# cvjena/mvlm

Measured on NVIDIA B200. Metric: scans/sec, higher is better.
Workload: dtype bf16

## Files before the change

### include/mvlm_b200.h

```cpp
#ifndef MVLM_B200_H
#define MVLM_B200_H

#include <stddef.h>
#include <stdint.h>

#ifdef __cplusplus
extern "C" {
#endif

#define MVLM_OK 0
#define MVLM_E_INVALID (-1)
#define MVLM_E_CUDA (-2)
#define MVLM_E_UNSUPPORTED (-3)

const char* mvlm_last_error(void);
int mvlm_version(void);
long long mvlm_launch_count(int reset);

typedef struct mvlm_conv_args {
  const void* in;
  int n, h, w, cin, in_cs;
  const void* wpacked;
  int cout_pad, n_tile, kh, kw, y_off0, x_off0;
  const float* bias;
  const float* pre_scale;
  const float* pre_shift;
  void* out_pre;
  int pre_cs, pre_co;
  const void* res1;
  int res1_cs, res1_co;
  const void* res2;
  int res2_cs, res2_co;
  void* out_raw;
  int raw_cs, raw_co;
  const float* post_scale;
  const float* post_shift;
  void* out_post;
  int post_cs, post_co;
  float* out_f32;
  unsigned long long* argmax_keys;
  int cout_real;
  int up_sy, up_sx, up_py, up_px;
  const float* mid_scale;
  const float* mid_shift;
  int pool2;
  const void* res_up;
  int up_cs, up_co;
} mvlm_conv_args;

int mvlm_conv2d_bf16(const mvlm_conv_args* args, void* stream);

void mvlm_debug_conv_profile(long long* dev_buf);
int mvlm_debug_conv_profile_ints(void);
void mvlm_debug_conv_mode(int mode);

int mvlm_pack_conv_weight(const float* w_oihw, int cout, int cin, int kh, int kw, int cout_pad,
                          int cin_pad, void* out_bf16, void* stream);

typedef struct mvlm_obj mvlm_obj;
int mvlm_obj_load(const char* path, int n_threads, mvlm_obj** out);
int mvlm_obj_counts(const mvlm_obj* obj, int* n_verts, int* n_tris, int* has_uv);
int mvlm_obj_copy(const mvlm_obj* obj, float* verts, float* uvs, int32_t* tris);
void mvlm_obj_free(mvlm_obj* obj);
#define MVLM_OBJ_MATERIALS 1
int mvlm_obj_load_ex(const char* path, int n_threads, int flags, mvlm_obj** out);
int mvlm_obj_materials(const mvlm_obj* obj, int32_t* tri_material, int* n_materials, int* n_libraries);
const char* mvlm_obj_material_name(const mvlm_obj* obj, int i);
const char* mvlm_obj_library_name(const mvlm_obj* obj, int i);
int mvlm_debug_obj_chunk_starts(const char* text, size_t len, int n_threads, long long* starts);

typedef struct mvlm_obj_parse_info {
  int32_t n_verts, n_tris, has_uv, fallback;
  int32_t n_positions;
  size_t n_bytes;
} mvlm_obj_parse_info;
size_t mvlm_obj_parse_workspace_bytes(size_t n_bytes);
int mvlm_obj_parse_device(const char* text_dev, size_t n_bytes, const char* path, void* workspace,
                          size_t workspace_bytes, void* stream, mvlm_obj_parse_info* info);
int mvlm_obj_parse_write(const mvlm_obj_parse_info* info, const void* workspace, float* verts, float* uvs,
                         int32_t* tris, void* stream);
#define MVLM_OBJ_MAX_NAME_LINES 65536
typedef struct mvlm_obj_name_line {
  int64_t offset;
  int32_t kind;
  int32_t tris_before;
} mvlm_obj_name_line;
size_t mvlm_obj_parse_workspace_bytes_ex(size_t n_bytes, int flags);
int mvlm_obj_parse_device_ex(const char* text_dev, size_t n_bytes, const char* path, void* workspace,
                             size_t workspace_bytes, int flags, void* stream, mvlm_obj_parse_info* info,
                             mvlm_obj_name_line* name_lines, int max_name_lines, int* n_name_lines);
int mvlm_obj_parse_tri_page(const mvlm_obj_parse_info* info, void* workspace, const int32_t* line_page, int n_usemtl,
                            int32_t* tri_page, void* stream);
int mvlm_debug_obj_parse_lines(const char* text, size_t len, int max_lines, int* n_lines, int32_t* kind,
                               int32_t* status, float* values, int32_t* n_tris, long long* corners,
                               long long max_corners);

typedef struct mvlm_mesh mvlm_mesh;
int mvlm_mesh_load(const char* path, int n_threads, mvlm_mesh** out);
int mvlm_mesh_counts(const mvlm_mesh* mesh, int* n_verts, int* n_tris, int* has_colors);
int mvlm_mesh_copy(const mvlm_mesh* mesh, float* verts, uint8_t* colors, int32_t* tris);
void mvlm_mesh_free(mvlm_mesh* mesh);

typedef struct mvlm_mesh_parse_info {
  int32_t n_verts, n_tris, has_colors, fallback;
  int32_t is_stl;
  size_t n_bytes;
} mvlm_mesh_parse_info;
size_t mvlm_mesh_parse_workspace_bytes(size_t n_bytes, int is_stl);
int mvlm_mesh_parse_device(const uint8_t* host, size_t n_bytes, int is_stl, const char* path, void* workspace,
                           size_t workspace_bytes, void* stream, mvlm_mesh_parse_info* info);
int mvlm_mesh_parse_write(const mvlm_mesh_parse_info* info, const void* workspace, float* verts, uint8_t* colors,
                          int32_t* tris, void* stream);

int mvlm_jpeg_info(const uint8_t* data, size_t len, int* width, int* height);
int mvlm_jpeg_decode_rgb(const uint8_t* data, size_t len, uint8_t* out_rgb_dev, int width, int height, void* stream);

size_t mvlm_raster_workspace_bytes(int n_views, int h, int w, int n_verts);
int mvlm_raster_multiview(const float* verts, int n_verts, const float* uvs, const int32_t* tris, int n_tris,
                          const uint8_t* tex, int tex_h, int tex_w, int tex_channels, const double* rot,
                          int n_views, int h, int w, int channel_mode, void* workspace, size_t workspace_bytes,
                          uint8_t* out_u8 , float* out_f32 ,
                          int32_t* out_tri_id , float* out_depth ,
                          void* stream);

#define MVLM_MAX_SCANS 64
typedef struct mvlm_raster_scan {
  const float* verts;
  int n_verts;
  const float* uvs;
  const int32_t* tris;
  int n_tris;
  const uint8_t* tex;
  int tex_h, tex_w, tex_channels;
} mvlm_raster_scan;
size_t mvlm_raster_multiscan_workspace_bytes(int n_scans, int n_views, int h, int w, int max_verts);
int mvlm_raster_multiscan(const mvlm_raster_scan* scans , int n_scans,
                          const double* rot , int n_views, int h, int w, int channel_mode, void* workspace,
                          size_t workspace_bytes, uint8_t* out_u8 , float* out_f32 ,
                          int32_t* out_tri_id , float* out_depth , void* stream);
int mvlm_raster_multiscan_colored(const mvlm_raster_scan* scans ,
                                  const uint8_t* const* vertex_rgba ,
                                  int n_scans, const double* rot , int n_views, int h, int w,
                                  int channel_mode, void* workspace, size_t workspace_bytes, uint8_t* out_u8,
                                  float* out_f32, int32_t* out_tri_id, float* out_depth, void* stream);
int mvlm_raster_multiscan_paged(const mvlm_raster_scan* scans ,
                                const uint8_t* const* vertex_rgba ,
                                const int32_t* const* pages ,
                                int n_scans, const double* rot , int n_views, int h, int w, int channel_mode,
                                void* workspace, size_t workspace_bytes, uint8_t* out_u8, float* out_f32,
                                int32_t* out_tri_id, float* out_depth, void* stream);

typedef struct mvlm_hourglass mvlm_hourglass;
size_t mvlm_hourglass_workspace_bytes(int n_landmarks, int cin, int n_views, int h, int w);
double mvlm_hourglass_flops_per_view(int n_landmarks, int cin, int h, int w);
int mvlm_hourglass_create(const char* const* names, const void* const* ptrs, const long long* numels,
                          int n_entries, int n_landmarks, int cin, int n_views, int h, int w, void* workspace,
                          size_t workspace_bytes, mvlm_hourglass** out);
int mvlm_hourglass_forward(mvlm_hourglass* net, const uint8_t* img_u8, const float* img_f32,
                           float* out_heatmaps, float* out_peaks, void* stream);
int mvlm_hourglass_forward_graph(mvlm_hourglass* net, const uint8_t* img_u8, const float* img_f32,
                                 float* out_heatmaps, float* out_peaks, void* stream);
int mvlm_hourglass_set_selection_method(mvlm_hourglass* net, int method);
int mvlm_hourglass_forward_keys(mvlm_hourglass* net, const uint8_t* img_u8, const float* img_f32, uint64_t* out_keys,
                                void* stream);
int mvlm_peaks_from_gathered_keys(const uint64_t* keys, int n_views, int n_landmarks, int w, int world, int slot_views,
                                  float* out_peaks , void* stream);
int mvlm_hourglass_num_launches(const mvlm_hourglass* net);
int mvlm_debug_hourglass_profile(mvlm_hourglass* net, const uint8_t* img_u8, const float* img_f32,
                                 float* out_peaks, int reps, float* ms_out, double* roles_out, int trace_op,
                                 long long* trace_out ,
                                 void* stream);
int mvlm_debug_hourglass_describe(const mvlm_hourglass* net, int op, char* buf, int buf_len);
int mvlm_hourglass_probe(const mvlm_hourglass* net, const char* name, const void** ptr, int* h, int* w, int* c);
void mvlm_hourglass_destroy(mvlm_hourglass* net);

int mvlm_heatmap_peaks(const float* heatmaps, int n_views, int n_landmarks, int h, int w, int method,
                       float* out_peaks, void* stream);

int mvlm_rays_from_peaks(const float* peaks , const double* rot , int n_landmarks,
                         int n_views, int image_size, double* out_starts, double* out_ends, void* stream);

size_t mvlm_consensus_workspace_bytes(int n_landmarks, int n_views, int n_hyp);
int mvlm_consensus(const float* peaks, const double* starts, const double* ends, int n_landmarks,
                   int n_views, int mode, double threshold_quantile, float threshold_absolute,
                   const uint32_t* draws, int n_hyp, double dist_thres, void* workspace,
                   size_t workspace_bytes, double* out_landmarks , double* out_errors ,
                   int32_t* out_nlines , void* stream);

size_t mvlm_consensus_multiscan_workspace_bytes(int n_scans, int n_landmarks, int n_views, int n_hyp);
int mvlm_consensus_multiscan(const float* peaks, const double* starts, const double* ends, int n_scans,
                             int n_landmarks, int n_views, int mode, double threshold_quantile,
                             float threshold_absolute, const uint32_t* draws, int draws_per_scan, int n_hyp,
                             double dist_thres, void* workspace, size_t workspace_bytes,
                             double* out_landmarks , double* out_errors ,
                             int32_t* out_nlines , void* stream);

size_t mvlm_snap_workspace_bytes(int n_landmarks, int n_tris);
int mvlm_snap_to_mesh(const float* verts, const int32_t* tris, int n_tris, const double* landmarks,
                      int n_landmarks, void* workspace, size_t workspace_bytes, double* out ,
                      int32_t* out_tri , void* stream);

size_t mvlm_snap_grid_bytes(int n_tris);
size_t mvlm_snap_grid_query_workspace_bytes(int n_landmarks, int n_tris);
int mvlm_snap_grid_build(const float* verts, const int32_t* tris, int n_tris, void* grid, size_t grid_bytes,
                         void* stream);
int mvlm_snap_grid_query(const float* verts, const int32_t* tris, int n_tris, const void* grid,
                         size_t grid_bytes, const double* landmarks, int n_landmarks, void* workspace,
                         size_t workspace_bytes, double* out , int32_t* out_tri ,
                         int32_t* out_stats , void* stream);
typedef struct mvlm_snap_mesh {
  const float* verts;
  const int32_t* tris;
  int n_tris;
  const void* grid;
  size_t grid_bytes;
} mvlm_snap_mesh;
size_t mvlm_snap_to_meshes_workspace_bytes(const mvlm_snap_mesh* meshes, int n_scans, int n_landmarks);
int mvlm_snap_to_meshes(const mvlm_snap_mesh* meshes, int n_scans, const double* landmarks ,
                        int n_landmarks, void* workspace, size_t workspace_bytes, double* out ,
                        int32_t* out_tri , void* stream);
int mvlm_debug_snap_grid_describe(const void* grid, int32_t* dims_nover , double* edge_tau ,
                                  void* stream);

#ifdef __cplusplus
}
#endif
#endif
```

### mvlm_b200/_lib.py

```python
from __future__ import annotations

import ctypes as C
import os
from pathlib import Path

_HERE = Path(__file__).resolve().parent
LIB_PATH = Path(os.environ.get("MVLM_B200_LIB") or _HERE / "libmvlm_b200.so")


class MvlmError(RuntimeError):
    pass


class ConvArgs(C.Structure):
    _fields_ = [
        ("in_", C.c_void_p),
        ("n", C.c_int), ("h", C.c_int), ("w", C.c_int), ("cin", C.c_int), ("in_cs", C.c_int),
        ("wpacked", C.c_void_p),
        ("cout_pad", C.c_int), ("n_tile", C.c_int), ("kh", C.c_int), ("kw", C.c_int),
        ("y_off0", C.c_int), ("x_off0", C.c_int),
        ("bias", C.c_void_p),
        ("pre_scale", C.c_void_p), ("pre_shift", C.c_void_p), ("out_pre", C.c_void_p),
        ("pre_cs", C.c_int), ("pre_co", C.c_int),
        ("res1", C.c_void_p), ("res1_cs", C.c_int), ("res1_co", C.c_int),
        ("res2", C.c_void_p), ("res2_cs", C.c_int), ("res2_co", C.c_int),
        ("out_raw", C.c_void_p), ("raw_cs", C.c_int), ("raw_co", C.c_int),
        ("post_scale", C.c_void_p), ("post_shift", C.c_void_p), ("out_post", C.c_void_p),
        ("post_cs", C.c_int), ("post_co", C.c_int),
        ("out_f32", C.c_void_p), ("argmax_keys", C.c_void_p),
        ("cout_real", C.c_int),
        ("up_sy", C.c_int), ("up_sx", C.c_int), ("up_py", C.c_int), ("up_px", C.c_int),
        ("mid_scale", C.c_void_p), ("mid_shift", C.c_void_p),
        ("pool2", C.c_int),
        ("res_up", C.c_void_p), ("up_cs", C.c_int), ("up_co", C.c_int),
    ]


class ObjParseInfo(C.Structure):
    _fields_ = [("n_verts", C.c_int32), ("n_tris", C.c_int32), ("has_uv", C.c_int32), ("fallback", C.c_int32),
                ("n_positions", C.c_int32), ("n_bytes", C.c_size_t)]


class ObjNameLine(C.Structure):
    _fields_ = [("offset", C.c_int64), ("kind", C.c_int32), ("tris_before", C.c_int32)]


class MeshParseInfo(C.Structure):
    _fields_ = [("n_verts", C.c_int32), ("n_tris", C.c_int32), ("has_colors", C.c_int32), ("fallback", C.c_int32),
                ("is_stl", C.c_int32), ("n_bytes", C.c_size_t)]


class RasterScan(C.Structure):
    _fields_ = [("verts", C.c_void_p), ("n_verts", C.c_int), ("uvs", C.c_void_p), ("tris", C.c_void_p),
                ("n_tris", C.c_int), ("tex", C.c_void_p), ("tex_h", C.c_int), ("tex_w", C.c_int),
                ("tex_channels", C.c_int)]


class SnapMesh(C.Structure):
    _fields_ = [("verts", C.c_void_p), ("tris", C.c_void_p), ("n_tris", C.c_int), ("grid", C.c_void_p),
                ("grid_bytes", C.c_size_t)]


MAX_SCANS = 64
OBJ_MATERIALS = 1
OBJ_MAX_NAME_LINES = 65536

_lib = None


def load() -> C.CDLL:
    global _lib
    if _lib is not None:
        return _lib
    if not LIB_PATH.exists():
        raise MvlmError(
            f"{LIB_PATH} is missing: run `python -m mvlm_b200.build` (there is no CPU fallback)")
    lib = C.CDLL(str(LIB_PATH))
    lib.mvlm_last_error.restype = C.c_char_p
    lib.mvlm_launch_count.restype = C.c_longlong
    lib.mvlm_launch_count.argtypes = [C.c_int]
    _lib = lib
    _declare(lib)
    return lib


def _declare(lib: C.CDLL) -> None:
    vp, i32, f32, f64, u64 = C.c_void_p, C.c_int, C.c_float, C.c_double, C.c_uint64
    sigs = {
        "mvlm_version": ([], i32),
        "mvlm_conv2d_bf16": ([C.POINTER(ConvArgs), vp], i32),
        "mvlm_pack_conv_weight": ([vp, i32, i32, i32, i32, i32, i32, vp, vp], i32),
        "mvlm_raster_workspace_bytes": ([i32, i32, i32, i32], C.c_size_t),
        "mvlm_raster_multiview": ([vp, i32, vp, vp, i32, vp, i32, i32, i32, vp, i32, i32, i32, i32, vp, C.c_size_t, vp, vp,
                                   vp, vp, vp], i32),
        "mvlm_raster_multiscan_workspace_bytes": ([i32, i32, i32, i32, i32], C.c_size_t),
        "mvlm_raster_multiscan": ([C.POINTER(RasterScan), i32, vp, i32, i32, i32, i32, vp, C.c_size_t, vp, vp, vp, vp, vp],
                                  i32),
        "mvlm_raster_multiscan_colored": ([C.POINTER(RasterScan), C.POINTER(vp), i32, vp, i32, i32, i32, i32, vp,
                                           C.c_size_t, vp, vp, vp, vp, vp], i32),
        "mvlm_raster_multiscan_paged": ([C.POINTER(RasterScan), C.POINTER(vp), C.POINTER(vp), i32, vp, i32, i32, i32,
                                         i32, vp, C.c_size_t, vp, vp, vp, vp, vp], i32),
        "mvlm_hourglass_workspace_bytes": ([i32, i32, i32, i32, i32], C.c_size_t),
        "mvlm_hourglass_flops_per_view": ([i32, i32, i32, i32], f64),
        "mvlm_hourglass_create": ([C.POINTER(C.c_char_p), C.POINTER(vp), C.POINTER(C.c_longlong), i32, i32, i32, i32,
                                   i32, i32, vp, C.c_size_t, C.POINTER(vp)], i32),
        "mvlm_hourglass_forward": ([vp, vp, vp, vp, vp, vp], i32),
        "mvlm_hourglass_forward_graph": ([vp, vp, vp, vp, vp, vp], i32),
        "mvlm_hourglass_set_selection_method": ([vp, i32], i32),
        "mvlm_hourglass_forward_keys": ([vp, vp, vp, vp, vp], i32),
        "mvlm_peaks_from_gathered_keys": ([vp, i32, i32, i32, i32, i32, vp, vp], i32),
        "mvlm_hourglass_num_launches": ([vp], i32),
        "mvlm_debug_hourglass_profile": ([vp, vp, vp, vp, i32, C.POINTER(C.c_float), C.POINTER(C.c_double), i32,
                                         C.POINTER(C.c_longlong), vp], i32),
        "mvlm_debug_conv_profile_ints": ([], i32),
        "mvlm_debug_hourglass_describe": ([vp, i32, C.c_char_p, i32], i32),
        "mvlm_hourglass_probe": ([vp, C.c_char_p, C.POINTER(vp), C.POINTER(i32), C.POINTER(i32), C.POINTER(i32)], i32),
        "mvlm_hourglass_destroy": ([vp], None),
        "mvlm_obj_load": ([C.c_char_p, i32, C.POINTER(vp)], i32),
        "mvlm_obj_counts": ([vp, C.POINTER(i32), C.POINTER(i32), C.POINTER(i32)], i32),
        "mvlm_obj_copy": ([vp, vp, vp, vp], i32),
        "mvlm_obj_free": ([vp], None),
        "mvlm_obj_load_ex": ([C.c_char_p, i32, i32, C.POINTER(vp)], i32),
        "mvlm_obj_materials": ([vp, vp, C.POINTER(i32), C.POINTER(i32)], i32),
        "mvlm_obj_material_name": ([vp, i32], C.c_char_p),
        "mvlm_obj_library_name": ([vp, i32], C.c_char_p),
        "mvlm_debug_obj_chunk_starts": ([C.c_char_p, C.c_size_t, i32, vp], i32),
        "mvlm_obj_parse_workspace_bytes": ([C.c_size_t], C.c_size_t),
        "mvlm_obj_parse_device": ([vp, C.c_size_t, C.c_char_p, vp, C.c_size_t, vp, C.POINTER(ObjParseInfo)], i32),
        "mvlm_obj_parse_write": ([C.POINTER(ObjParseInfo), vp, vp, vp, vp, vp], i32),
        "mvlm_obj_parse_workspace_bytes_ex": ([C.c_size_t, i32], C.c_size_t),
        "mvlm_obj_parse_device_ex": ([vp, C.c_size_t, C.c_char_p, vp, C.c_size_t, i32, vp, C.POINTER(ObjParseInfo),
                                      C.POINTER(ObjNameLine), i32, C.POINTER(i32)], i32),
        "mvlm_obj_parse_tri_page": ([C.POINTER(ObjParseInfo), vp, vp, i32, vp, vp], i32),
        "mvlm_debug_obj_parse_lines": ([C.c_char_p, C.c_size_t, i32, C.POINTER(i32), vp, vp, vp, vp, vp, C.c_longlong],
                                       i32),
        "mvlm_mesh_load": ([C.c_char_p, i32, C.POINTER(vp)], i32),
        "mvlm_mesh_counts": ([vp, C.POINTER(i32), C.POINTER(i32), C.POINTER(i32)], i32),
        "mvlm_mesh_copy": ([vp, vp, vp, vp], i32),
        "mvlm_mesh_free": ([vp], None),
        "mvlm_mesh_parse_workspace_bytes": ([C.c_size_t, i32], C.c_size_t),
        "mvlm_mesh_parse_device": ([vp, C.c_size_t, i32, C.c_char_p, vp, C.c_size_t, vp, C.POINTER(MeshParseInfo)], i32),
        "mvlm_mesh_parse_write": ([C.POINTER(MeshParseInfo), vp, vp, vp, vp, vp], i32),
        "mvlm_jpeg_info": ([C.c_char_p, C.c_size_t, C.POINTER(i32), C.POINTER(i32)], i32),
        "mvlm_jpeg_decode_rgb": ([C.c_char_p, C.c_size_t, vp, i32, i32, vp], i32),
        "mvlm_heatmap_peaks": ([vp, i32, i32, i32, i32, i32, vp, vp], i32),
        "mvlm_rays_from_peaks": ([vp, vp, i32, i32, i32, vp, vp, vp], i32),
        "mvlm_consensus_workspace_bytes": ([i32, i32, i32], C.c_size_t),
        "mvlm_consensus": ([vp, vp, vp, i32, i32, i32, f64, f32, vp, i32, f64, vp, C.c_size_t, vp, vp, vp, vp], i32),
        "mvlm_consensus_multiscan_workspace_bytes": ([i32, i32, i32, i32], C.c_size_t),
        "mvlm_consensus_multiscan": ([vp, vp, vp, i32, i32, i32, i32, f64, f32, vp, i32, i32, f64, vp, C.c_size_t, vp, vp,
                                      vp, vp], i32),
        "mvlm_snap_workspace_bytes": ([i32, i32], C.c_size_t),
        "mvlm_snap_to_meshes_workspace_bytes": ([C.POINTER(SnapMesh), i32, i32], C.c_size_t),
        "mvlm_snap_to_meshes": ([C.POINTER(SnapMesh), i32, vp, i32, vp, C.c_size_t, vp, vp, vp], i32),
        "mvlm_snap_to_mesh": ([vp, vp, i32, vp, i32, vp, C.c_size_t, vp, vp, vp], i32),
        "mvlm_snap_grid_bytes": ([i32], C.c_size_t),
        "mvlm_snap_grid_build": ([vp, vp, i32, vp, C.c_size_t, vp], i32),
        "mvlm_snap_grid_query_workspace_bytes": ([i32, i32], C.c_size_t),
        "mvlm_snap_grid_query": ([vp, vp, i32, vp, C.c_size_t, vp, i32, vp, C.c_size_t, vp, vp, vp, vp], i32),
        "mvlm_debug_snap_grid_describe": ([vp, vp, vp, vp], i32),
    }
    sigs.update(_EXTRA_SIGS)
    for name, (argtypes, restype) in sigs.items():
        fn = getattr(lib, name)
        fn.argtypes = argtypes
        fn.restype = restype


_EXTRA_SIGS: dict = {}


def check(rc: int, what: str = "") -> None:
    if rc != 0:
        msg = load().mvlm_last_error().decode("utf-8", "replace")
        raise MvlmError(f"{what or 'mvlm call'} failed ({rc}): {msg}")


def ptr(t) -> int | None:
    if t is None:
        return None
    return t.data_ptr()


def cur_stream() -> int:
    import torch

    return torch.cuda.current_stream().cuda_stream
```

### mvlm_b200/csrc/api.cu

```cuda
#include <stdarg.h>

#include <atomic>

#include "../../include/mvlm_b200.h"
#include "common.cuh"
#include "conv_umma.cuh"
#include "hourglass.cuh"
#include "stages.cuh"

namespace mvlm {

static thread_local char g_err[1024] = "";
static std::atomic<long long> g_launches{0};

void set_error(const char* fmt, ...) {
  va_list ap;
  va_start(ap, fmt);
  vsnprintf(g_err, sizeof(g_err), fmt, ap);
  va_end(ap);
}

void count_launch(int n) { g_launches.fetch_add(n, std::memory_order_relaxed); }

int sm_count() {
  static std::atomic<int> cached[kMaxDevices];
  int dev = 0;
  if (cudaGetDevice(&dev) != cudaSuccess || dev < 0 || dev >= kMaxDevices) return kNumSMs;
  int n = cached[dev].load(std::memory_order_relaxed);
  if (n == 0) {
    if (cudaDeviceGetAttribute(&n, cudaDevAttrMultiProcessorCount, dev) != cudaSuccess || n <= 0) n = kNumSMs;
    cached[dev].store(n, std::memory_order_relaxed);
  }
  return n;
}

}

using namespace mvlm;
static_assert(kMaxScans == MVLM_MAX_SCANS, "scan table size");

extern "C" {

const char* mvlm_last_error(void) { return g_err; }

int mvlm_version(void) { return 1; }

long long mvlm_launch_count(int reset) {
  return reset ? g_launches.exchange(0) : g_launches.load();
}

void mvlm_debug_conv_profile(long long* dev_buf) { conv_set_profile_buffer(dev_buf); }
int mvlm_debug_conv_profile_ints(void) { return kConvProfInts; }
void mvlm_debug_conv_mode(int mode) { conv_set_debug_mode(mode); }

int mvlm_conv2d_bf16(const mvlm_conv_args* a, void* stream) {
  MVLM_REQUIRE(a != nullptr, "mvlm_conv2d_bf16: null args");
  ConvShape s;
  s.in = static_cast<const __nv_bfloat16*>(a->in);
  s.n = a->n; s.h = a->h; s.w = a->w; s.cin = a->cin; s.in_cs = a->in_cs;
  s.wpacked = static_cast<const __nv_bfloat16*>(a->wpacked);
  s.cout_pad = a->cout_pad; s.n_tile = a->n_tile; s.kh = a->kh; s.kw = a->kw;
  s.y_off0 = a->y_off0; s.x_off0 = a->x_off0;
  ConvEpilogue e;
  e.bias = a->bias;
  e.mid_scale = a->mid_scale; e.mid_shift = a->mid_shift;
  e.pool2 = a->pool2 != 0;
  e.pre_scale = a->pre_scale; e.pre_shift = a->pre_shift;
  e.out_pre = static_cast<__nv_bfloat16*>(a->out_pre); e.pre_cs = a->pre_cs; e.pre_co = a->pre_co;
  e.res1 = static_cast<const __nv_bfloat16*>(a->res1); e.res1_cs = a->res1_cs; e.res1_co = a->res1_co;
  e.res2 = static_cast<const __nv_bfloat16*>(a->res2); e.res2_cs = a->res2_cs; e.res2_co = a->res2_co;
  e.res_up = static_cast<const __nv_bfloat16*>(a->res_up); e.up_cs = a->up_cs; e.up_co = a->up_co;
  e.out_raw = static_cast<__nv_bfloat16*>(a->out_raw); e.raw_cs = a->raw_cs; e.raw_co = a->raw_co;
  e.post_scale = a->post_scale; e.post_shift = a->post_shift;
  e.out_post = static_cast<__nv_bfloat16*>(a->out_post); e.post_cs = a->post_cs; e.post_co = a->post_co;
  e.out_f32 = a->out_f32; e.argmax_keys = a->argmax_keys; e.cout_real = a->cout_real;
  e.up_sy = a->up_sy > 0 ? a->up_sy : 1; e.up_sx = a->up_sx > 0 ? a->up_sx : 1;
  e.up_py = a->up_py; e.up_px = a->up_px;
  ConvParams p;
  int rc = conv_plan(s, e, &p);
  if (rc != MVLM_OK) return rc;
  return conv_launch(p, static_cast<cudaStream_t>(stream));
}

int mvlm_pack_conv_weight(const float* w_oihw, int cout, int cin, int kh, int kw, int cout_pad, int cin_pad,
                          void* out_bf16, void* stream) {
  MVLM_REQUIRE(w_oihw && out_bf16, "mvlm_pack_conv_weight: null pointer");
  MVLM_REQUIRE(cout_pad >= cout && cin_pad >= cin, "mvlm_pack_conv_weight: pads smaller than dims");
  const int rc = pack_conv_weight(w_oihw, cout, cin, kh, kw, cout_pad, cin_pad, static_cast<__nv_bfloat16*>(out_bf16),
                                  static_cast<cudaStream_t>(stream));
  count_launch();
  return rc;
}

size_t mvlm_raster_workspace_bytes(int n_views, int h, int w, int n_verts) {
  return raster_workspace_bytes(n_views, h, w, n_verts);
}

int mvlm_raster_multiview(const float* verts, int n_verts, const float* uvs, const int32_t* tris, int n_tris,
                          const uint8_t* tex, int tex_h, int tex_w, int tex_channels, const double* rot, int n_views, int h,
                          int w, int channel_mode, void* workspace, size_t workspace_bytes, uint8_t* out_u8, float* out_f32,
                          int32_t* out_tri_id, float* out_depth, void* stream) {
  const mvlm_raster_scan scan = {verts, n_verts, uvs, tris, n_tris, tex, tex_h, tex_w, tex_channels};
  return mvlm_raster_multiscan(&scan, 1, rot, n_views, h, w, channel_mode, workspace, workspace_bytes, out_u8, out_f32,
                               out_tri_id, out_depth, stream);
}

size_t mvlm_raster_multiscan_workspace_bytes(int n_scans, int n_views, int h, int w, int max_verts) {
  return raster_workspace_bytes(n_scans * n_views, h, w, max_verts);
}

int mvlm_raster_multiscan(const mvlm_raster_scan* scans, int n_scans, const double* rot, int n_views, int h, int w,
                          int channel_mode, void* workspace, size_t workspace_bytes, uint8_t* out_u8, float* out_f32,
                          int32_t* out_tri_id, float* out_depth, void* stream) {
  return mvlm_raster_multiscan_colored(scans, nullptr, n_scans, rot, n_views, h, w, channel_mode, workspace,
                                       workspace_bytes, out_u8, out_f32, out_tri_id, out_depth, stream);
}

int mvlm_raster_multiscan_colored(const mvlm_raster_scan* scans, const uint8_t* const* vertex_rgba, int n_scans,
                                  const double* rot, int n_views, int h, int w, int channel_mode, void* workspace,
                                  size_t workspace_bytes, uint8_t* out_u8, float* out_f32, int32_t* out_tri_id,
                                  float* out_depth, void* stream) {
  return mvlm_raster_multiscan_paged(scans, vertex_rgba, nullptr, n_scans, rot, n_views, h, w, channel_mode, workspace,
                                     workspace_bytes, out_u8, out_f32, out_tri_id, out_depth, stream);
}

int mvlm_raster_multiscan_paged(const mvlm_raster_scan* scans, const uint8_t* const* vertex_rgba,
                                const int32_t* const* pages, int n_scans, const double* rot, int n_views, int h, int w,
                                int channel_mode, void* workspace, size_t workspace_bytes, uint8_t* out_u8,
                                float* out_f32, int32_t* out_tri_id, float* out_depth, void* stream) {
  MVLM_REQUIRE(scans, "mvlm_raster_multiscan: null scan table");
  MVLM_REQUIRE(n_scans > 0 && n_scans <= kMaxScans, "mvlm_raster_multiscan: 1 to %d scans per pass (got %d)", kMaxScans,
               n_scans);
  RasterScan table[kMaxScans];
  for (int s = 0; s < n_scans; ++s) {
    const mvlm_raster_scan& q = scans[s];
    const uchar4* colors = vertex_rgba ? reinterpret_cast<const uchar4*>(vertex_rgba[s]) : nullptr;
    MVLM_REQUIRE((reinterpret_cast<uintptr_t>(colors) & 3) == 0, "mvlm_raster_multiscan: vertex colours of scan %d not 4-byte aligned", s);
    const int* paged = pages ? pages[s] : nullptr;
    MVLM_REQUIRE(!paged || (q.tex && q.uvs && q.tex_channels == 4 && (reinterpret_cast<uintptr_t>(q.tex) & 3) == 0),
                 "mvlm_raster_multiscan: scan %d has pages but no 4-byte aligned RGBA texel buffer and uvs", s);
    table[s] = RasterScan{q.verts, q.uvs, q.tris, q.tex, colors, paged, q.n_verts, q.n_tris, q.tex_h, q.tex_w,
                          q.tex_channels};
  }
  RasterArgs a;
  a.scans = table; a.n_scans = n_scans;
  a.rot = rot; a.n_views = n_views; a.h = h; a.w = w; a.channel_mode = channel_mode;
  a.zbuf = static_cast<unsigned long long*>(workspace); a.workspace_bytes = workspace_bytes;
  a.out_u8 = out_u8; a.out_f32 = out_f32; a.out_tri = out_tri_id; a.out_z = out_depth;
  return raster_launch(a, static_cast<cudaStream_t>(stream));
}

struct mvlm_hourglass {
  HourglassNet net;
};

size_t mvlm_hourglass_workspace_bytes(int n_landmarks, int cin, int n_views, int h, int w) {
  HourglassNet dry;
  if (dry.build(nullptr, n_landmarks, cin, n_views, h, w, nullptr, 0, true) != MVLM_OK) return 0;
  return dry.workspace_needed();
}

double mvlm_hourglass_flops_per_view(int n_landmarks, int cin, int h, int w) {
  HourglassNet dry;
  if (dry.build(nullptr, n_landmarks, cin, 1, h, w, nullptr, 0, true) != MVLM_OK) return 0.0;
  return dry.flops_per_view();
}

int mvlm_hourglass_create(const char* const* names, const void* const* ptrs, const long long* numels, int n_entries,
                          int n_landmarks, int cin, int n_views, int h, int w, void* workspace, size_t workspace_bytes,
                          mvlm_hourglass** out) {
  MVLM_REQUIRE(names && ptrs && out, "mvlm_hourglass_create: null pointer");
  StateDict sd;
  for (int i = 0; i < n_entries; ++i) {
    SdEntry e;
    e.p = static_cast<const float*>(ptrs[i]);
    e.numel = numels ? numels[i] : -1;
    sd[names[i]] = e;
  }
  mvlm_hourglass* h_ = new mvlm_hourglass();
  const int rc = h_->net.build(&sd, n_landmarks, cin, n_views, h, w, workspace, workspace_bytes, false);
  if (rc != MVLM_OK) {
    delete h_;
    return rc;
  }
  *out = h_;
  return MVLM_OK;
}

int mvlm_hourglass_forward(mvlm_hourglass* net, const uint8_t* img_u8, const float* img_f32, float* out_heatmaps,
                           float* out_peaks, void* stream) {
  MVLM_REQUIRE(net, "mvlm_hourglass_forward: null handle");
  return net->net.forward(img_u8, img_f32, out_heatmaps, out_peaks, static_cast<cudaStream_t>(stream));
}

int mvlm_hourglass_forward_graph(mvlm_hourglass* net, const uint8_t* img_u8, const float* img_f32,
                                 float* out_heatmaps, float* out_peaks, void* stream) {
  MVLM_REQUIRE(net, "mvlm_hourglass_forward_graph: null handle");
  return net->net.forward_graph(img_u8, img_f32, out_heatmaps, out_peaks, static_cast<cudaStream_t>(stream));
}

int mvlm_hourglass_set_selection_method(mvlm_hourglass* net, int method) {
  MVLM_REQUIRE(net, "mvlm_hourglass_set_selection_method: null handle");
  return net->net.set_selection_method(method);
}

int mvlm_hourglass_forward_keys(mvlm_hourglass* net, const uint8_t* img_u8, const float* img_f32, uint64_t* out_keys,
                                void* stream) {
  MVLM_REQUIRE(net, "mvlm_hourglass_forward_keys: null handle");
  return net->net.forward_keys(img_u8, img_f32, reinterpret_cast<unsigned long long*>(out_keys),
                               static_cast<cudaStream_t>(stream));
}

int mvlm_peaks_from_gathered_keys(const uint64_t* keys, int n_views, int n_landmarks, int w, int world, int slot_views,
                                  float* out_peaks, void* stream) {
  return peaks_from_gathered_keys(reinterpret_cast<const unsigned long long*>(keys), n_views, n_landmarks, w, world,
                                  slot_views, out_peaks, static_cast<cudaStream_t>(stream));
}

int mvlm_debug_hourglass_profile(mvlm_hourglass* net, const uint8_t* img_u8, const float* img_f32, float* out_peaks,
                                 int reps, float* ms_out, double* roles_out, int trace_op, long long* trace_out,
                                 void* stream) {
  MVLM_REQUIRE(net, "mvlm_debug_hourglass_profile: null handle");
  return net->net.profile_ops(img_u8, img_f32, out_peaks, reps, ms_out, roles_out, trace_op, trace_out,
                              static_cast<cudaStream_t>(stream));
}

int mvlm_debug_hourglass_describe(const mvlm_hourglass* net, int op, char* buf, int buf_len) {
  MVLM_REQUIRE(net && buf && buf_len > 0, "mvlm_debug_hourglass_describe: null pointer");
  snprintf(buf, buf_len, "%s", net->net.describe_op(op).c_str());
  return MVLM_OK;
}

int mvlm_hourglass_num_launches(const mvlm_hourglass* net) { return net ? net->net.n_ops() : 0; }

int mvlm_hourglass_probe(const mvlm_hourglass* net, const char* name, const void** ptr, int* h, int* w, int* c) {
  MVLM_REQUIRE(net && name && ptr && h && w && c, "mvlm_hourglass_probe: null pointer");
  auto it = net->net.probes.find(name);
  MVLM_REQUIRE(it != net->net.probes.end(), "mvlm_hourglass_probe: unknown probe %s", name);
  *ptr = it->second.p; *h = it->second.h; *w = it->second.w; *c = it->second.c;
  return MVLM_OK;
}

void mvlm_hourglass_destroy(mvlm_hourglass* net) { delete net; }

int mvlm_heatmap_peaks(const float* heatmaps, int n_views, int n_landmarks, int h, int w, int method,
                       float* out_peaks, void* stream) {
  return peaks_from_heatmaps(heatmaps, n_views, n_landmarks, h, w, method, out_peaks,
                             static_cast<cudaStream_t>(stream));
}

int mvlm_rays_from_peaks(const float* peaks, const double* rot, int n_landmarks, int n_views, int image_size,
                         double* out_starts, double* out_ends, void* stream) {
  return rays_from_peaks(peaks, rot, n_landmarks, n_views, image_size, out_starts, out_ends,
                         static_cast<cudaStream_t>(stream));
}

size_t mvlm_consensus_workspace_bytes(int n_landmarks, int n_views, int n_hyp) {
  return consensus_workspace_bytes(n_landmarks, n_views, n_hyp);
}

int mvlm_consensus(const float* peaks, const double* starts, const double* ends, int n_landmarks, int n_views,
                   int mode, double threshold_quantile, float threshold_absolute, const uint32_t* draws, int n_hyp,
                   double dist_thres, void* workspace, size_t workspace_bytes, double* out_landmarks,
                   double* out_errors, int32_t* out_nlines, void* stream) {
  return mvlm_consensus_multiscan(peaks, starts, ends, 1, n_landmarks, n_views, mode, threshold_quantile,
                                  threshold_absolute, draws, 0, n_hyp, dist_thres, workspace, workspace_bytes,
                                  out_landmarks, out_errors, out_nlines, stream);
}

size_t mvlm_consensus_multiscan_workspace_bytes(int n_scans, int n_landmarks, int n_views, int n_hyp) {
  return consensus_workspace_bytes(n_landmarks, n_views, n_hyp, n_scans);
}

int mvlm_consensus_multiscan(const float* peaks, const double* starts, const double* ends, int n_scans,
                             int n_landmarks, int n_views, int mode, double threshold_quantile,
                             float threshold_absolute, const uint32_t* draws, int draws_per_scan, int n_hyp,
                             double dist_thres, void* workspace, size_t workspace_bytes, double* out_landmarks,
                             double* out_errors, int32_t* out_nlines, void* stream) {
  ConsensusArgs a;
  a.peaks = peaks; a.starts = starts; a.ends = ends; a.l = n_landmarks; a.v = n_views; a.n_scans = n_scans;
  a.mode = mode;
  a.threshold_quantile = threshold_quantile; a.threshold_absolute = threshold_absolute;
  a.draws = draws; a.n_hyp = n_hyp; a.dist_thres = dist_thres;
  a.draws_scan_stride = draws_per_scan ? static_cast<size_t>(n_landmarks) * n_hyp * 8 : 0;
  a.workspace = workspace; a.workspace_bytes = workspace_bytes;
  a.out_landmarks = out_landmarks; a.out_errors = out_errors; a.out_nlines = out_nlines;
  return consensus_launch(a, static_cast<cudaStream_t>(stream));
}

size_t mvlm_snap_workspace_bytes(int n_landmarks, int n_tris) { return snap_workspace_bytes(n_landmarks, n_tris); }

int mvlm_snap_to_mesh(const float* verts, const int32_t* tris, int n_tris, const double* landmarks, int n_landmarks,
                      void* workspace, size_t workspace_bytes, double* out, int32_t* out_tri, void* stream) {
  return snap_launch(verts, tris, n_tris, landmarks, n_landmarks, workspace, workspace_bytes, out, out_tri,
                     static_cast<cudaStream_t>(stream));
}

size_t mvlm_snap_grid_bytes(int n_tris) { return snap_grid_bytes(n_tris); }

int mvlm_snap_grid_build(const float* verts, const int32_t* tris, int n_tris, void* grid, size_t grid_bytes, void* stream) {
  return snap_grid_build(verts, tris, n_tris, grid, grid_bytes, static_cast<cudaStream_t>(stream));
}

size_t mvlm_snap_grid_query_workspace_bytes(int n_landmarks, int n_tris) {
  return snap_grid_query_workspace_bytes(n_landmarks, n_tris);
}

int mvlm_snap_grid_query(const float* verts, const int32_t* tris, int n_tris, const void* grid, size_t grid_bytes,
                         const double* landmarks, int n_landmarks, void* workspace, size_t workspace_bytes, double* out,
                         int32_t* out_tri, int32_t* out_stats, void* stream) {
  return snap_grid_query(verts, tris, n_tris, grid, grid_bytes, landmarks, n_landmarks, workspace, workspace_bytes, out,
                         out_tri, out_stats, static_cast<cudaStream_t>(stream));
}

static int snap_table(const mvlm_snap_mesh* meshes, int n_scans, SnapMesh* table, const void** grids) {
  MVLM_REQUIRE(meshes, "mvlm_snap_to_meshes: null mesh table");
  MVLM_REQUIRE(n_scans > 0 && n_scans <= kMaxScans, "mvlm_snap_to_meshes: 1 to %d scans per pass (got %d)", kMaxScans,
               n_scans);
  for (int i = 0; i < n_scans; ++i) {
    table[i] = SnapMesh{meshes[i].verts, meshes[i].tris, meshes[i].n_tris};
// ... 33 lines not shown
```

### mvlm_b200/csrc/conv_epilogue.cuh

```cuda
#pragma once
#include "conv_umma.cuh"

#include <type_traits>

namespace mvlm {
namespace epi {

constexpr int kThreads = 352;
constexpr int kEpiWarps = 8;
constexpr int kTileW = 8;
constexpr int kMaxTileH = 32;
constexpr int kMTile = 128;
constexpr int kStageFloats = 16 * 36;
constexpr int kMaxCout = 256;
constexpr int kTraceTiles = 64;

enum : int { F_PRE = 1, F_RES1 = 2, F_RES2 = 4, F_RAW = 8, F_POST = 16, F_F32 = 32 , F_ARGMAX = 64,
              F_MID = 128 , F_POOL = 256 ,
              F_UP = 512 ,
              F_M64 = 1024 ,
              F_POST2 = 2048 ,
              F_POOLX = 4096 ,
              F_STAT = 8192  };
constexpr int F_HEAD = F_F32 | F_ARGMAX;

inline int feature_mask(const ConvEpilogue& e) {
  return (e.out_pre ? F_PRE : 0) | (e.res1 ? F_RES1 : 0) | (e.res2 ? F_RES2 : 0) | (e.out_raw ? F_RAW : 0) |
         (e.out_post ? F_POST : 0) | (e.out_f32 ? F_F32 : 0) | (e.argmax_keys ? F_ARGMAX : 0) |
         (e.mid_scale ? F_MID : 0) | (e.pool2 ? F_POOL : 0) | (e.res_up ? F_UP : 0) |
         (e.aux_mode == 1 ? F_POST2 : 0) | (e.aux_mode == 2 ? F_POOLX : 0);
}

#ifdef __CUDACC__

__device__ __forceinline__ uint32_t order_f32(float f) {
  const uint32_t b = __float_as_uint(f);
  return b ^ (static_cast<uint32_t>(static_cast<int32_t>(b) >> 31) | 0x80000000u);
}

__device__ __forceinline__ uint4 pack8(const float (&f)[8]) {
  __nv_bfloat162 a = __floats2bfloat162_rn(f[0], f[1]);
  __nv_bfloat162 b = __floats2bfloat162_rn(f[2], f[3]);
  __nv_bfloat162 c = __floats2bfloat162_rn(f[4], f[5]);
  __nv_bfloat162 d = __floats2bfloat162_rn(f[6], f[7]);
  uint4 r;
  r.x = *reinterpret_cast<uint32_t*>(&a);
  r.y = *reinterpret_cast<uint32_t*>(&b);
  r.z = *reinterpret_cast<uint32_t*>(&c);
  r.w = *reinterpret_cast<uint32_t*>(&d);
  return r;
}
__device__ __forceinline__ float fmax_nan(float a, float b) {
  float r;
  asm("max.NaN.f32 %0, %1, %2;" : "=f"(r) : "f"(a), "f"(b));
  return r;
}
__device__ __forceinline__ float fmax3_nan(float a, float b, float c) {
  float r;
  asm("max.NaN.f32 %0, %1, %2, %3;" : "=f"(r) : "f"(a), "f"(b), "f"(c));
  return r;
}
__device__ __forceinline__ uint32_t relu_bf16x2(float lo, float hi) {
  uint32_t r;
  asm("cvt.rn.relu.bf16x2.f32 %0, %1, %2;" : "=r"(r) : "f"(hi), "f"(lo));
  return r;
}
__device__ __forceinline__ uint4 affine_relu_pack8(const float (&f)[8], const float (&sc)[8], const float (&sh)[8]) {
  uint4 r;
  r.x = relu_bf16x2(fmaf(f[0], sc[0], sh[0]), fmaf(f[1], sc[1], sh[1]));
  r.y = relu_bf16x2(fmaf(f[2], sc[2], sh[2]), fmaf(f[3], sc[3], sh[3]));
  r.z = relu_bf16x2(fmaf(f[4], sc[4], sh[4]), fmaf(f[5], sc[5], sh[5]));
  r.w = relu_bf16x2(fmaf(f[6], sc[6], sh[6]), fmaf(f[7], sc[7], sh[7]));
  return r;
}
__device__ __forceinline__ void add8(const uint4& q, float (&f)[8]) {
  const __nv_bfloat162* h = reinterpret_cast<const __nv_bfloat162*>(&q);
#pragma unroll
  for (int j = 0; j < 4; ++j) {
    const float2 t = __bfloat1622float2(h[j]);
    f[2 * j] += t.x;
    f[2 * j + 1] += t.y;
  }
}
__device__ __forceinline__ uint4 max_bf16x8(const uint4& a, const uint4& b) {
  uint4 r;
  const __nv_bfloat162* pa = reinterpret_cast<const __nv_bfloat162*>(&a);
  const __nv_bfloat162* pb = reinterpret_cast<const __nv_bfloat162*>(&b);
  __nv_bfloat162* pr = reinterpret_cast<__nv_bfloat162*>(&r);
#pragma unroll
  for (int j = 0; j < 4; ++j) pr[j] = __hmax2(pa[j], pb[j]);
  return r;
}
__device__ __forceinline__ void lds8(const float* src, float (&v)[8]) {
  const float4 a = reinterpret_cast<const float4*>(src)[0];
  const float4 b = reinterpret_cast<const float4*>(src)[1];
  v[0] = a.x; v[1] = a.y; v[2] = a.z; v[3] = a.w; v[4] = b.x; v[5] = b.y; v[6] = b.z; v[7] = b.w;
}

__device__ __forceinline__ void timed_wait(uint64_t* b, uint32_t parity, bool prof, long long& acc) {
  if (!prof) { ptx::mbar_wait_trap(b, parity); return; }
  const long long t0 = clock64();
  ptx::mbar_wait_trap(b, parity);
  acc += clock64() - t0;
}

struct TileCoord {
  int mt, tx, ty, img;
};

struct ChannelParams {
  const float* bias;
  const float* mid_s;
  const float* mid_t;
  const float* pre_s;
  const float* pre_t;
  const float* post_s;
  const float* post_t;
};

struct ArgmaxState {
  uint32_t best_hi = 0u, best_lo = 0u;
  int cur_img = -1;
};

struct EpiTrace {
  long long* trace = nullptr;
  int trace_i = 0;
  long long t0 = 0;
  bool on = false;
};
#define MVLM_EPI_TRACE(slot)                                                                              \
  do {                                                                                                    \
    if (tr.on && tr.trace && tr.trace_i < kTraceTiles) tr.trace[tr.trace_i * 16 + (slot)] = clock64() - tr.t0; \
  } while (0)

template <int F>
__device__ __forceinline__ void epilogue_tile(const ConvShape& s, const ConvEpilogue& e, const int tile_h,
                                              const ChannelParams& ep, const TileCoord& tc,
                                              uint64_t* t_full, const uint32_t parity, const uint32_t tmem_acc,
                                              float* stage, const int ew, const int lane_grp, const int lane,
                                              ArgmaxState& am, const bool prof, long long& w0, EpiTrace& tr) {
  constexpr bool WS = (F & F_M64) != 0;
  constexpr int kM = kMTile;
  constexpr int kChGrp = 32;
  constexpr int kPitch = 36;
  constexpr int kCols = 16;
  constexpr int kUnitRows = kCols / 8;
  static_assert(kCols * kPitch <= kStageFloats, "transpose buffer");
  const int rep_log2 = !WS ? 0 : (s.cout_pad <= 32 ? 2 : 1);
  const int n_cgrp = 4 >> rep_log2;
  const int cgrp = lane_grp & (n_cgrp - 1);
  const int replica = lane_grp >> (2 - rep_log2);
  const int n_units = max(1, tile_h / kUnitRows);
  const int upr = max(1, n_units >> rep_log2);
  const int upw = max(1, upr >> 1);
  const int u_local = (ew >> 2) * upw;
  const int u_begin = replica * upr + u_local;
  const int oh = s.h * e.up_sy, ow = s.w * e.up_sx;
  const int pj = lane >> 2;
  const int cq = (lane & 3) * 8;
  constexpr bool kBf16Out = (F & (F_PRE | F_RAW | F_POST)) != 0;
  const uint32_t rs_pre = static_cast<uint32_t>(s.w * e.pre_cs) * 2u, rs_res1 = static_cast<uint32_t>(s.w * e.res1_cs) * 2u;
  const uint32_t rs_res2 = static_cast<uint32_t>(s.w * e.res2_cs) * 2u;
  const uint32_t rs_up = static_cast<uint32_t>((s.w >> 1) * e.up_cs) * 2u;
  const uint32_t rs_raw = static_cast<uint32_t>(((F & F_POOL) ? (s.w >> 1) : s.w) * e.raw_cs) * 2u;
  const uint32_t rs_post = static_cast<uint32_t>(((F & F_POOL) ? (s.w >> 1) : s.w) * e.post_cs) * 2u;
  const uint32_t rs_aux1 = static_cast<uint32_t>(((F & F_POOLX) ? (s.w >> 1) : s.w) * e.aux1_cs) * 2u;
  const uint32_t rs_aux2 = static_cast<uint32_t>((s.w >> 1) * e.aux2_cs) * 2u;
  constexpr bool kHasRes = (F & (F_RES1 | F_RES2 | F_UP)) != 0;
  constexpr int kMaxUpw = WS ? 4 : 8;
  constexpr int kResRegs = 4 * (2 * (((F & F_RES1) ? 1 : 0) + ((F & F_RES2) ? 1 : 0)) + ((F & F_UP) ? 1 : 0));
  constexpr int kResBudget = 64;
  constexpr int kPref = !kHasRes ? 1 : (kResRegs * kMaxUpw <= kResBudget ? kMaxUpw : (kResRegs * kMaxUpw <= 2 * kResBudget ? kMaxUpw / 2 : (kMaxUpw >= 4 ? kMaxUpw / 4 : 1)));
  uint4 r1[kPref][2], r2[(F & F_RES2) ? kPref : 1][2], ru[(F & F_UP) ? kPref : 1][1];

  const int m0 = tc.mt * kM;
  const int c_lane = m0 + cgrp * kChGrp + lane;
  const int c0 = m0 + cgrp * kChGrp + cq;
  const bool grp_active = m0 + cgrp * kChGrp < s.cout_pad;
  const int y_first = tc.ty * tile_h + kUnitRows * u_begin;
  const bool rows_active = u_local < upr && y_first < s.h;
  const bool ch_ok = c0 < s.cout_pad;
  const int xa = tc.tx * kTileW + pj;
  const bool vx = ch_ok && xa < s.w;
  auto pix = [&]() __attribute__((always_inline)) { return (static_cast<uint32_t>(tc.img) * s.h + y_first) * s.w + xa; };
  auto ppix = [&]() __attribute__((always_inline)) {
    return (static_cast<uint32_t>(tc.img) * (s.h >> 1) + (y_first >> 1)) * (s.w >> 1) + (xa >> 1);
  };
  if ((F & F_ARGMAX) && tc.img != am.cur_img) {
    if (am.cur_img >= 0 && am.best_hi != 0u && c_lane < e.cout_real)
      atomicMax(e.argmax_keys + static_cast<size_t>(am.cur_img) * e.cout_real + c_lane,
                (static_cast<unsigned long long>(am.best_hi) << 32) | am.best_lo);
    am.best_hi = 0u; am.best_lo = 0u;
    am.cur_img = tc.img;
  }
  uint8_t* const b_pre = (F & F_PRE) ? reinterpret_cast<uint8_t*>(e.out_pre + e.pre_co + c0 + static_cast<size_t>(pix()) * e.pre_cs) : nullptr;
  uint8_t* const b_raw = (F & F_RAW) ? reinterpret_cast<uint8_t*>(e.out_raw + e.raw_co + c0 + static_cast<size_t>((F & F_POOL) ? ppix() : pix()) * e.raw_cs) : nullptr;
  uint8_t* const b_post = (F & F_POST) ? reinterpret_cast<uint8_t*>(e.out_post + e.post_co + c0 + static_cast<size_t>((F & F_POOL) ? ppix() : pix()) * e.post_cs) : nullptr;
  uint8_t* const b_aux1 = (F & (F_POST2 | F_POOLX)) ? reinterpret_cast<uint8_t*>(e.out_aux1 + e.aux1_co + c0 + static_cast<size_t>((F & F_POOLX) ? ppix() : pix()) * e.aux1_cs) : nullptr;
  uint8_t* const b_aux2 = (F & F_POOLX) ? reinterpret_cast<uint8_t*>(e.out_aux2 + e.aux2_co + c0 + static_cast<size_t>(ppix()) * e.aux2_cs) : nullptr;
  const int n_rows_ok = vx ? s.h - y_first : 0;
  const uint8_t* const b_res1 = (F & F_RES1) ? reinterpret_cast<const uint8_t*>(e.res1 + e.res1_co + c0 + static_cast<size_t>(pix()) * e.res1_cs) : nullptr;
  const uint8_t* const b_res2 = (F & F_RES2) ? reinterpret_cast<const uint8_t*>(e.res2 + e.res2_co + c0 + static_cast<size_t>(pix()) * e.res2_cs) : nullptr;
  const uint8_t* const b_up = (F & F_UP) ? reinterpret_cast<const uint8_t*>(e.res_up + e.up_co + c0 + static_cast<size_t>(ppix()) * e.up_cs) : nullptr;
  auto prefetch_batch = [&](int u0) __attribute__((always_inline)) {
#pragma unroll
    for (int q = 0; q < kPref; ++q) {
      const int u = u0 + q;
      if (u < upw) {
#pragma unroll
        for (int ip = 0; ip < 2; ++ip) {
          const int row = kUnitRows * u + ip;
          if (row < n_rows_ok) {
            if (F & F_RES1) r1[q][ip] = *reinterpret_cast<const uint4*>(b_res1 + static_cast<size_t>(row * rs_res1));
            if (F & F_RES2) r2[q][ip] = *reinterpret_cast<const uint4*>(b_res2 + static_cast<size_t>(row * rs_res2));
            if ((F & F_UP) && ip == 0)
              ru[q][0] = *reinterpret_cast<const uint4*>(b_up + static_cast<size_t>((row >> 1) * rs_up));
          }
        }
      }
    }
  };
  if (kHasRes && grp_active && rows_active) prefetch_batch(0);
  float pre_s[8], pre_t[8], post_s[8], post_t[8];
  const int c0_ok = ch_ok ? c0 : 0;
  if (F & F_PRE) { lds8(ep.pre_s + c0_ok, pre_s); lds8(ep.pre_t + c0_ok, pre_t); }
  if (F & F_POST) { lds8(ep.post_s + c0_ok, post_s); lds8(ep.post_t + c0_ok, post_t); }
  const int c_lane_ok = c_lane < s.cout_pad ? c_lane : 0;
  const float bias_c = ep.bias[c_lane_ok];
  const float mid_s_c = ep.mid_s[c_lane_ok], mid_t_c = ep.mid_t[c_lane_ok];
  MVLM_EPI_TRACE(7);
  timed_wait(t_full, parity, prof, w0);
  ptx::tc_fence_after();
  MVLM_EPI_TRACE(5);
  if (grp_active && rows_active) {
    const uint32_t taddr = tmem_acc + (static_cast<uint32_t>(lane_grp * 32) << 16) + static_cast<uint32_t>((WS ? u_local : u_begin) * kCols);
    uint32_t vr[kCols];
    auto tmem_load = [&](int u) __attribute__((always_inline)) { ptx::tmem_ld16(taddr + u * kCols, vr); };
    tmem_load(0);
#pragma unroll
    for (int r = 0; r < kMaxUpw; ++r) {
      if (r < upw) {
        if (kHasRes && kPref < kMaxUpw && r > 0 && r % kPref == 0) prefetch_batch(r);
        const int y = y_first + kUnitRows * r;
        ptx::tmem_ld_wait();
        if (r < 2) MVLM_EPI_TRACE(8 + 4 * r);
        if (y < s.h) {
          if (F & F_HEAD) {
            const int x0 = tc.tx * kTileW;
            const int nvx = s.w - x0;
            bool exact_search = c_lane < e.cout_real;
            if constexpr ((F & F_HEAD) == F_ARGMAX) {
              if (c_lane < e.cout_real) {
                auto unit = [&](auto interior_c) __attribute__((always_inline)) {
                  constexpr bool kInterior = decltype(interior_c)::value;
                  auto ok = [&](int j) __attribute__((always_inline)) { return kInterior || ((j & 7) < nvx && y + (j >> 3) < s.h); };
                  float w[kCols];
#pragma unroll
                  for (int j = 0; j < kCols; ++j) w[j] = ok(j) ? __uint_as_float(vr[j]) : -INFINITY;
                  float m = fmax3_nan(w[0], w[1], w[2]);
#pragma unroll
                  for (int j = 3; j + 1 < kCols; j += 2) m = fmax3_nan(m, w[j], w[j + 1]);
                  m = fmax_nan(m, w[kCols - 1]);
                  const float mb = m + bias_c;
                  const uint32_t key = order_f32(mb);
                  exact_search = mb != mb;
                  if (key >= am.best_hi && !exact_search) {
                    const uint32_t mbits = __float_as_uint(mb);
                    int jf = kCols - 1;
#pragma unroll
                    for (int j = kCols - 2; j >= 0; --j)
                      if (__float_as_uint(w[j] + bias_c) == mbits && ok(j)) jf = j;
                    const int oy = (y + (jf >> 3)) * e.up_sy + e.up_py;
                    const uint32_t lo = 0xFFFFFFFFu - static_cast<uint32_t>(oy * ow + (x0 + (jf & 7)) * e.up_sx + e.up_px);
                    if (key > am.best_hi || lo > am.best_lo) {
                      am.best_hi = key;
                      am.best_lo = lo;
                    }
                  }
                };
                if (nvx >= kTileW && y + kUnitRows <= s.h) unit(std::true_type());
                else unit(std::false_type());
              }
            }
            if (exact_search) {
#pragma unroll
              for (int i = 0; i < kUnitRows; ++i) {
                if (y + i < s.h) {
                  const int oy = (y + i) * e.up_sy + e.up_py;
                  const uint32_t idx0 = static_cast<uint32_t>(oy * ow + x0 * e.up_sx + e.up_px);
                  if (F & F_ARGMAX) {
                    uint32_t k8[8];
                    uint32_t j8[8];
#pragma unroll
                    for (int j = 0; j < 8; ++j) {
                      k8[j] = j < nvx ? order_f32(__uint_as_float(vr[8 * i + j]) + bias_c) : 0u;
                      j8[j] = static_cast<uint32_t>(j);
                    }
#pragma unroll
                    for (int st = 1; st < 8; st *= 2) {
#pragma unroll
                      for (int j = 0; j < 8; j += 2 * st) {
                        const bool take = k8[j + st] > k8[j];
                        k8[j] = take ? k8[j + st] : k8[j];
                        j8[j] = take ? j8[j + st] : j8[j];
                      }
                    }
                    const uint32_t lo = 0xFFFFFFFFu - (idx0 + j8[0] * static_cast<uint32_t>(e.up_sx));
                    if (k8[0] > am.best_hi || (k8[0] == am.best_hi && lo > am.best_lo)) {
                      am.best_hi = k8[0];
                      am.best_lo = lo;
                    }
                  }
                  if (F & F_F32) {
                    float* dst = e.out_f32 + (static_cast<size_t>(tc.img) * e.cout_real + c_lane) * oh * ow + idx0;
#pragma unroll
                    for (int j = 0; j < 8; ++j)
                      if (j < nvx) dst[j * e.up_sx] = __uint_as_float(vr[8 * i + j]) + bias_c;
                  }
                }
              }
            }
          }
// ... 101 lines not shown
```

### mvlm_b200/csrc/conv_umma.cu

```cuda
#include "conv_epilogue.cuh"

#include <algorithm>
#include <type_traits>
#include <atomic>

namespace mvlm {

namespace {

using namespace epi;
constexpr int kMaxHSlots = 4;
constexpr int kMaxWSlots = 12;
constexpr int kPoolBytes = 198 * 1024;

struct __align__(8) Barriers {
  uint64_t h_full[kMaxHSlots];
  uint64_t h_empty[kMaxHSlots];
  uint64_t w_full[kMaxWSlots];
  uint64_t w_empty[kMaxWSlots];
  uint64_t t_full[2];
  uint64_t t_empty[2];
  uint32_t tmem_base;
};
static_assert(sizeof(Barriers) <= 512, "barrier block");

struct EpiParams {
  float bias[kMaxCout];
  float mid_s[kMaxCout];
  float mid_t[kMaxCout];
  float pre_s[kMaxCout];
  float pre_t[kMaxCout];
  float post_s[kMaxCout];
  float post_t[kMaxCout];
};

constexpr int kSmemBytes = kPoolBytes + kEpiWarps * kStageFloats * 4 + 512 + static_cast<int>(sizeof(EpiParams)) +
                           1024 ;
static_assert(kSmemBytes <= 227 * 1024, "shared memory budget");

__device__ __forceinline__ TileCoord decode_tile(const ConvParams& p, int t) {
  TileCoord c;
  c.mt = t % p.n_nt;
  int r = t / p.n_nt;
  c.tx = r % p.tiles_x;
  r /= p.tiles_x;
  c.ty = r % p.tiles_y;
  c.img = r / p.tiles_y;
  return c;
}

struct TileIter {
  TileCoord c, d;
  int n_nt, tiles_x, tiles_y;
  __device__ __forceinline__ TileIter(const ConvParams& p, int t_begin, int t_step)
      : c(decode_tile(p, t_begin)), d(decode_tile(p, t_step)), n_nt(p.n_nt), tiles_x(p.tiles_x), tiles_y(p.tiles_y) {}
  __device__ __forceinline__ void next() {
    c.mt += d.mt;
    int carry = c.mt >= n_nt ? 1 : 0;
    c.mt -= carry ? n_nt : 0;
    c.tx += d.tx + carry;
    carry = c.tx >= tiles_x ? 1 : 0;
    c.tx -= carry ? tiles_x : 0;
    c.ty += d.ty + carry;
    carry = c.ty >= tiles_y ? 1 : 0;
    c.ty -= carry ? tiles_y : 0;
    c.img += d.img + carry;
  }
};

template <int F>
__global__ void __launch_bounds__(kThreads, 1) conv_umma_kernel(const __grid_constant__ ConvParams p) {
  constexpr bool ARGMAX = (F & F_ARGMAX) != 0;
  extern __shared__ uint8_t smem_raw[];
  const uint32_t raw_addr = ptx::smem_u32(smem_raw);
  uint8_t* smem = smem_raw + ((1024u - (raw_addr & 1023u)) & 1023u);
  uint8_t* h_slots = smem;
  uint8_t* w_slots = smem + p.n_hslots * p.h_slot_bytes;
  float* stage_all = reinterpret_cast<float*>(smem + kPoolBytes);
  Barriers* bar = reinterpret_cast<Barriers*>(reinterpret_cast<uint8_t*>(stage_all) + kEpiWarps * kStageFloats * 4);
  EpiParams* ep = reinterpret_cast<EpiParams*>(reinterpret_cast<uint8_t*>(bar) + 512);

  const int warp = threadIdx.x >> 5;
  const int lane = threadIdx.x & 31;

  const ConvShape& s = p.s;
  const ConvEpilogue& e = p.e;
  const int n_chunks = (s.cin + 63) >> 6;
  const int n_hslots = p.n_hslots, n_wslots = p.n_wslots;
  const int halo_px = kTileW + s.kw - 1;
  const int halo_rows = p.tile_h + s.kh - 1;
  constexpr bool M64 = (F & F_M64) != 0;
  constexpr bool STAT = (F & F_STAT) != 0;
  constexpr int kM = M64 ? 64 : kMTile;
  const int w_rows = s.cout_pad < kM ? s.cout_pad : kM;
  const int mma_m = M64 ? (s.cout_pad <= 32 ? 32 : 64) : kMTile;
  const uint32_t w_tap_bytes = M64 ? 64u * 128u : ((static_cast<uint32_t>(w_rows) * 128u + 1023u) & ~1023u);
  const uint32_t w_slot_bytes = w_tap_bytes * static_cast<uint32_t>(M64 ? s.kh : 1);
  const bool w_stat = p.w_stationary != 0;

  int t_begin, t_end, t_step;
  if (ARGMAX) {
    const int per = (p.total_tiles + gridDim.x - 1) / gridDim.x;
    t_begin = blockIdx.x * per;
    t_end = min(p.total_tiles, t_begin + per);
    t_step = 1;
  } else {
    t_begin = blockIdx.x; t_end = p.total_tiles; t_step = gridDim.x;
  }

  for (int i = threadIdx.x; i < s.cout_pad; i += kThreads) {
    ep->bias[i] = e.bias ? e.bias[i] : 0.f;
    ep->mid_s[i] = e.mid_scale ? e.mid_scale[i] : (e.aux_scale ? e.aux_scale[i] : 1.f);
    ep->mid_t[i] = e.mid_scale ? e.mid_shift[i] : (e.aux_shift ? e.aux_shift[i] : 0.f);
    ep->pre_s[i] = e.out_pre ? e.pre_scale[i] : 0.f;
    ep->pre_t[i] = e.out_pre ? e.pre_shift[i] : 0.f;
    ep->post_s[i] = e.out_post ? e.post_scale[i] : 0.f;
    ep->post_t[i] = e.out_post ? e.post_shift[i] : 0.f;
  }
  if (warp == 0 && lane == 0) {
    ptx::tma_prefetch_desc(&p.tm_a);
    ptx::tma_prefetch_desc(&p.tm_b);
    if (p.tail) { ptx::tma_prefetch_desc(&p.tm_a2); ptx::tma_prefetch_desc(&p.tm_b2); }
    if (F & F_RES1) ptx::tma_prefetch_desc(&p.tm_r1);
    if (F & F_RES2) ptx::tma_prefetch_desc(&p.tm_r2);
    if (F & F_UP) ptx::tma_prefetch_desc(&p.tm_up);
    for (int i = 0; i < n_hslots; ++i) {
      ptx::mbar_init(&bar->h_full[i], 1);
      ptx::mbar_init(&bar->h_empty[i], 1);
    }
    for (int i = 0; i < n_wslots; ++i) {
      ptx::mbar_init(&bar->w_full[i], 1);
      ptx::mbar_init(&bar->w_empty[i], 1);
    }
    for (int i = 0; i < 2; ++i) {
      ptx::mbar_init(&bar->t_full[i], 1);
      ptx::mbar_init(&bar->t_empty[i], kEpiWarps);
    }
    ptx::fence_mbar_init();
  }
  if (warp == 1) {
    ptx::tmem_alloc(&bar->tmem_base, 512);
    ptx::tmem_relinquish();
  }
  ptx::tc_fence_before();
  __syncthreads();
  ptx::tc_fence_after();
  asm volatile("griddepcontrol.wait;" ::: "memory");
  asm volatile("griddepcontrol.launch_dependents;" ::: "memory");
  const uint32_t tmem_base = bar->tmem_base;
  const bool prof = p.prof != nullptr;
  const long long t_kernel0 = clock64();
  long long w0 = 0, w1 = 0;
  long long* const trace = (prof && blockIdx.x == 0) ? p.prof + kNumSMs * 8 : nullptr;
  int trace_i = 0;
#define MVLM_TRACE(slot)                                                                  \
  do {                                                                                    \
    if (trace && trace_i < kTraceTiles) trace[trace_i * 16 + (slot)] = clock64() - t_kernel0; \
  } while (0)

  if (warp == 0) {
    if (ptx::elect_one() && (p.debug_mode & 1) == 0) {
      int sh = 0;
      uint32_t ph = 0;
      TileIter it(p, t_begin, t_step);
      for (int t = t_begin; t < t_end; t += t_step, it.next()) {
        const TileCoord tc = it.c;
        const int x0 = tc.tx * kTileW + s.x_off0;
        const int y0 = tc.ty * p.tile_h + s.y_off0;
        for (int c = 0; c < n_chunks; ++c) {
          const bool is_tail = p.tail != 0 && c == n_chunks - 1;
          const uint32_t row_b = is_tail ? static_cast<uint32_t>(p.tail) * 2u : 128u;
          timed_wait(&bar->h_empty[sh], ph ^ 1, prof, w0);
          ptx::mbar_expect_tx(&bar->h_full[sh], static_cast<uint32_t>(halo_rows * halo_px) * row_b);
          ptx::tma_load_4d(is_tail ? &p.tm_a2 : &p.tm_a, &bar->h_full[sh], h_slots + sh * p.h_slot_bytes, c * 64, x0, y0, tc.img);
          if (c == 0) MVLM_TRACE(0);
          if (++sh == n_hslots) { sh = 0; ph ^= 1; }
        }
        if constexpr ((F & (F_RES1 | F_RES2 | F_UP)) != 0) {
          const int xa = tc.tx * kTileW, ya = tc.ty * p.tile_h, c_lo = tc.mt * kM;
          if (F & F_RES1) ptx::tma_prefetch_l2_4d(&p.tm_r1, c_lo, xa, ya, tc.img);
          if (F & F_RES2) ptx::tma_prefetch_l2_4d(&p.tm_r2, c_lo, xa, ya, tc.img);
          if (F & F_UP) ptx::tma_prefetch_l2_4d(&p.tm_up, c_lo, xa >> 1, ya >> 1, tc.img);
        }
        ++trace_i;
      }
      if (prof) { p.prof[blockIdx.x * 8 + 0] = w0; p.prof[blockIdx.x * 8 + 7] = clock64() - t_kernel0; }
    }
  } else if (warp == 10) {
    if (ptx::elect_one() && (p.debug_mode & 1) == 0) {
      int sw = 0;
      uint32_t pw = 0;
      for (int t = t_begin; t < t_end; t += t_step) {
        const int mt = t % p.n_nt;
        for (int c = 0; c < n_chunks; ++c) {
          const bool is_tail = p.tail != 0 && c == n_chunks - 1;
          const void* tmb = is_tail ? &p.tm_b2 : &p.tm_b;
          const uint32_t row_b = is_tail ? static_cast<uint32_t>(p.tail) * 2u : 128u;
          const uint32_t wb = static_cast<uint32_t>(w_rows) * row_b;
          if constexpr (M64) {
            for (int kx = 0; kx < s.kw; ++kx) {
              if (!w_stat) timed_wait(&bar->w_empty[sw], pw ^ 1, prof, w1);
              ptx::mbar_expect_tx(&bar->w_full[sw], wb * static_cast<uint32_t>(s.kh));
              for (int ky = 0; ky < s.kh; ++ky)
                ptx::tma_load_2d(tmb, &bar->w_full[sw], w_slots + sw * w_slot_bytes + ky * w_tap_bytes,
                                 (kx * s.kh + ky) * s.cin + c * 64, mt * kM);
              if (++sw == n_wslots) { sw = 0; pw ^= 1; }
            }
          } else
          for (int tap = 0; tap < s.kw * s.kh; ++tap) {
            if (!w_stat) timed_wait(&bar->w_empty[sw], pw ^ 1, prof, w1);
            ptx::mbar_expect_tx(&bar->w_full[sw], wb);
            ptx::tma_load_2d(tmb, &bar->w_full[sw], w_slots + sw * w_slot_bytes, tap * s.cin + c * 64, mt * kM);
            if (++sw == n_wslots) { sw = 0; pw ^= 1; }
          }
        }
        MVLM_TRACE(1);
        ++trace_i;
        if (w_stat) break;
      }
      if (prof) p.prof[blockIdx.x * 8 + 1] = w1;
    }
  } else if (warp == 1) {
    if (ptx::elect_one()) {
      const uint32_t idesc = ptx::umma_idesc_bf16(mma_m, p.tile_h * kTileW);
      const bool live = (p.debug_mode & 1) == 0;
      const int n_kx = s.kw, n_ky = s.kh;
      const uint32_t tail_row_b = p.tail ? static_cast<uint32_t>(p.tail) * 2u : 128u;
      const uint32_t tail_swz = !p.tail ? 2u : (p.tail == 16 ? 6u : 4u);
      const uint64_t a_hi_full = static_cast<uint64_t>(((8u * 128u) >> 4) | (1u << 14) | (2u << 29)) << 32;
      const uint64_t b_hi_full = static_cast<uint64_t>(((static_cast<uint32_t>(halo_px) * 128u) >> 4) | (1u << 14) | (2u << 29)) << 32;
      const uint64_t a_hi_tail = static_cast<uint64_t>(((8u * tail_row_b) >> 4) | (1u << 14) | (tail_swz << 29)) << 32;
      const uint64_t b_hi_tail = static_cast<uint64_t>(((static_cast<uint32_t>(halo_px) * tail_row_b) >> 4) | (1u << 14) | (tail_swz << 29)) << 32;
      const uint32_t h_lo0 = (ptx::smem_u32(h_slots) >> 4) | (1u << 16), h_step = static_cast<uint32_t>(p.h_slot_bytes) >> 4;
      const uint32_t w_lo0 = (ptx::smem_u32(w_slots) >> 4) | (1u << 16), w_step = w_slot_bytes >> 4;
      const int last_chunk = n_chunks - 1;
      const int nk_last = (s.cin - last_chunk * 64) >= 64 ? 4 : ((s.cin - last_chunk * 64) >> 4);
      int sh = 0, sw = 0;
      uint32_t ph = 0, pw = 0;
      int acc = 0;
      uint32_t pacc = 0;
      bool w_wait = live;
      for (int t = t_begin; t < t_end; t += t_step) {
        timed_wait(&bar->t_empty[acc], pacc ^ 1, prof, w1);
        ptx::tc_fence_after();
        MVLM_TRACE(2);
        const uint32_t d = tmem_base + static_cast<uint32_t>(acc * 256);
        uint32_t accumulate = 0;
        for (int c = 0; c < n_chunks; ++c) {
          const bool is_tail = p.tail != 0 && c == last_chunk;
          const int nk = c == last_chunk ? nk_last : 4;
          const uint32_t rb16 = (is_tail ? tail_row_b : 128u) >> 4;
          const uint64_t a_hi = is_tail ? a_hi_tail : a_hi_full;
          const uint64_t b_hi = is_tail ? b_hi_tail : b_hi_full;
          const uint32_t ky_step = static_cast<uint32_t>(halo_px) * rb16;
          if (live) timed_wait(&bar->h_full[sh], ph, prof, w0);
          if (c == 0) MVLM_TRACE(3);
          uint32_t x_col = h_lo0 + static_cast<uint32_t>(sh) * h_step;
          if (STAT && !w_wait && (nk == 4 || nk == 2 || nk == 1)) {
            auto taps = [&](auto nk_c, auto kk_c) __attribute__((always_inline)) {
              constexpr int NK = decltype(nk_c)::value;
              constexpr int KK = decltype(kk_c)::value;
              constexpr uint32_t kRb16 = NK * 2;
              const uint32_t tap16 = M64 ? (64u * 128u >> 4) : w_step;
              const uint32_t w_base = w_lo0 + static_cast<uint32_t>(c * KK * KK) * tap16;
#pragma unroll
              for (int tap = 0; tap < KK * KK; ++tap) {
                const uint32_t x_lo = x_col + static_cast<uint32_t>(((tap % KK) * (kTileW + KK - 1) + tap / KK)) * kRb16;
                const uint32_t w_lo = w_base + static_cast<uint32_t>(tap) * tap16;
#pragma unroll
                for (int k = 0; k < NK; ++k) {
                  const uint32_t en = (tap == 0 && k == 0) ? accumulate : 1u;
                  if constexpr (M64) ptx::umma_ws_bf16(d, a_hi | (w_lo + 2 * k), b_hi | (x_lo + 2 * k), idesc, en);
                  else ptx::umma_bf16(d, a_hi | (w_lo + 2 * k), b_hi | (x_lo + 2 * k), idesc, en);
                }
              }
              accumulate = 1;
            };
            using std::integral_constant;
            if constexpr (M64) {
              if (nk == 4) taps(integral_constant<int, 4>(), integral_constant<int, 3>());
              else if (nk == 2) taps(integral_constant<int, 2>(), integral_constant<int, 3>());
              else taps(integral_constant<int, 1>(), integral_constant<int, 3>());
            } else {
              if (nk == 4) taps(integral_constant<int, 4>(), integral_constant<int, 2>());
              else if (nk == 2) taps(integral_constant<int, 2>(), integral_constant<int, 2>());
              else taps(integral_constant<int, 1>(), integral_constant<int, 2>());
            }
          } else if constexpr (M64) {
            for (int kx = 0; kx < n_kx; ++kx, x_col += rb16) {
              if (w_wait) timed_wait(&bar->w_full[sw], w_stat ? 0u : pw, prof, w0);
              uint32_t x_lo = x_col;
              uint32_t w_lo = w_lo0 + static_cast<uint32_t>(sw) * w_step;
              for (int ky = 0; ky < n_ky; ++ky, x_lo += ky_step, w_lo += (w_tap_bytes >> 4)) {
                ptx::umma_ws_bf16(d, a_hi | w_lo, b_hi | x_lo, idesc, accumulate);
                if (nk == 4) {
                  ptx::umma_ws_bf16(d, a_hi | (w_lo + 2), b_hi | (x_lo + 2), idesc, 1u);
                  ptx::umma_ws_bf16(d, a_hi | (w_lo + 4), b_hi | (x_lo + 4), idesc, 1u);
                  ptx::umma_ws_bf16(d, a_hi | (w_lo + 6), b_hi | (x_lo + 6), idesc, 1u);
                } else {
                  for (int k = 1; k < nk; ++k) ptx::umma_ws_bf16(d, a_hi | (w_lo + 2 * k), b_hi | (x_lo + 2 * k), idesc, 1u);
                }
                accumulate = 1;
              }
              if (live && !w_stat) ptx::umma_commit(&bar->w_empty[sw]);
              if (++sw == n_wslots) { sw = 0; pw ^= 1; }
            }
          } else
          for (int kx = 0; kx < n_kx; ++kx, x_col += rb16) {
            uint32_t x_lo = x_col;
            for (int ky = 0; ky < n_ky; ++ky, x_lo += ky_step) {
              if (w_wait) timed_wait(&bar->w_full[sw], w_stat ? 0u : pw, prof, w0);
              const uint32_t w_lo = w_lo0 + static_cast<uint32_t>(sw) * w_step;
              auto mma = [&](int k, uint32_t en) __attribute__((always_inline)) {
                if constexpr (M64) ptx::umma_ws_bf16(d, a_hi | (w_lo + 2 * k), b_hi | (x_lo + 2 * k), idesc, en);
                else ptx::umma_bf16(d, a_hi | (w_lo + 2 * k), b_hi | (x_lo + 2 * k), idesc, en);
              };
              mma(0, accumulate);
              if (nk == 4) {
                mma(1, 1u); mma(2, 1u); mma(3, 1u);
              } else {
                for (int k = 1; k < nk; ++k) mma(k, 1u);
              }
              accumulate = 1;
              if (live && !w_stat) ptx::umma_commit(&bar->w_empty[sw]);
              if (++sw == n_wslots) { sw = 0; pw ^= 1; }
            }
          }
          if (live) ptx::umma_commit(&bar->h_empty[sh]);
          if (++sh == n_hslots) { sh = 0; ph ^= 1; }
        }
        ptx::umma_commit(&bar->t_full[acc]);
        MVLM_TRACE(4);
        ++trace_i;
        if (w_stat) w_wait = false;
        if (++acc == 2) { acc = 0; pacc ^= 1; }
      }
      if (prof) { p.prof[blockIdx.x * 8 + 2] = w0; p.prof[blockIdx.x * 8 + 3] = w1; p.prof[blockIdx.x * 8 + 4] = clock64() - t_kernel0; }
    }
  } else {
    float* stage = stage_all + (warp - 2) * kStageFloats;
    const ChannelParams cp = {ep->bias, ep->mid_s, ep->mid_t, ep->pre_s, ep->pre_t, ep->post_s, ep->post_t};
    int acc = 0;
    uint32_t pacc = 0;
    ArgmaxState am;
    EpiTrace tr;
    tr.trace = trace; tr.t0 = t_kernel0; tr.on = warp == 2 && lane == 0;
    TileIter it(p, t_begin, t_step);
    for (int t = t_begin; t < t_end; t += t_step, it.next()) {
      const TileCoord tc = it.c;
      tr.trace_i = trace_i;
      if (p.debug_mode & 2) {
        timed_wait(&bar->t_full[acc], pacc, prof, w0);
        ptx::tc_fence_after();
      } else {
        epilogue_tile<F>(s, e, p.tile_h, cp, tc, &bar->t_full[acc], pacc, tmem_base + static_cast<uint32_t>(acc * 256),
                         stage, warp - 2, warp & 3, lane, am, prof, w0, tr);
      }
      ptx::tc_fence_before();
      __syncwarp();
      if (lane == 0) ptx::mbar_arrive(&bar->t_empty[acc]);
      if (warp == 2 && lane == 0) MVLM_TRACE(6);
      ++trace_i;
      if (++acc == 2) { acc = 0; pacc ^= 1; }
    }
    epilogue_argmax_flush<F>(s, e, warp & 3, lane, am);
    if (prof && warp == 2 && lane == 0) { p.prof[blockIdx.x * 8 + 5] = w0; p.prof[blockIdx.x * 8 + 6] = clock64() - t_kernel0; }
  }

#undef MVLM_TRACE
  ptx::tc_fence_before();
  __syncthreads();
  if (warp == 1) {
    ptx::tc_fence_after();
    ptx::tmem_dealloc(tmem_base, 512);
  }
}

typedef CUresult (*EncodeTiledFn)(CUtensorMap*, CUtensorMapDataType, cuuint32_t, void*,
                                  const cuuint64_t*, const cuuint64_t*, const cuuint32_t*,
                                  const cuuint32_t*, CUtensorMapInterleave, CUtensorMapSwizzle,
                                  CUtensorMapL2promotion, CUtensorMapFloatOOBfill);

EncodeTiledFn get_encode_fn() {
  static EncodeTiledFn fn = nullptr;
  if (fn) return fn;
  void* sym = nullptr;
  cudaDriverEntryPointQueryResult q;
  if (cudaGetDriverEntryPoint("cuTensorMapEncodeTiled", &sym, cudaEnableDefault, &q) != cudaSuccess ||
      q != cudaDriverEntryPointSuccess || !sym)
    return nullptr;
  fn = reinterpret_cast<EncodeTiledFn>(sym);
  return fn;
}

template <int F>
int launch_t(const ConvParams& p, cudaStream_t stream) {
  static std::atomic<bool> configured[kMaxDevices];
  int dev = 0;
  MVLM_CHECK_CUDA(cudaGetDevice(&dev));
  if (dev < 0 || dev >= kMaxDevices || !configured[dev].load(std::memory_order_acquire)) {
    MVLM_CHECK_CUDA(cudaFuncSetAttribute(conv_umma_kernel<F>, cudaFuncAttributeMaxDynamicSharedMemorySize, kSmemBytes));
    if (dev >= 0 && dev < kMaxDevices) configured[dev].store(true, std::memory_order_release);
  }
  const int n_sms = sm_count();
  const int grid = p.total_tiles < n_sms ? p.total_tiles : n_sms;
  cudaLaunchConfig_t cfg = {};
  cfg.gridDim = dim3(static_cast<unsigned>(grid));
  cfg.blockDim = dim3(kThreads);
  cfg.dynamicSmemBytes = kSmemBytes;
  cfg.stream = stream;
  cudaLaunchAttribute attr[1];
  attr[0].id = cudaLaunchAttributeProgrammaticStreamSerialization;
  attr[0].val.programmaticStreamSerializationAllowed = 1;
  cfg.attrs = attr;
  cfg.numAttrs = 1;
  MVLM_CHECK_CUDA(cudaLaunchKernelEx(&cfg, conv_umma_kernel<F>, p));
  count_launch();
  MVLM_CHECK_CUDA(cudaGetLastError());
  return MVLM_OK;
}

thread_local long long* g_prof_buf = nullptr;
thread_local int g_debug_mode = 0;

}

int conv_plan(const ConvShape& s, const ConvEpilogue& e, ConvParams* out) {
  MVLM_REQUIRE(s.in && s.wpacked, "conv_plan: null input/weights");
  MVLM_REQUIRE(s.n > 0 && s.h > 0 && s.w > 0, "conv_plan: bad image dims %d %d %d", s.n, s.h, s.w);
  MVLM_REQUIRE(s.cin >= 16 && s.cin % 16 == 0, "conv_plan: cin=%d must be a multiple of 16", s.cin);
  MVLM_REQUIRE(s.in_cs >= s.cin && s.in_cs % 8 == 0, "conv_plan: in_cs=%d invalid", s.in_cs);
  MVLM_REQUIRE(s.cout_pad >= 16 && s.cout_pad % 16 == 0, "conv_plan: cout_pad=%d must be a multiple of 16", s.cout_pad);
  MVLM_REQUIRE(s.cout_pad <= kMTile || s.cout_pad % kMTile == 0,
               "conv_plan: cout_pad=%d must be <= 128 or a multiple of 128", s.cout_pad);
  MVLM_REQUIRE(s.cout_pad <= kMaxCout, "conv_plan: cout_pad=%d exceeds %d", s.cout_pad, kMaxCout);
  MVLM_REQUIRE(!e.argmax_keys || s.cout_pad <= kMTile, "conv_plan: fused arg-max needs cout_pad <= 128");
  MVLM_REQUIRE(!e.pool2 || (s.h % 2 == 0 && s.w % 2 == 0 && (e.out_raw || e.out_post) && !e.out_f32 && !e.argmax_keys),
               "conv_plan: pool2 needs even H, W and a bf16 raw/post output");
  MVLM_REQUIRE(!e.res_up || (s.h % 2 == 0 && s.w % 2 == 0 && !e.pool2 && !e.out_f32 && !e.argmax_keys),
               "conv_plan: res_up needs even H, W and bf16 outputs");
  MVLM_REQUIRE(!e.mid_scale || (e.mid_shift && !e.out_f32 && !e.argmax_keys), "conv_plan: mid affine needs mid_shift and bf16 outputs");
  MVLM_REQUIRE(e.aux_mode >= 0 && e.aux_mode <= 2, "conv_plan: unknown aux_mode %d", e.aux_mode);
  MVLM_REQUIRE(e.aux_mode == 0 || (e.aux_scale && e.aux_shift && e.out_aux1 && !e.mid_scale && !e.pool2 && !e.out_f32 &&
                                   !e.argmax_keys && e.aux1_cs % 8 == 0),
               "conv_plan: aux copies need aux_scale / aux_shift / out_aux1 and cannot be combined with mid / pool2 / fp32 outputs");
  MVLM_REQUIRE(e.aux_mode != 2 || (e.out_aux2 && e.aux2_cs % 8 == 0 && s.h % 2 == 0 && s.w % 2 == 0),
               "conv_plan: pooled aux copies need out_aux2 and even H, W");
  MVLM_REQUIRE(!((e.argmax_keys || e.out_f32) && (e.res1 || e.res2 || e.out_pre || e.out_raw || e.out_post)),
               "conv_plan: fp32 / arg-max outputs cannot be combined with bf16 outputs or residual inputs");
  MVLM_REQUIRE(1ll * s.n * s.h * s.w < (1ll << 32), "conv_plan: %d x %d x %d pixels exceed 32-bit pixel indices", s.n, s.h, s.w);
  MVLM_REQUIRE(s.kh >= 1 && s.kh <= 3 && s.kw >= 1 && s.kw <= 3, "conv_plan: kernel %dx%d unsupported", s.kh, s.kw);
  MVLM_REQUIRE((reinterpret_cast<uintptr_t>(s.in) & 15) == 0 && (reinterpret_cast<uintptr_t>(s.wpacked) & 15) == 0,
               "conv_plan: pointers must be 16-byte aligned");
  EncodeTiledFn enc = get_encode_fn();
  if (!enc) {
    set_error("conv_plan: cuTensorMapEncodeTiled entry point unavailable");
    return MVLM_E_CUDA;
  }
  ConvParams p;
  memset(&p, 0, sizeof(p));
  p.s = s;
  p.e = e;
  const int tile_h = s.h >= 32 ? kMaxTileH : (s.h >= 16 ? 16 : ((s.h >= 8 || s.cout_pad <= 64) ? 8 : 4));
  p.tile_h = tile_h;
  {
    const int hbytes = (kTileW + s.kw - 1) * (tile_h + s.kh - 1) * 128;
    p.h_slot_bytes = (hbytes + 1023) & ~1023;
    const int m_tile = s.cout_pad <= 64 ? 64 : kMTile;
    const int w_tap = m_tile == 64 ? 64 * 128 : ((std::min(s.cout_pad, kMTile) * 128 + 1023) & ~1023);
    const int wslot = w_tap * (m_tile == 64 ? s.kh : 1);
    const int n_wtiles = ((s.cin + 63) / 64) * (m_tile == 64 ? s.kw : s.kh * s.kw);
    int nh = s.kh * s.kw == 1 ? 3 : 2, nw = s.kh * s.kw == 1 ? 6 : (m_tile == 64 ? kMaxWSlots : 7);
    const bool fits_128 = m_tile == kMTile && s.cout_pad <= kMTile && n_wtiles <= kMaxWSlots &&
                          nh * p.h_slot_bytes + n_wtiles * wslot <= kPoolBytes;
    p.w_stationary = (m_tile == 64 ? n_wtiles * wslot <= kMaxWSlots * 8192 : fits_128) ? 1 : 0;
    if (p.w_stationary) nw = n_wtiles;
    while (nh * p.h_slot_bytes + nw * wslot > kPoolBytes && nw > 2 && !p.w_stationary) --nw;
    while (nh * p.h_slot_bytes + nw * wslot > kPoolBytes && nh > 2) --nh;
    MVLM_REQUIRE(nh * p.h_slot_bytes + nw * wslot <= kPoolBytes, "conv_plan: operand rings do not fit");
    p.n_hslots = nh;
    p.n_wslots = nw;
  }
  {
    cuuint64_t gdim[4] = {(cuuint64_t)s.cin, (cuuint64_t)s.w, (cuuint64_t)s.h, (cuuint64_t)s.n};
    cuuint64_t gstr[3] = {(cuuint64_t)s.in_cs * 2, (cuuint64_t)s.in_cs * 2 * s.w,
                          (cuuint64_t)s.in_cs * 2 * s.w * s.h};
    cuuint32_t box[4] = {64, (cuuint32_t)(kTileW + s.kw - 1), (cuuint32_t)(tile_h + s.kh - 1), 1};
    cuuint32_t estr[4] = {1, 1, 1, 1};
    CUresult r = enc(&p.tm_a, CU_TENSOR_MAP_DATA_TYPE_BFLOAT16, 4, const_cast<__nv_bfloat16*>(s.in), gdim, gstr,
                     box, estr, CU_TENSOR_MAP_INTERLEAVE_NONE, CU_TENSOR_MAP_SWIZZLE_128B,
                     CU_TENSOR_MAP_L2_PROMOTION_L2_128B, CU_TENSOR_MAP_FLOAT_OOB_FILL_NONE);
    if (r != CUDA_SUCCESS) {
      set_error("conv_plan: cuTensorMapEncodeTiled(X) failed with %d (cin=%d w=%d h=%d n=%d cs=%d)", (int)r, s.cin,
                s.w, s.h, s.n, s.in_cs);
      return MVLM_E_CUDA;
    }
  }
  {
    const cuuint64_t ktot = (cuuint64_t)s.kw * s.kh * s.cin;
    cuuint64_t gdim[2] = {ktot, (cuuint64_t)s.cout_pad};
    cuuint64_t gstr[1] = {ktot * 2};
    cuuint32_t box[2] = {64, (cuuint32_t)(s.cout_pad < kMTile ? s.cout_pad : kMTile)};
    cuuint32_t estr[2] = {1, 1};
    CUresult r = enc(&p.tm_b, CU_TENSOR_MAP_DATA_TYPE_BFLOAT16, 2, const_cast<__nv_bfloat16*>(s.wpacked), gdim,
                     gstr, box, estr, CU_TENSOR_MAP_INTERLEAVE_NONE, CU_TENSOR_MAP_SWIZZLE_128B,
                     CU_TENSOR_MAP_L2_PROMOTION_L2_256B, CU_TENSOR_MAP_FLOAT_OOB_FILL_NONE);
    if (r != CUDA_SUCCESS) {
      set_error("conv_plan: cuTensorMapEncodeTiled(W) failed with %d (ktot=%llu cout_pad=%d)", (int)r,
                (unsigned long long)ktot, s.cout_pad);
      return MVLM_E_CUDA;
    }
  }
  p.tail = (s.cin % 64 == 16 || s.cin % 64 == 32) ? s.cin % 64 : 0;
  if (p.tail) {
    const CUtensorMapSwizzle sw = p.tail == 16 ? CU_TENSOR_MAP_SWIZZLE_32B : CU_TENSOR_MAP_SWIZZLE_64B;
    cuuint64_t gdim[4] = {(cuuint64_t)s.cin, (cuuint64_t)s.w, (cuuint64_t)s.h, (cuuint64_t)s.n};
    cuuint64_t gstr[3] = {(cuuint64_t)s.in_cs * 2, (cuuint64_t)s.in_cs * 2 * s.w, (cuuint64_t)s.in_cs * 2 * s.w * s.h};
    cuuint32_t box[4] = {(cuuint32_t)p.tail, (cuuint32_t)(kTileW + s.kw - 1), (cuuint32_t)(tile_h + s.kh - 1), 1};
    cuuint32_t estr[4] = {1, 1, 1, 1};
    CUresult r = enc(&p.tm_a2, CU_TENSOR_MAP_DATA_TYPE_BFLOAT16, 4, const_cast<__nv_bfloat16*>(s.in), gdim, gstr, box,
                     estr, CU_TENSOR_MAP_INTERLEAVE_NONE, sw, CU_TENSOR_MAP_L2_PROMOTION_L2_128B,
                     CU_TENSOR_MAP_FLOAT_OOB_FILL_NONE);
    const cuuint64_t ktot = (cuuint64_t)s.kw * s.kh * s.cin;
    cuuint64_t gdim2[2] = {ktot, (cuuint64_t)s.cout_pad};
    cuuint64_t gstr2[1] = {ktot * 2};
    cuuint32_t box2[2] = {(cuuint32_t)p.tail, (cuuint32_t)(s.cout_pad < kMTile ? s.cout_pad : kMTile)};
    CUresult r2 = enc(&p.tm_b2, CU_TENSOR_MAP_DATA_TYPE_BFLOAT16, 2, const_cast<__nv_bfloat16*>(s.wpacked), gdim2,
                      gstr2, box2, estr, CU_TENSOR_MAP_INTERLEAVE_NONE, sw, CU_TENSOR_MAP_L2_PROMOTION_L2_256B,
                      CU_TENSOR_MAP_FLOAT_OOB_FILL_NONE);
    if (r != CUDA_SUCCESS || r2 != CUDA_SUCCESS) {
      set_error("conv_plan: cuTensorMapEncodeTiled(tail %d) failed with %d / %d", p.tail, (int)r, (int)r2);
      return MVLM_E_CUDA;
    }
  }
  {
    auto res_map = [&](CUtensorMap* tm, const __nv_bfloat16* base, int co, int cs, int hh, int ww, int box_w, int box_h) -> bool {
      if (!base) return true;
      const int c_ext = std::min(s.cout_pad, cs);
      cuuint64_t gdim[4] = {(cuuint64_t)c_ext, (cuuint64_t)ww, (cuuint64_t)hh, (cuuint64_t)s.n};
      cuuint64_t gstr[3] = {(cuuint64_t)cs * 2, (cuuint64_t)cs * 2 * ww, (cuuint64_t)cs * 2 * ww * hh};
      cuuint32_t box[4] = {(cuuint32_t)std::min(c_ext, s.cout_pad <= 64 ? 64 : kMTile), (cuuint32_t)box_w, (cuuint32_t)box_h, 1};
      cuuint32_t estr[4] = {1, 1, 1, 1};
      return enc(tm, CU_TENSOR_MAP_DATA_TYPE_BFLOAT16, 4, const_cast<__nv_bfloat16*>(base + co), gdim, gstr, box, estr,
                 CU_TENSOR_MAP_INTERLEAVE_NONE, CU_TENSOR_MAP_SWIZZLE_NONE, CU_TENSOR_MAP_L2_PROMOTION_L2_128B,
                 CU_TENSOR_MAP_FLOAT_OOB_FILL_NONE) == CUDA_SUCCESS;
    };
    const bool ok = res_map(&p.tm_r1, e.res1, e.res1_co, e.res1_cs, s.h, s.w, kTileW, tile_h) &&
                    res_map(&p.tm_r2, e.res2, e.res2_co, e.res2_cs, s.h, s.w, kTileW, tile_h) &&
                    res_map(&p.tm_up, e.res_up, e.up_co, e.up_cs, s.h >> 1, s.w >> 1, kTileW / 2, std::max(1, tile_h / 2));
    if (!ok) {
      set_error("conv_plan: cuTensorMapEncodeTiled(residual) failed (cout_pad=%d w=%d h=%d)", s.cout_pad, s.w, s.h);
      return MVLM_E_CUDA;
    }
  }
  p.tiles_x = ceil_div(s.w, kTileW);
  p.tiles_y = ceil_div(s.h, tile_h);
  p.n_nt = s.cout_pad <= 64 ? 1 : ceil_div(s.cout_pad, kMTile);
  p.total_tiles = s.n * p.tiles_x * p.tiles_y * p.n_nt;
  p.prof = nullptr;
  p.debug_mode = 0;
  *out = p;
  return MVLM_OK;
}

void conv_set_profile_buffer(long long* dev_buf) { g_prof_buf = dev_buf; }
void conv_set_debug_mode(int mode) { g_debug_mode = mode; }

int conv_launch(const ConvParams& p_in, cudaStream_t stream) {
  ConvParams p = p_in;
  p.prof = g_prof_buf;
  p.debug_mode = g_debug_mode;
  const ConvEpilogue& e = p.e;
  const int f = feature_mask(e);
  const bool m64 = p.s.cout_pad <= 64;
  const bool stat = m64 && p.w_stationary && p.s.kw == 3 && p.s.kh == 3;
#define MVLM_CASE_BOTH(FLAGS) \
  case (FLAGS):               \
    return m64 ? (stat ? launch_t<(FLAGS) | F_M64 | F_STAT>(p, stream) : launch_t<(FLAGS) | F_M64>(p, stream)) : launch_t<(FLAGS)>(p, stream)
#define MVLM_CASE_128(FLAGS) \
  case (FLAGS):              \
    if (!m64) return launch_t<(FLAGS)>(p, stream); \
    break
  if (f == F_ARGMAX && !m64 && p.w_stationary && p.s.kw == 2 && p.s.kh == 2) return launch_t<F_ARGMAX | F_STAT>(p, stream);
  switch (f) {
    MVLM_CASE_BOTH(F_PRE | F_RES1 | F_RAW | F_POST);
    MVLM_CASE_BOTH(F_PRE | F_RES1 | F_RAW);
    MVLM_CASE_BOTH(F_RES1 | F_RAW | F_POST);
    MVLM_CASE_BOTH(F_RES1 | F_RAW);
    MVLM_CASE_BOTH(F_RAW);
    MVLM_CASE_128(F_PRE);
    MVLM_CASE_128(F_RES1 | F_RES2 | F_RAW | F_POST);
    MVLM_CASE_128(F_ARGMAX);
    MVLM_CASE_BOTH(F_F32);
    MVLM_CASE_BOTH(F_F32 | F_ARGMAX);
    MVLM_CASE_BOTH(F_MID | F_PRE | F_POST);
    MVLM_CASE_BOTH(F_POOL | F_PRE | F_RES1 | F_RAW | F_POST);
    MVLM_CASE_BOTH(F_POOL | F_RES1 | F_RAW | F_POST);
    MVLM_CASE_BOTH(F_POOL | F_RAW);
    MVLM_CASE_128(F_PRE | F_RES1 | F_RES2 | F_RAW | F_POST);
    MVLM_CASE_BOTH(F_UP | F_PRE | F_RES1 | F_RAW | F_POST);
    MVLM_CASE_BOTH(F_UP | F_PRE | F_RES1 | F_RAW);
    MVLM_CASE_BOTH(F_UP | F_RES1 | F_RAW | F_POST);
    MVLM_CASE_BOTH(F_UP | F_RES1 | F_RAW);
    MVLM_CASE_BOTH(F_POST2 | F_PRE | F_RES1 | F_RAW | F_POST);
    MVLM_CASE_BOTH(F_POST2 | F_RES1 | F_RAW | F_POST);
    MVLM_CASE_BOTH(F_POOLX | F_PRE | F_RES1 | F_RAW | F_POST);
    MVLM_CASE_BOTH(F_POOLX | F_RES1 | F_RAW | F_POST);
    MVLM_CASE_128(F_POOLX | F_RES1 | F_RES2 | F_RAW | F_POST);
  }
#undef MVLM_CASE_BOTH
#undef MVLM_CASE_128
  set_error("conv_launch: unsupported epilogue combination 0x%x (cout_pad %d)", f, p.s.cout_pad);
  return MVLM_E_UNSUPPORTED;
}

}
```

### mvlm_b200/csrc/conv_umma.cuh

```cuda
#pragma once
#include "common.cuh"

namespace mvlm {

struct ConvEpilogue {
  const float* bias = nullptr;
  const float* mid_scale = nullptr;
  const float* mid_shift = nullptr;
  const float* pre_scale = nullptr;
  const float* pre_shift = nullptr;
  __nv_bfloat16* out_pre = nullptr;
  int pre_cs = 0, pre_co = 0;
  const __nv_bfloat16* res1 = nullptr;
  int res1_cs = 0, res1_co = 0;
  const __nv_bfloat16* res2 = nullptr;
  int res2_cs = 0, res2_co = 0;
  const __nv_bfloat16* res_up = nullptr;
  int up_cs = 0, up_co = 0;
  __nv_bfloat16* out_raw = nullptr;
  int raw_cs = 0, raw_co = 0;
  const float* post_scale = nullptr;
  const float* post_shift = nullptr;
  __nv_bfloat16* out_post = nullptr;
  int post_cs = 0, post_co = 0;
  int aux_mode = 0;
  const float* aux_scale = nullptr;
  const float* aux_shift = nullptr;
  __nv_bfloat16* out_aux1 = nullptr;
  int aux1_cs = 0, aux1_co = 0;
  __nv_bfloat16* out_aux2 = nullptr;
  int aux2_cs = 0, aux2_co = 0;
  bool pool2 = false;
  float* out_f32 = nullptr;
  unsigned long long* argmax_keys = nullptr;
  int cout_real = 0;
  int up_sy = 1, up_sx = 1, up_py = 0, up_px = 0;
};

struct ConvShape {
  const __nv_bfloat16* in = nullptr;
  int n = 0, h = 0, w = 0;
  int cin = 0;
  int in_cs = 0;
  const __nv_bfloat16* wpacked = nullptr;
  int cout_pad = 0;
  int n_tile = 0;
  int kh = 3, kw = 3;
  int y_off0 = -1, x_off0 = -1;
};

struct alignas(64) ConvParams {
  CUtensorMap tm_a;
  CUtensorMap tm_b;
  CUtensorMap tm_a2;
  CUtensorMap tm_b2;
  CUtensorMap tm_r1, tm_r2, tm_up;
  int tail;
  ConvShape s;
  ConvEpilogue e;
  int tiles_x, tiles_y, n_nt, total_tiles;
  int tile_h;
  int h_slot_bytes, n_hslots, n_wslots;
  int w_stationary;
  long long* prof;
  int debug_mode;
};

int conv_plan(const ConvShape& s, const ConvEpilogue& e, ConvParams* out);
int conv_launch(const ConvParams& p, cudaStream_t stream);
int pack_conv_weight(const float* w_oihw, int cout, int cin, int kh, int kw, int cout_pad, int cin_pad,
                     __nv_bfloat16* out, cudaStream_t stream);
constexpr int kConvTraceTiles = 64;
constexpr int kConvProfInts = 148 * 8 + kConvTraceTiles * 16;
void conv_set_profile_buffer(long long* dev_buf);
void conv_set_debug_mode(int mode);

}
```

### mvlm_b200/csrc/hourglass.cu

```cuda
#include "hourglass.cuh"

#include <math.h>
#include <stdlib.h>

#include <algorithm>

namespace mvlm {

namespace {

__global__ void fold_bn_kernel(const float* w, const float* b, const float* m, const float* v, float eps, int n,
                               float* scale, float* shift) {
  const int i = blockIdx.x * blockDim.x + threadIdx.x;
  if (i >= n) return;
  const float s = w[i] / sqrtf(v[i] + eps);
  scale[i] = s;
  shift[i] = b[i] - m[i] * s;
}

__global__ void pack_conv_weight_kernel(const float* __restrict__ w, int cout, int cin, int kh, int kw,
                                        int cout_pad, int cin_pad, __nv_bfloat16* __restrict__ out) {
  const long long total = 1ll * cout_pad * kw * kh * cin_pad;
  for (long long i = blockIdx.x * 1ll * blockDim.x + threadIdx.x; i < total;
       i += 1ll * gridDim.x * blockDim.x) {
// ... 124 lines not shown
  std::vector<Block> free_list;
  std::vector<size_t> live;
  size_t top = 0;
  auto release = [&](size_t id) {
    Block nb = {bufs_[id].offset, bufs_[id].bytes};
    size_t k = 0;
    while (k < free_list.size() && free_list[k].off < nb.off) ++k;
    free_list.insert(free_list.begin() + k, nb);
    for (size_t j = 0; j + 1 < free_list.size();) {
      if (free_list[j].off + free_list[j].bytes == free_list[j + 1].off) {
        free_list[j].bytes += free_list[j + 1].bytes;
        free_list.erase(free_list.begin() + j + 1);
      } else {
        ++j;
      }
    }
    if (!free_list.empty() && free_list.back().off + free_list.back().bytes == top) {
      top = free_list.back().off;
      free_list.pop_back();
    }
  };
  for (size_t id : order) {
    Buf& b = bufs_[id];
    for (size_t j = 0; j < live.size();) {
      if (bufs_[live[j]].last < b.first) {
        release(live[j]);
        live.erase(live.begin() + j);
      } else {
        ++j;
      }
    }
    size_t best = free_list.size();
    for (size_t j = 0; j < free_list.size(); ++j)
      if (free_list[j].bytes >= b.bytes && (best == free_list.size() || free_list[j].bytes < free_list[best].bytes)) best = j;
    if (best < free_list.size()) {
      b.offset = free_list[best].off;
      free_list[best].off += b.bytes;
      free_list[best].bytes -= b.bytes;
      if (free_list[best].bytes == 0) free_list.erase(free_list.begin() + best);
    } else {
      b.offset = top;
      top += b.bytes;
    }
    ws_needed_ = std::max(ws_needed_, b.offset + b.bytes);
    ws_needed_ = std::max(ws_needed_, top);
    live.push_back(id);
  }
}

HourglassNet::T HourglassNet::alloc(int h, int w, int c) {
  T t;
  t.h = h; t.w = w; t.c = c;
  t.p = static_cast<__nv_bfloat16*>(ws_alloc(static_cast<size_t>(V_) * h * w * c * sizeof(__nv_bfloat16)));
  return t;
}

int HourglassNet::param(const std::string& name, long long numel, size_t bytes, void** dst, const float** src) {
  const size_t aligned = (bytes + 255) & ~static_cast<size_t>(255);
  *dst = (layout_pass_ || params_ == nullptr || param_off_ + aligned > param_cap_) ? nullptr : params_ + param_off_;
  *src = nullptr;
  param_off_ += aligned;
  if (layout_pass_) return MVLM_OK;
  const int rc = sd_get(name, numel, src);
  if (rc) return rc;
  MVLM_REQUIRE(*dst, "hourglass: parameter arena exhausted (%s)", name.c_str());
  return MVLM_OK;
}

int HourglassNet::sd_get(const std::string& name, long long numel, const float** out) const {
  auto f = sd_->find(name);
  MVLM_REQUIRE(f != sd_->end(), "hourglass: missing state_dict key %s", name.c_str());
  MVLM_REQUIRE(f->second.p != nullptr, "hourglass: null tensor for state_dict key %s", name.c_str());
  MVLM_REQUIRE(f->second.numel < 0 || f->second.numel == numel,
               "hourglass: size mismatch for %s: the checkpoint has %lld elements, this model (%d landmarks, %d image "
               "channels) needs %lld", name.c_str(), f->second.numel, L_, cin_, numel);
  *out = f->second.p;
  return MVLM_OK;
}

int HourglassNet::bn(const std::string& name, int c, const float** scale, const float** shift) {
  auto it = bn_cache_.find(name);
  if (it == bn_cache_.end()) {
    void* buf;
    const float* src[4];
    int rc = param(name + ".weight", c, sizeof(float) * 2 * c, &buf, &src[0]);
    if (rc) return rc;
    float* f = static_cast<float*>(buf);
    if (!layout_pass_) {
      const char* suffix[3] = {".bias", ".running_mean", ".running_var"};
      for (int k = 0; k < 3; ++k)
        if ((rc = sd_get(name + suffix[k], c, &src[k + 1]))) return rc;
      fold_bn_kernel<<<ceil_div(c, 128), 128, 0, build_stream_>>>(src[0], src[1], src[2], src[3], 1e-5f, c, f, f + c);
      MVLM_CHECK_CUDA(cudaGetLastError());
    }
    it = bn_cache_.emplace(name, std::make_pair(f, f ? f + c : nullptr)).first;
  }
  *scale = it->second.first;
  *shift = it->second.second;
  return MVLM_OK;
}

int HourglassNet::packed(const std::string& name, int cout, int cin, int k, int cout_pad, int cin_pad,
                         const __nv_bfloat16** out) {
  void* buf;
  const float* src;
  const int rc = param(name, 1ll * cout * cin * k * k, sizeof(__nv_bfloat16) * cout_pad * k * k * cin_pad, &buf, &src);
  *out = static_cast<__nv_bfloat16*>(buf);
  if (rc || layout_pass_) return rc;
  return pack_conv_weight(src, cout, cin, k, k, cout_pad, cin_pad, static_cast<__nv_bfloat16*>(buf), build_stream_);
}

int HourglassNet::bias(const std::string& name, int cout, int cout_pad, const float** out) {
  void* buf;
  const float* src;
  const int rc = param(name, cout, sizeof(float) * cout_pad, &buf, &src);
  *out = static_cast<float*>(buf);
  if (rc || layout_pass_) return rc;
  pad_bias_kernel<<<ceil_div(cout_pad, 128), 128, 0, build_stream_>>>(src, cout, cout_pad, static_cast<float*>(buf));
  MVLM_CHECK_CUDA(cudaGetLastError());
  return MVLM_OK;
}

int HourglassNet::stem_weight(const __nv_bfloat16** out) {
  void* buf;
  const float* src;
  const int rc = param("conv1.weight", 64ll * cin_ * 9, sizeof(__nv_bfloat16) * 64 * 9 * 16, &buf, &src);
  *out = static_cast<__nv_bfloat16*>(buf);
  if (rc || layout_pass_) return rc;
  pack_stem_weight_kernel<<<36, 256, 0, build_stream_>>>(src, 64, cin_, 64, static_cast<__nv_bfloat16*>(buf));
  MVLM_CHECK_CUDA(cudaGetLastError());
  return MVLM_OK;
}

int HourglassNet::phase_weight(int a, int b, const __nv_bfloat16** out) {
  void* buf;
  const float* src;
  const int rc = param("conv11.weight", 9ll * L_ * L_, sizeof(__nv_bfloat16) * Lp_ * 4 * Lp_, &buf, &src);
  *out = static_cast<__nv_bfloat16*>(buf);
  if (rc || layout_pass_) return rc;
  pack_phase_weight_kernel<<<64, 256, 0, build_stream_>>>(src, L_, L_, a, b, Lp_, Lp_, static_cast<__nv_bfloat16*>(buf));
  MVLM_CHECK_CUDA(cudaGetLastError());
  return MVLM_OK;
}

int HourglassNet::emit_conv(const char* tag, T in, int cin, const __nv_bfloat16* w, int cout_pad, int n_tile, int kh,
                            int kw, int y_off0, int x_off0, const ConvEpilogue& e, double flops, bool is_head) {
  flops_ += flops;
  note_conv(in.p, e);
  NetOp op;
  op.kind = NetOp::CONV;
  op.tag = tag;
  op.is_head = is_head;
  op.h = in.h; op.w = in.w;
  if (!layout_pass_) {
    ConvShape s;
    s.in = in.p; s.n = V_; s.h = in.h; s.w = in.w; s.cin = cin; s.in_cs = in.c;
    s.wpacked = w; s.cout_pad = cout_pad; s.n_tile = n_tile; s.kh = kh; s.kw = kw;
    s.y_off0 = y_off0; s.x_off0 = x_off0;
    const int rc = conv_plan(s, e, &op.conv);
    if (rc) return rc;
  }
  ops_.push_back(op);
  return MVLM_OK;
}

int HourglassNet::rb(const std::string& p, T x, T a_in, T ar, int cin, int cout, const char* post_bn, T* post_act,
                     T* y_out, T* pool_raw, const T* up_low, const RbAux* aux) {
  const int h = a_in.h, w = a_in.w;
  T y = alloc(h, w, cout);
  T skip = x;
  int rc;
  if (cin != cout) {
    ConvEpilogue e;
    e.out_raw = y.p; e.raw_cs = cout; e.raw_co = 0;
    const __nv_bfloat16* wr;
    if ((rc = packed(p + ".resample.2.weight", cout, cin, 1, cout, cin, &wr)) ||
        (rc = emit_conv("rb.resample", ar, cin, wr, cout, cout < 128 ? cout : 128, 1, 1, 0, 0, e,
                        2.0 * cout * cin * ar.h * ar.w)))
      return rc;
    skip = y;
  }
  const float *ps = nullptr, *pt = nullptr;
  if (post_bn) {
    rc = bn(post_bn, cout, &ps, &pt);
    if (rc) return rc;
    *post_act = pool_raw ? alloc(h / 2, w / 2, cout) : alloc(h, w, cout);
  }
  if (pool_raw) *pool_raw = alloc(h / 2, w / 2, cout);
  const float *as = nullptr, *at = nullptr;
  if (aux) {
    rc = bn(aux->bn, cout, &as, &at);
    if (rc) return rc;
    *aux->out1 = aux->mode == 2 ? alloc(h / 2, w / 2, cout) : alloc(h, w, cout);
    if (aux->mode == 2) *aux->out2 = alloc(h / 2, w / 2, cout);
  }
  const int c1 = cout / 2, c2 = cout / 4;
  T a1 = alloc(h, w, c1);
  T a2 = alloc(h, w, c2);
  const int widths[3] = {c1, c2, c2};
  const int offs[3] = {0, c1, c1 + c2};
  const int cins[3] = {cin, c1, c2};
  const T ins[3] = {a_in, a1, a2};
  const T pres[3] = {a1, a2, T()};
  const char* pre_bn[3] = {".bn2", ".bn3", nullptr};
  const char* names[3] = {".conv1", ".conv2", ".conv3"};
  for (int i = 0; i < 3; ++i) {
    ConvEpilogue e;
    if (pre_bn[i]) {
      rc = bn(p + pre_bn[i], widths[i], &e.pre_scale, &e.pre_shift);
      if (rc) return rc;
      e.out_pre = pres[i].p; e.pre_cs = pres[i].c; e.pre_co = 0;
    }
    e.res1 = skip.p; e.res1_cs = skip.c; e.res1_co = offs[i];
    if (up_low) { e.res_up = up_low->p; e.up_cs = up_low->c; e.up_co = offs[i]; }
    e.out_raw = pool_raw ? pool_raw->p : y.p; e.raw_cs = cout; e.raw_co = offs[i];
    e.pool2 = pool_raw != nullptr;
    if (post_bn) {
      e.post_scale = layout_pass_ ? nullptr : ps + offs[i];
      e.post_shift = layout_pass_ ? nullptr : pt + offs[i];
      e.out_post = post_act->p; e.post_cs = cout; e.post_co = offs[i];
    }
    if (aux) {
      e.aux_mode = aux->mode;
      e.aux_scale = layout_pass_ ? nullptr : as + offs[i];
      e.aux_shift = layout_pass_ ? nullptr : at + offs[i];
      e.out_aux1 = aux->out1->p; e.aux1_cs = cout; e.aux1_co = offs[i];
      if (aux->mode == 2) { e.out_aux2 = aux->out2->p; e.aux2_cs = cout; e.aux2_co = offs[i]; }
    }
    const int nt = widths[i] < 128 ? widths[i] : 128;
    const __nv_bfloat16* wc;
    if ((rc = packed(p + names[i] + ".weight", widths[i], cins[i], 3, widths[i], cins[i], &wc)) ||
        (rc = emit_conv("rb.conv", ins[i], cins[i], wc, widths[i], nt, 3, 3, -1, -1, e,
                        2.0 * widths[i] * cins[i] * 9 * h * w)))
      return rc;
  }
  *y_out = y;
  return MVLM_OK;
}

int HourglassNet::emit_pool(T in, T out_raw, const char* bn_name, T out_act) {
  note_use(in.p); note_use(out_raw.p); note_use(out_act.p);
  NetOp op;
  op.kind = NetOp::POOL;
  op.in0 = in.p; op.out_raw = out_raw.p; op.out_act = out_act.p;
  op.h = in.h; op.w = in.w; op.c = in.c;
  if (bn_name) {
    int rc = bn(bn_name, in.c, &op.scale, &op.shift);
    if (rc) return rc;
  }
  ops_.push_back(op);
  return MVLM_OK;
}

int HourglassNet::hourglass(const std::string& p, T x, T a_x, T* out, const T* in_pooled, const T* in_pooled_act) {
  const int F = 256;
  int rc;
  T none;
  T lows[5], a_lows[5];
  T cur = x;
  const int low_blocks[5] = {2, 4, 6, 8, 10};
  const int skip_blocks[4] = {3, 5, 7, 9};
  T pooled, a;
  if (in_pooled) {
    pooled = *in_pooled;
    a = *in_pooled_act;
  }
  for (int lvl = 0; lvl < 5; ++lvl) {
    const std::string lb = p + ".rb" + std::to_string(low_blocks[lvl]);
    if (!(fuse_elt_ && (lvl > 0 || in_pooled))) {
      pooled = alloc(cur.h / 2, cur.w / 2, F);
      a = alloc(cur.h / 2, cur.w / 2, F);
      rc = emit_pool(cur, pooled, (lb + ".bn1").c_str(), a);
      if (rc) return rc;
    }
    const int nxt = lvl < 4 ? skip_blocks[lvl] : 11;
    const std::string post = p + ".rb" + std::to_string(nxt) + ".bn1";
    T next_pooled, next_a;
    const std::string next_bn = lvl < 4 ? p + ".rb" + std::to_string(low_blocks[lvl + 1]) + ".bn1" : "";
    RbAux aux = {2, next_bn.c_str(), &next_pooled, &next_a};
    rc = rb(lb, pooled, a, none, F, F, post.c_str(), &a_lows[lvl], &lows[lvl], nullptr, nullptr,
            (fuse_elt_ && lvl < 4) ? &aux : nullptr);
    if (rc) return rc;
    cur = lows[lvl];
    pooled = next_pooled;
    a = next_a;
  }
  T low2, a2, low3;
  rc = rb(p + ".rb11", cur, a_lows[4], none, F, F, (p + ".rb12.bn1").c_str(), &a2, &low2);
  if (rc) return rc;
  rc = rb(p + ".rb12", low2, a2, none, F, F, nullptr, nullptr, &low3);
  if (rc) return rc;
  cur = low3;
  const int ups[4][2] = {{13, 14}, {15, 16}, {17, 18}, {19, 20}};
  for (int lvl = 0; lvl < 4; ++lvl) {
    const std::string sb = p + ".rb" + std::to_string(skip_blocks[3 - lvl]);
    const std::string b1 = p + ".rb" + std::to_string(ups[lvl][0]);
    const std::string b2 = p + ".rb" + std::to_string(ups[lvl][1]);
    T s, a;
    rc = rb(sb, lows[3 - lvl], a_lows[3 - lvl], none, F, F, (b1 + ".bn1").c_str(), &a, &s, nullptr, &cur);
    if (rc) return rc;
    T l1, a1, l2;
    rc = rb(b1, s, a, none, F, F, (b2 + ".bn1").c_str(), &a1, &l1);
    if (rc) return rc;
    rc = rb(b2, l1, a1, none, F, F, nullptr, nullptr, &l2);
    if (rc) return rc;
    cur = l2;
  }
  T add5;
  rc = rb(p + ".rb1", x, a_x, none, F, F, nullptr, nullptr, &add5, nullptr, &cur);
  if (rc) return rc;
  *out = add5;
  return MVLM_OK;
}

int HourglassNet::build(const StateDict* sd, int n_landmarks, int cin, int n_views, int h,
                        int w, void* workspace, size_t workspace_bytes, bool dry) {
  MVLM_REQUIRE(n_landmarks > 0 && n_landmarks <= 128, "hourglass: n_landmarks=%d unsupported", n_landmarks);
  MVLM_REQUIRE(cin >= 1 && cin <= 4, "hourglass: image channels=%d unsupported", cin);
  MVLM_REQUIRE(n_views > 0 && h >= 64 && w >= 64 && h % 64 == 0 && w % 64 == 0,
               "hourglass: image size %dx%d must be a positive multiple of 64", h, w);
  MVLM_REQUIRE(dry || (sd && workspace), "hourglass: null state_dict/workspace");
  sd_ = sd;
  V_ = n_views; H_ = h; W_ = w; L_ = n_landmarks; cin_ = cin;
  Lp_ = pad_to(L_, 16);
  if (Lp_ == 112) Lp_ = 128;
  if (Lp_ == 48) Lp_ = 64;
  if (Lp_ == 16) Lp_ = 32;
  ws_ = static_cast<uint8_t*>(workspace); ws_size_ = workspace_bytes;
  keep_probes_ = getenv("MVLM_HG_KEEP_PROBES") != nullptr && atoi(getenv("MVLM_HG_KEEP_PROBES")) != 0;
  reuse_ = !(getenv("MVLM_HG_NO_REUSE") != nullptr && atoi(getenv("MVLM_HG_NO_REUSE")) != 0);
  fuse_elt_ = !(getenv("MVLM_HG_ELT_FUSION") != nullptr && atoi(getenv("MVLM_HG_ELT_FUSION")) == 0);
  bufs_.clear(); fake_off_ = 0; ws_needed_ = 0; next_buf_ = 0;
  layout_pass_ = true;
  int rc = emit();
  layout_pass_ = false;
  if (rc) return rc;
  assign_offsets();
  if (dry) return MVLM_OK;
  MVLM_REQUIRE(ws_needed_ <= ws_size_, "hourglass: workspace too small (%zu needed, %zu given)", ws_needed_, ws_size_);
  const size_t param_bytes = param_off_ + 4096;
  MVLM_CHECK_CUDA(cudaMalloc(&params_, param_bytes));
  owned_.push_back(params_);
  param_cap_ = param_bytes;
  MVLM_CHECK_CUDA(cudaStreamCreateWithFlags(&build_stream_, cudaStreamNonBlocking));
  rc = emit();
  if (rc == MVLM_OK && param_off_ > param_bytes) {
    set_error("hourglass: parameter arena overrun (%zu of %zu bytes)", param_off_, param_bytes);
    rc = MVLM_E_INVALID;
  }
  const cudaError_t ce = cudaStreamSynchronize(build_stream_);
  cudaStreamDestroy(build_stream_);
  build_stream_ = nullptr;
  if (rc) return rc;
  MVLM_CHECK_CUDA(ce);
  return MVLM_OK;
}

void HourglassNet::probe(const char* name, const T& t) {
  probes[name] = {t.p, t.h, t.w, t.c};
  if (layout_pass_ && keep_probes_ && t.p) {
    const size_t off = static_cast<size_t>(reinterpret_cast<const uint8_t*>(t.p) - kFakeBase);
    for (Buf& b : bufs_)
      if (b.fake_off == off) b.pinned = true;
  }
}

int HourglassNet::emit() {
  const int h = H_, w = W_, cin = cin_;
  ops_.clear(); flops_ = 0.0; probes.clear();
  param_off_ = 0; bn_cache_.clear();
  int rc;
  const int F = 256, h2 = h / 2, w2 = w / 2;

  T a_c2 = alloc(h, w, 64), ar_c2 = alloc(h, w, 64);
  T img16 = alloc(h, w, 16);
  {
    note_use(img16.p);
    NetOp op;
    op.kind = NetOp::STEM;
    op.out_raw = img16.p; op.h = h; op.w = w; op.c = cin;
    ops_.push_back(op);
    const __nv_bfloat16* w1;
    ConvEpilogue e;
    if ((rc = stem_weight(&w1))) return rc;
    if ((rc = bias("conv1.bias", 64, 64, &e.bias))) return rc;
    if ((rc = bn("bn1", 64, &e.mid_scale, &e.mid_shift))) return rc;
    if ((rc = bn("conv2.bn1", 64, &e.pre_scale, &e.pre_shift))) return rc;
    if ((rc = bn("conv2.resample.0", 64, &e.post_scale, &e.post_shift))) return rc;
    e.out_pre = a_c2.p; e.pre_cs = 64; e.pre_co = 0;
    e.out_post = ar_c2.p; e.post_cs = 64; e.post_co = 0;
    if ((rc = emit_conv("conv1", img16, 16, w1, 64, 64, 3, 3, -1, -1, e, 2.0 * 64 * cin * 9 * h * w))) return rc;
  }
  T none, y2, y3, r3, a3, a4, a_h1, ar4;
  T x1;
  if ((rc = rb("conv2", none, a_c2, ar_c2, 64, 128, "conv3.bn1", &a3, &y2, &x1))) return rc;
  probe("x1", x1);
  if (fuse_elt_) {
    RbAux aux = {1, "conv4.resample.0", &ar4, nullptr};
    if ((rc = rb("conv3", x1, a3, none, 128, 128, "conv4.bn1", &a4, &y3, nullptr, nullptr, &aux))) return rc;
    probe("y3", y3);
  } else {
    if ((rc = rb("conv3", x1, a3, none, 128, 128, "conv4.bn1", &a4, &y3))) return rc;
    probe("y3", y3);
    ar4 = alloc(h2, w2, 128);
    note_use(y3.p); note_use(ar4.p);
    NetOp op;
    op.kind = NetOp::BNRELU;
    op.in0 = y3.p; op.out_act = ar4.p; op.h = h2; op.w = w2; op.c = 128;
    if ((rc = bn("conv4.resample.0", 128, &op.scale, &op.shift))) return rc;
    ops_.push_back(op);
  }
  T p1, pa1, p2, pa2;
  RbAux aux4 = {2, "hg1.rb2.bn1", &p1, &pa1};
  if ((rc = rb("conv4", y3, a4, ar4, 128, F, "hg1.rb1.bn1", &a_h1, &r3, nullptr, nullptr, fuse_elt_ ? &aux4 : nullptr))) return rc;
  probe("r3", r3);
  T hg1;
  if ((rc = hourglass("hg1", r3, a_h1, &hg1, fuse_elt_ ? &p1 : nullptr, fuse_elt_ ? &pa1 : nullptr))) return rc;
  probe("hg1", hg1);
  T ll1 = alloc(h2, w2, F);
  {
    ConvEpilogue e;
    const __nv_bfloat16* w5;
    if ((rc = bn("bn2", F, &e.pre_scale, &e.pre_shift))) return rc;
    e.out_pre = ll1.p; e.pre_cs = F; e.pre_co = 0;
    if ((rc = packed("conv5.weight", F, F, 3, F, F, &w5)) || (rc = bias("conv5.bias", F, F, &e.bias)) ||
        (rc = emit_conv("conv5", hg1, F, w5, F, 128, 3, 3, -1, -1, e, 2.0 * F * F * 9 * h2 * w2)))
      return rc;
  }
  T x6 = alloc(h2, w2, Lp_);
  {
    ConvEpilogue e;
    const __nv_bfloat16* w6;
    e.out_raw = x6.p; e.raw_cs = Lp_; e.raw_co = 0;
    if ((rc = packed("conv6.weight", L_, F, 3, Lp_, F, &w6)) || (rc = bias("conv6.bias", L_, Lp_, &e.bias)) ||
        (rc = emit_conv("conv6", ll1, F, w6, Lp_, Lp_, 3, 3, -1, -1, e, 2.0 * L_ * F * 9 * h2 * w2)))
      return rc;
  }
  T sum = alloc(h2, w2, F), a_h2;
  {
    ConvEpilogue e;
    e.res1 = r3.p; e.res1_cs = F; e.res1_co = 0;
    e.res2 = ll1.p; e.res2_cs = F; e.res2_co = 0;
    e.out_raw = sum.p; e.raw_cs = F; e.raw_co = 0;
    a_h2 = alloc(h2, w2, F);
    if ((rc = bn("hg2.rb1.bn1", F, &e.post_scale, &e.post_shift))) return rc;
    e.out_post = a_h2.p; e.post_cs = F; e.post_co = 0;
    if (fuse_elt_) {
      p2 = alloc(h2 / 2, w2 / 2, F);
      pa2 = alloc(h2 / 2, w2 / 2, F);
      if ((rc = bn("hg2.rb2.bn1", F, &e.aux_scale, &e.aux_shift))) return rc;
      e.aux_mode = 2;
      e.out_aux1 = p2.p; e.aux1_cs = F; e.aux1_co = 0;
      e.out_aux2 = pa2.p; e.aux2_cs = F; e.aux2_co = 0;
    }
    const __nv_bfloat16* w7;
    if ((rc = packed("conv7.weight", F, L_, 3, F, Lp_, &w7)) || (rc = bias("conv7.bias", F, F, &e.bias)) ||
        (rc = emit_conv("conv7", x6, Lp_, w7, F, 128, 3, 3, -1, -1, e, 2.0 * F * L_ * 9 * h2 * w2)))
      return rc;
  }
  probe("sum_temp", sum);
  T hg2;
  if ((rc = hourglass("hg2", sum, a_h2, &hg2, fuse_elt_ ? &p2 : nullptr, fuse_elt_ ? &pa2 : nullptr))) return rc;
  T ll2 = alloc(h2, w2, F);
  {
    ConvEpilogue e;
    const __nv_bfloat16* w9;
    if ((rc = bn("bn3", F, &e.pre_scale, &e.pre_shift))) return rc;
    e.out_pre = ll2.p; e.pre_cs = F; e.pre_co = 0;
    if ((rc = packed("conv9.weight", F, F, 3, F, F, &w9)) || (rc = bias("conv9.bias", F, F, &e.bias)) ||
        (rc = emit_conv("conv9", hg2, F, w9, F, 128, 3, 3, -1, -1, e, 2.0 * F * F * 9 * h2 * w2)))
      return rc;
  }
  T x10 = alloc(h2, w2, Lp_);
  {
    ConvEpilogue e;
    const __nv_bfloat16* w10;
    e.out_raw = x10.p; e.raw_cs = Lp_; e.raw_co = 0;
    if ((rc = packed("conv10.weight", L_, F, 3, Lp_, F, &w10)) || (rc = bias("conv10.bias", L_, Lp_, &e.bias)) ||
        (rc = emit_conv("conv10", ll2, F, w10, Lp_, Lp_, 3, 3, -1, -1, e, 2.0 * L_ * F * 9 * h2 * w2)))
      return rc;
  }
  probe("x10", x10);
  keys_ = static_cast<unsigned long long*>(ws_alloc(sizeof(unsigned long long) * V_ * L_));
  {
    note_use(keys_);
    NetOp op;
    op.kind = NetOp::MEMSET;
    op.bytes = sizeof(unsigned long long) * V_ * L_;
    ops_.push_back(op);
  }
  if ((rc = bias("conv11.bias", L_, Lp_, &b11_))) return rc;
  x10_ = x10.p;
  for (int a = 0; a < 2; ++a) {
    for (int b = 0; b < 2; ++b) {
      ConvEpilogue e;
      e.bias = b11_;
      e.argmax_keys = keys_;
      e.cout_real = L_;
      e.up_sy = 2; e.up_sx = 2; e.up_py = a; e.up_px = b;
      if ((rc = phase_weight(a, b, &phase_w_[2 * a + b])) ||
          (rc = emit_conv("conv11.phase", x10, Lp_, phase_w_[2 * a + b], Lp_, Lp_, 2, 2, a - 1, b - 1, e,
                          2.0 * L_ * L_ * 9 * h2 * w2, true)))
        return rc;
    }
  }
  {
    note_use(keys_);
    note_use(x10.p);
    NetOp op;
    op.kind = NetOp::PEAKS;
    ops_.push_back(op);
  }
  return MVLM_OK;
}

int HourglassNet::run_op(NetOp& op, const unsigned char* img_u8, const float* img_f32, float* out_heatmaps,
                         float* out_peaks, cudaStream_t stream) {
  unsigned long long* const keys = out_keys_ ? out_keys_ : keys_;
  switch (op.kind) {
    case NetOp::STEM:
      return image_to_hilo16(img_u8, img_f32, op.c, static_cast<size_t>(V_) * op.h * op.w, op.out_raw, stream);
    case NetOp::CONV:
      if (op.is_head) {
        ConvParams p = op.conv;
        p.e.out_f32 = out_heatmaps;
        p.e.argmax_keys = keys;
        return conv_launch(p, stream);
      }
      return conv_launch(op.conv, stream);
    case NetOp::POOL:
      return pool2_act(op.in0, V_, op.h, op.w, op.c, op.out_raw, op.scale, op.shift, op.out_act, stream);
    case NetOp::BNRELU:
      return bn_relu(op.in0, static_cast<size_t>(V_) * op.h * op.w, op.c, op.scale, op.shift, op.out_act, stream);
    case NetOp::MEMSET:
      MVLM_CHECK_CUDA(cudaMemsetAsync(keys, 0, op.bytes, stream));
      return MVLM_OK;
    case NetOp::PEAKS:
      if (out_peaks && !out_keys_) {
        if (peak_method_ == 1)
          return peaks_moment_from_keys(keys_, x10_, Lp_, Lp_, phase_w_, b11_, V_, L_, H_, W_, out_peaks, stream);
        return peaks_from_keys(keys_, V_, L_, H_, W_, out_peaks, stream);
      }
      return MVLM_OK;
  }
  return MVLM_OK;
}

int HourglassNet::set_selection_method(int method) {
  MVLM_REQUIRE(method == 0 || method == 1, "hourglass: unknown selection method %d", method);
  if (method != peak_method_) {
    for (auto& g : graphs_) cudaGraphExecDestroy(g.second);
    graphs_.clear();
    peak_method_ = method;
  }
  return MVLM_OK;
}

int HourglassNet::forward_keys(const unsigned char* img_u8, const float* img_f32, unsigned long long* out_keys,
                               cudaStream_t stream) {
  MVLM_REQUIRE(out_keys, "hourglass: null key buffer");
  out_keys_ = out_keys;
  const int rc = forward_graph(img_u8, img_f32, nullptr, reinterpret_cast<float*>(out_keys), stream);
  out_keys_ = nullptr;
  return rc;
}

int HourglassNet::forward(const unsigned char* img_u8, const float* img_f32, float* out_heatmaps, float* out_peaks,
                          cudaStream_t stream) {
  MVLM_REQUIRE(params_, "hourglass: forward on a dry plan");
  MVLM_REQUIRE(out_peaks || out_heatmaps, "hourglass: no output requested");
  for (NetOp& op : ops_) {
    const int rc = run_op(op, img_u8, img_f32, out_heatmaps, out_peaks, stream);
    if (rc != MVLM_OK) return rc;
  }
  return MVLM_OK;
}

int HourglassNet::profile_ops(const unsigned char* img_u8, const float* img_f32, float* out_peaks, int reps,
                              float* ms_out, double* roles_out, int trace_op, long long* trace_out,
                              cudaStream_t stream) {
  MVLM_REQUIRE(params_ && out_peaks && ms_out && reps > 0, "hourglass: bad profile_ops arguments");
  const size_t n = ops_.size();
  std::vector<cudaEvent_t> ev(n + 1);
  for (auto& e : ev) MVLM_CHECK_CUDA(cudaEventCreate(&e));
  for (size_t i = 0; i < n; ++i) ms_out[i] = 0.f;
  int rc = forward(img_u8, img_f32, nullptr, out_peaks, stream);
  for (int r = 0; r < reps && rc == MVLM_OK; ++r) {
    MVLM_CHECK_CUDA(cudaEventRecord(ev[0], stream));
    for (size_t i = 0; i < n && rc == MVLM_OK; ++i) {
      rc = run_op(ops_[i], img_u8, img_f32, nullptr, out_peaks, stream);
      MVLM_CHECK_CUDA(cudaEventRecord(ev[i + 1], stream));
    }
    MVLM_CHECK_CUDA(cudaStreamSynchronize(stream));
    for (size_t i = 0; i < n; ++i) {
      float ms = 0.f;
      MVLM_CHECK_CUDA(cudaEventElapsedTime(&ms, ev[i], ev[i + 1]));
      ms_out[i] += ms / reps;
    }
  }
  for (auto& e : ev) cudaEventDestroy(e);
  if (roles_out && rc == MVLM_OK) {
    long long* dev = nullptr;
    MVLM_CHECK_CUDA(cudaMalloc(&dev, sizeof(long long) * kConvProfInts));
    std::vector<long long> host(kConvProfInts);
    for (size_t i = 0; i < n && rc == MVLM_OK; ++i) {
      for (int k = 0; k < 8; ++k) roles_out[i * 8 + k] = 0.0;
      if (ops_[i].kind == NetOp::CONV) {
        MVLM_CHECK_CUDA(cudaMemsetAsync(dev, 0, sizeof(long long) * kConvProfInts, stream));
        conv_set_profile_buffer(dev);
      }
      rc = run_op(ops_[i], img_u8, img_f32, nullptr, out_peaks, stream);
      conv_set_profile_buffer(nullptr);
      if (ops_[i].kind == NetOp::CONV && rc == MVLM_OK) {
        MVLM_CHECK_CUDA(cudaStreamSynchronize(stream));
        MVLM_CHECK_CUDA(cudaMemcpy(host.data(), dev, sizeof(long long) * kConvProfInts, cudaMemcpyDeviceToHost));
        if (trace_out && static_cast<int>(i) == trace_op)
          for (int k = 0; k < kConvTraceTiles * 16; ++k) trace_out[k] = host[kNumSMs * 8 + k];
        int ctas = 0;
        for (int c = 0; c < kNumSMs; ++c) {
          if (host[c * 8 + 4] == 0) continue;
          ++ctas;
          for (int k = 0; k < 8; ++k) roles_out[i * 8 + k] += static_cast<double>(host[c * 8 + k]);
        }
        for (int k = 0; k < 8; ++k) roles_out[i * 8 + k] /= ctas > 0 ? ctas : 1;
      }
    }
    cudaFree(dev);
  }
  return rc;
}

std::string HourglassNet::describe_op(int i) const {
  if (i < 0 || i >= static_cast<int>(ops_.size())) return "";
  const NetOp& op = ops_[i];
  char buf[256];
  switch (op.kind) {
    case NetOp::CONV: {
      const ConvShape& s = op.conv.s;
      const ConvEpilogue& e = op.conv.e;
      snprintf(buf, sizeof(buf), "conv %s %dx%d %d->%d k%d%s%s%s%s%s%s%s%s", op.tag, s.h, s.w, s.cin, s.cout_pad, s.kh,
               e.out_pre ? " pre" : "", e.res1 ? " res1" : "", e.res2 ? " res2" : "", e.res_up ? " up" : "", e.out_raw ? " raw" : "",
               e.out_post ? " post" : "", e.pool2 ? " pool" : (e.aux_mode == 2 ? " +pooled" : (e.aux_mode == 1 ? " +act2" : "")),
               e.argmax_keys ? " argmax" : "");
      break;
    }
    case NetOp::POOL: snprintf(buf, sizeof(buf), "pool %dx%dx%d", op.h, op.w, op.c); break;
    case NetOp::BNRELU: snprintf(buf, sizeof(buf), "bnrelu %dx%dx%d", op.h, op.w, op.c); break;
    case NetOp::STEM: snprintf(buf, sizeof(buf), "stem-stage %dx%dx%d", op.h, op.w, op.c); break;
    case NetOp::MEMSET: snprintf(buf, sizeof(buf), "memset %zu", op.bytes); break;
    case NetOp::PEAKS: snprintf(buf, sizeof(buf), "peaks"); break;
  }
  return buf;
}

int HourglassNet::forward_graph(const unsigned char* img_u8, const float* img_f32, float* out_heatmaps,
                                float* out_peaks, cudaStream_t stream) {
  for (auto& g : graphs_) {
    if (g.first.a == img_u8 && g.first.b == img_f32 && g.first.c == out_heatmaps && g.first.d == out_peaks) {
      MVLM_CHECK_CUDA(cudaGraphLaunch(g.second, stream));
      count_launch(static_cast<int>(ops_.size()));
      return MVLM_OK;
    }
  }
  int rc = forward(img_u8, img_f32, out_heatmaps, out_peaks, stream);
  if (rc != MVLM_OK) return rc;
  if (graphs_.size() >= kMaxGraphs) {
    cudaGraphExecDestroy(graphs_.front().second);
    graphs_.erase(graphs_.begin());
  }
  cudaGraph_t graph = nullptr;
  if (cudaStreamBeginCapture(stream, cudaStreamCaptureModeThreadLocal) != cudaSuccess) {
    cudaGetLastError();
    return MVLM_OK;
  }
  rc = forward(img_u8, img_f32, out_heatmaps, out_peaks, stream);
  const cudaError_t ce = cudaStreamEndCapture(stream, &graph);
  if (rc != MVLM_OK || ce != cudaSuccess || !graph) {
    cudaGetLastError();
    if (graph) cudaGraphDestroy(graph);
    return rc;
  }
  cudaGraphExec_t exec = nullptr;
  if (cudaGraphInstantiate(&exec, graph, 0) == cudaSuccess && exec) {
    graphs_.push_back({GraphKey{img_u8, img_f32, out_heatmaps, out_peaks}, exec});
    MVLM_CHECK_CUDA(cudaGraphLaunch(exec, stream));
  } else {
    cudaGetLastError();
    rc = forward(img_u8, img_f32, out_heatmaps, out_peaks, stream);
  }
  cudaGraphDestroy(graph);
  return rc;
}

}
```

### mvlm_b200/csrc/hourglass.cuh

```cuda
#pragma once
#include <map>
#include <string>
#include <vector>

#include "conv_umma.cuh"
#include "stages.cuh"

namespace mvlm {

struct SdEntry {
  const float* p = nullptr;
  long long numel = -1;
};
typedef std::map<std::string, SdEntry> StateDict;

struct NetOp {
  enum Kind { CONV, POOL, BNRELU, STEM, MEMSET, PEAKS } kind;
  ConvParams conv;
  const __nv_bfloat16* in0 = nullptr;
  __nv_bfloat16* out_raw = nullptr;
  __nv_bfloat16* out_act = nullptr;
  const float* scale = nullptr;
  const float* shift = nullptr;
  int h = 0, w = 0, c = 0;
  size_t bytes = 0;
  bool is_head = false;
  const char* tag = "";
};

class HourglassNet {
 public:
  HourglassNet() = default;
  ~HourglassNet();
  int build(const StateDict* sd, int n_landmarks, int cin, int n_views, int h, int w,
            void* workspace, size_t workspace_bytes, bool dry);
  int forward(const unsigned char* img_u8, const float* img_f32, float* out_heatmaps, float* out_peaks,
              cudaStream_t stream);
  int run_op(NetOp& op, const unsigned char* img_u8, const float* img_f32, float* out_heatmaps, float* out_peaks,
             cudaStream_t stream);
  int forward_graph(const unsigned char* img_u8, const float* img_f32, float* out_heatmaps, float* out_peaks,
                    cudaStream_t stream);

  int set_selection_method(int method);
  int forward_keys(const unsigned char* img_u8, const float* img_f32, unsigned long long* out_keys, cudaStream_t stream);

  int profile_ops(const unsigned char* img_u8, const float* img_f32, float* out_peaks, int reps, float* ms_out,
                  double* roles_out, int trace_op, long long* trace_out, cudaStream_t stream);
  std::string describe_op(int i) const;

  size_t workspace_needed() const { return ws_needed_; }
  int n_views() const { return V_; }
  int n_landmarks() const { return L_; }
  int height() const { return H_; }
  int width() const { return W_; }
  double flops_per_view() const { return flops_; }
  int n_ops() const { return static_cast<int>(ops_.size()); }
  const std::vector<NetOp>& ops() const { return ops_; }
  struct Probe { const __nv_bfloat16* p; int h, w, c; };
  std::map<std::string, Probe> probes;

 private:
  struct T { __nv_bfloat16* p = nullptr; int h = 0, w = 0, c = 0; };
  T alloc(int h, int w, int c);
  void* ws_alloc(size_t bytes);
  struct Buf {
    size_t bytes = 0, fake_off = 0, offset = 0;
    int first = -1, last = -1;
    bool pinned = false;
  };
  int emit();
  void note_use(const void* p);
  void note_conv(const void* in, const ConvEpilogue& e);
  void assign_offsets();
  void probe(const char* name, const T& t);
  int param(const std::string& name, long long numel, size_t bytes, void** dst, const float** src);
  unsigned char* params_ = nullptr;
  size_t param_off_ = 0, param_cap_ = 0;
  cudaStream_t build_stream_ = nullptr;
  static constexpr size_t kMaxGraphs = 8;
  std::vector<Buf> bufs_;
  size_t fake_off_ = 0, ws_needed_ = 0, next_buf_ = 0;
  bool layout_pass_ = false, keep_probes_ = false, reuse_ = true, fuse_elt_ = false;
  int bn(const std::string& name, int c, const float** scale, const float** shift);
  int packed(const std::string& name, int cout, int cin, int k, int cout_pad, int cin_pad, const __nv_bfloat16** out);
  int bias(const std::string& name, int cout, int cout_pad, const float** out);
  int stem_weight(const __nv_bfloat16** out);
  int phase_weight(int a, int b, const __nv_bfloat16** out);
  int emit_conv(const char* tag, T in, int cin, const __nv_bfloat16* w, int cout_pad, int n_tile, int kh, int kw,
                int y_off0, int x_off0, const ConvEpilogue& e, double flops, bool is_head = false);
  struct RbAux { int mode; const char* bn; T* out1; T* out2; };
  int rb(const std::string& p, T x, T a_in, T ar, int cin, int cout, const char* post_bn, T* post_act, T* y_out,
         T* pool_raw = nullptr, const T* up_low = nullptr, const RbAux* aux = nullptr);
  int hourglass(const std::string& p, T x, T a_x, T* out, const T* in_pooled = nullptr, const T* in_pooled_act = nullptr);
  int emit_pool(T in, T out_raw, const char* bn_name, T out_act);

  const StateDict* sd_ = nullptr;
  int sd_get(const std::string& name, long long numel, const float** out) const;
  int V_ = 0, H_ = 0, W_ = 0, L_ = 0, Lp_ = 0, cin_ = 0;
  uint8_t* ws_ = nullptr;
  size_t ws_size_ = 0;
  std::vector<void*> owned_;
  std::map<std::string, std::pair<float*, float*>> bn_cache_;
  std::vector<NetOp> ops_;
  unsigned long long* keys_ = nullptr;
  unsigned long long* out_keys_ = nullptr;
  int peak_method_ = 0;
  const __nv_bfloat16* phase_w_[4] = {nullptr, nullptr, nullptr, nullptr};
  const float* b11_ = nullptr;
  const __nv_bfloat16* x10_ = nullptr;
  double flops_ = 0.0;
  struct GraphKey { const void* a; const void* b; const void* c; const void* d; };
  std::vector<std::pair<GraphKey, cudaGraphExec_t>> graphs_;
};

}
```

### mvlm_b200/ops.py

```python
from __future__ import annotations

import contextlib
import ctypes as C

import os
from typing import NamedTuple

import torch

from . import _lib
from ._lib import ConvArgs, check, cur_stream, ptr


def pack_conv_weight(w_oihw: torch.Tensor, cout_pad: int, cin_pad: int) -> torch.Tensor:
    lib = _lib.load()
    w = w_oihw.contiguous().float()
    cout, cin, kh, kw = w.shape
    out = torch.empty((cout_pad, kw, kh, cin_pad), dtype=torch.bfloat16, device=w.device)
    check(lib.mvlm_pack_conv_weight(ptr(w), cout, cin, kh, kw, cout_pad, cin_pad, ptr(out), cur_stream()),
          "mvlm_pack_conv_weight")
    return out


def conv2d_bf16(x: torch.Tensor, wpacked: torch.Tensor, *, cin: int | None = None, n_tile: int,
                kh: int = 3, kw: int = 3, y_off0: int | None = None, x_off0: int | None = None,
                bias=None, mid=None, pre=None, res1=None, res2=None, out_raw=None, post=None,
                out_f32=None, argmax_keys=None, cout_real: int | None = None,
                up=(1, 1, 0, 0), pool2: bool = False, res_up=None) -> None:
    lib = _lib.load()
    n, h, w, cs = x.shape
    a = ConvArgs()
    a.in_ = ptr(x)
    a.n, a.h, a.w, a.cin, a.in_cs = n, h, w, (cin if cin is not None else cs), cs
    a.wpacked = ptr(wpacked)
    a.cout_pad = wpacked.shape[0]
    a.n_tile, a.kh, a.kw = n_tile, kh, kw
    a.y_off0 = -(kh // 2) if y_off0 is None else y_off0
    a.x_off0 = -(kw // 2) if x_off0 is None else x_off0
    a.bias = ptr(bias)
    if mid is not None:
        a.mid_scale, a.mid_shift = ptr(mid[0]), ptr(mid[1])
    if pre is not None:
        a.pre_scale, a.pre_shift, a.out_pre = ptr(pre[0]), ptr(pre[1]), ptr(pre[2])
        a.pre_cs, a.pre_co = pre[2].shape[-1], pre[3]
    if res1 is not None:
        a.res1, a.res1_cs, a.res1_co = ptr(res1[0]), res1[0].shape[-1], res1[1]
    if res2 is not None:
        a.res2, a.res2_cs, a.res2_co = ptr(res2[0]), res2[0].shape[-1], res2[1]
    if out_raw is not None:
        a.out_raw, a.raw_cs, a.raw_co = ptr(out_raw[0]), out_raw[0].shape[-1], out_raw[1]
    if post is not None:
        a.post_scale, a.post_shift, a.out_post = ptr(post[0]), ptr(post[1]), ptr(post[2])
        a.post_cs, a.post_co = post[2].shape[-1], post[3]
    a.out_f32 = ptr(out_f32)
    a.argmax_keys = ptr(argmax_keys)
    a.cout_real = cout_real if cout_real is not None else wpacked.shape[0]
    a.up_sy, a.up_sx, a.up_py, a.up_px = up
    a.pool2 = 1 if pool2 else 0
    if res_up is not None:
        a.res_up, a.up_cs, a.up_co = ptr(res_up[0]), res_up[0].shape[-1], res_up[1]
    check(lib.mvlm_conv2d_bf16(C.byref(a), cur_stream()), "mvlm_conv2d_bf16")


CHANNEL_MODES = {"RGB+depth": 0, "geometry+depth": 1, "RGB": 2, "depth": 3, "geometry": 4}
MODE_CHANNELS = {0: 4, 1: 2, 2: 3, 3: 1, 4: 1}


def raster_workspace(n_views: int, h: int, w: int, n_verts: int, device) -> torch.Tensor:
    n = _lib.load().mvlm_raster_workspace_bytes(n_views, h, w, n_verts)
    return torch.empty(((n + 7) // 8,), dtype=torch.int64, device=device)


def raster_multiview(verts, uvs, tris, tex, rot, h: int, w: int, channel_mode: str = "RGB+depth",
                     want_f32: bool = False, want_tri: bool = False, want_z: bool = False, zbuf=None, out_u8=None):
    lib = _lib.load()
    dev = verts.device
    mode = CHANNEL_MODES[channel_mode]
    v = rot.shape[0]
    need = lib.mvlm_raster_workspace_bytes(v, h, w, verts.shape[0])
    if zbuf is None or zbuf.numel() * zbuf.element_size() < need:
        zbuf = raster_workspace(v, h, w, verts.shape[0], dev)
    if out_u8 is None:
        out_u8 = torch.empty((v, h, w, 4), dtype=torch.uint8, device=dev)
    f32 = torch.empty((v, h, w, MODE_CHANNELS[mode]), dtype=torch.float32, device=dev) if want_f32 else None
    tri = torch.empty((v, h, w), dtype=torch.int32, device=dev) if want_tri else None
    z = torch.empty((v, h, w), dtype=torch.float32, device=dev) if want_z else None
    th, tw, tc = (tex.shape[0], tex.shape[1], tex.shape[2]) if tex is not None else (0, 0, 3)
    check(lib.mvlm_raster_multiview(ptr(verts), verts.shape[0], ptr(uvs), ptr(tris), tris.shape[0], ptr(tex), th, tw, tc,
                                    ptr(rot), v, h, w, mode, ptr(zbuf), zbuf.numel() * zbuf.element_size(), ptr(out_u8),
                                    ptr(f32), ptr(tri), ptr(z), cur_stream()),
          "mvlm_raster_multiview")
    return {"u8": out_u8, "f32": f32, "tri": tri, "z": z}


class RasterInput(NamedTuple):
    verts: torch.Tensor
    uvs: torch.Tensor | None
    tris: torch.Tensor
    tex: torch.Tensor | None
    colors: torch.Tensor | None = None
    pages: torch.Tensor | None = None


def raster_multiscan(scans, rot, h: int, w: int, channel_mode: str = "RGB+depth", want_f32: bool = False,
                     want_tri: bool = False, want_z: bool = False, zbuf=None, out_u8=None):
    lib = _lib.load()
    n = len(scans)
    if not 1 <= n <= _lib.MAX_SCANS:
        raise ValueError(f"1 to {_lib.MAX_SCANS} scans per pass (got {n})")
    total = rot.shape[0]
    if total % n:
        raise ValueError(f"{total} views do not split evenly over {n} scans")
    v = total // n
    dev = scans[0][0].device
    mode = CHANNEL_MODES[channel_mode]
    table = (_lib.RasterScan * n)()
    rgba = (C.c_void_p * n)()
    paged = (C.c_void_p * n)()
    for i, (e, scan) in enumerate(zip(table, scans)):
        try:
            s = RasterInput(*scan)
        except TypeError:
            raise ValueError("a scan is (verts, uvs, tris, tex[, colors[, pages]])") from None
        if s.colors is not None and (s.colors.dtype != torch.uint8 or tuple(s.colors.shape) != (s.verts.shape[0], 4)):
            raise ValueError(f"vertex colours must be ({s.verts.shape[0]}, 4) uint8 RGBA")
        if s.pages is not None and (s.pages.dtype != torch.int32 or s.pages.dim() != 1
                                    or s.pages.numel() < s.tris.shape[0] or (s.pages.numel() - s.tris.shape[0]) % 3
                                    or s.tex is None or s.tex.shape[-1] != 4):
            raise ValueError("pages must be an int32 (Nt + 3P,) table with an RGBA texel buffer as tex")
        e.verts, e.n_verts, e.uvs = ptr(s.verts), s.verts.shape[0], ptr(s.uvs)
        e.tris, e.n_tris = ptr(s.tris), s.tris.shape[0]
        e.tex, (e.tex_h, e.tex_w, e.tex_channels) = ptr(s.tex), (s.tex.shape[:3] if s.tex is not None else (0, 0, 3))
        rgba[i], paged[i] = ptr(s.colors), ptr(s.pages)
    need = lib.mvlm_raster_multiscan_workspace_bytes(n, v, h, w, max(s[0].shape[0] for s in scans))
    if zbuf is None or zbuf.numel() * zbuf.element_size() < need:
        zbuf = torch.empty(((need + 7) // 8,), dtype=torch.int64, device=dev)
    if out_u8 is None:
        out_u8 = torch.empty((total, h, w, 4), dtype=torch.uint8, device=dev)
    f32 = torch.empty((total, h, w, MODE_CHANNELS[mode]), dtype=torch.float32, device=dev) if want_f32 else None
    tri = torch.empty((total, h, w), dtype=torch.int32, device=dev) if want_tri else None
    z = torch.empty((total, h, w), dtype=torch.float32, device=dev) if want_z else None
    check(lib.mvlm_raster_multiscan_paged(table, rgba, paged, n, ptr(rot), v, h, w, mode, ptr(zbuf),
                                          zbuf.numel() * zbuf.element_size(), ptr(out_u8), ptr(f32), ptr(tri), ptr(z),
                                          cur_stream()), "mvlm_raster_multiscan_paged")
    return {"u8": out_u8, "f32": f32, "tri": tri, "z": z}


def _on_device(device):
    device = torch.device(device)
    return torch.cuda.device(device) if device.type == "cuda" else contextlib.nullcontext()


@contextlib.contextmanager
def _plan_env(**kv):
    old = {k: os.environ.get(k) for k in kv}
    os.environ.update(kv)
    try:
        yield
    finally:
        for k, v in old.items():
            if v is None:
                os.environ.pop(k, None)
            else:
                os.environ[k] = v


class Hourglass:

    def __init__(self, state_dict: dict, n_landmarks: int, cin: int, n_views: int, h: int, w: int, device="cuda",
                 keep_probes: bool = False):
        lib = _lib.load()
        self.n_landmarks, self.cin, self.n_views, self.h, self.w = n_landmarks, cin, n_views, h, w
        self.device = torch.device(device)
        self.keep_probes = bool(keep_probes)
        with _on_device(self.device), _plan_env(MVLM_HG_KEEP_PROBES="1" if keep_probes else "0"):
            self._create(lib, state_dict, n_landmarks, cin, n_views, h, w)

    def _create(self, lib, state_dict, n_landmarks, cin, n_views, h, w):
        self._sd = {k: v.detach().to(self.device, torch.float32).contiguous() for k, v in state_dict.items()
                    if v.is_floating_point()}
        nbytes = lib.mvlm_hourglass_workspace_bytes(n_landmarks, cin, n_views, h, w)
        if nbytes == 0:
            raise _lib.MvlmError("mvlm_hourglass_workspace_bytes: " + lib.mvlm_last_error().decode())
        self.workspace = torch.empty((nbytes,), dtype=torch.uint8, device=self.device)
        names = list(self._sd.keys())
        arr_n = (C.c_char_p * len(names))(*[n.encode() for n in names])
        arr_p = (C.c_void_p * len(names))(*[self._sd[n].data_ptr() for n in names])
        arr_k = (C.c_longlong * len(names))(*[self._sd[n].numel() for n in names])
        handle = C.c_void_p()
        if self.device.type == "cuda":
            torch.cuda.current_stream(self.device).synchronize()
        check(lib.mvlm_hourglass_create(arr_n, arr_p, arr_k, len(names), n_landmarks, cin, n_views, h, w,
                                        self.workspace.data_ptr(), nbytes, C.byref(handle)), "mvlm_hourglass_create")
        self._h = handle
        self.flops_per_view = lib.mvlm_hourglass_flops_per_view(n_landmarks, cin, h, w)
        self.num_launches = lib.mvlm_hourglass_num_launches(handle)

    def forward(self, img, want_heatmaps: bool = False, want_peaks: bool = True, graph: bool = False,
                selection_method: str = "simple"):
        with _on_device(self.device):
            check(_lib.load().mvlm_hourglass_set_selection_method(self._h, {"simple": 0, "moment": 1}[selection_method]),
                  "mvlm_hourglass_set_selection_method")
            return self._forward(img, want_heatmaps, want_peaks, graph)

    def _forward(self, img, want_heatmaps: bool = False, want_peaks: bool = True, graph: bool = False):
        lib = _lib.load()
        assert img.shape[0] == self.n_views and img.shape[1] == self.h and img.shape[2] == self.w
        u8 = img if img.dtype == torch.uint8 else None
        f32 = img.contiguous() if img.dtype == torch.float32 else None
        if u8 is None and f32 is None:
            raise TypeError("img must be uint8 (V,H,W,4) or float32 (V,H,W,cin)")
# ... 189 lines not shown
```

Baseline: 62.44.

## Add 16-warp epilogue variant with setmaxnreg for large 1x1 raw-output convs

Adds a wide conv kernel form with 640 threads and 16 epilogue warps, used for 1x1 non-head convs at high resolution whose epilogue only writes raw output. Producer warps drop registers via setmaxnreg so the epilogue warps get more, and the operand smem pool shrinks to make room for the extra staging buffers. The goal is to cut epilogue drain time (TMEM to global) that bounds these memory-heavy 1x1 layers. In exchange the smaller pool can mean fewer operand ring slots, and register pressure per epilogue thread is tighter.

```diff
diff --git a/include/mvlm_b200.h b/include/mvlm_b200.h
--- a/include/mvlm_b200.h
+++ b/include/mvlm_b200.h
@@ -46,6 +46,7 @@
   int pool2;
   const void* res_up;
   int up_cs, up_co;
+  int epi_wide;
 } mvlm_conv_args;
 
 int mvlm_conv2d_bf16(const mvlm_conv_args* args, void* stream);
@@ -153,6 +154,7 @@
 typedef struct mvlm_hourglass mvlm_hourglass;
 size_t mvlm_hourglass_workspace_bytes(int n_landmarks, int cin, int n_views, int h, int w);
 double mvlm_hourglass_flops_per_view(int n_landmarks, int cin, int h, int w);
+int mvlm_hourglass_wide_ops(int n_landmarks, int cin, int n_views, int h, int w, int* ops, int cap);
 int mvlm_hourglass_create(const char* const* names, const void* const* ptrs, const long long* numels,
                           int n_entries, int n_landmarks, int cin, int n_views, int h, int w, void* workspace,
                           size_t workspace_bytes, mvlm_hourglass** out);
diff --git a/mvlm_b200/_lib.py b/mvlm_b200/_lib.py
--- a/mvlm_b200/_lib.py
+++ b/mvlm_b200/_lib.py
@@ -33,6 +33,7 @@
         ("mid_scale", C.c_void_p), ("mid_shift", C.c_void_p),
         ("pool2", C.c_int),
         ("res_up", C.c_void_p), ("up_cs", C.c_int), ("up_co", C.c_int),
+        ("epi_wide", C.c_int),
     ]
 
 
@@ -102,6 +103,7 @@
                                          i32, vp, C.c_size_t, vp, vp, vp, vp, vp], i32),
         "mvlm_hourglass_workspace_bytes": ([i32, i32, i32, i32, i32], C.c_size_t),
         "mvlm_hourglass_flops_per_view": ([i32, i32, i32, i32], f64),
+        "mvlm_hourglass_wide_ops": ([i32, i32, i32, i32, i32, C.POINTER(i32), i32], i32),
         "mvlm_hourglass_create": ([C.POINTER(C.c_char_p), C.POINTER(vp), C.POINTER(C.c_longlong), i32, i32, i32, i32,
                                    i32, i32, vp, C.c_size_t, C.POINTER(vp)], i32),
         "mvlm_hourglass_forward": ([vp, vp, vp, vp, vp, vp], i32),
diff --git a/mvlm_b200/csrc/api.cu b/mvlm_b200/csrc/api.cu
--- a/mvlm_b200/csrc/api.cu
+++ b/mvlm_b200/csrc/api.cu
@@ -77,7 +77,7 @@
   e.up_sy = a->up_sy > 0 ? a->up_sy : 1; e.up_sx = a->up_sx > 0 ? a->up_sx : 1;
   e.up_py = a->up_py; e.up_px = a->up_px;
   ConvParams p;
-  int rc = conv_plan(s, e, &p);
+  int rc = conv_plan(s, e, a->epi_wide != 0, &p);
   if (rc != MVLM_OK) return rc;
   return conv_launch(p, static_cast<cudaStream_t>(stream));
 }
@@ -166,6 +166,18 @@
   return dry.flops_per_view();
 }
 
+int mvlm_hourglass_wide_ops(int n_landmarks, int cin, int n_views, int h, int w, int* ops, int cap) {
+  HourglassNet dry;
+  if (dry.build(nullptr, n_landmarks, cin, n_views, h, w, nullptr, 0, true) != MVLM_OK) return -1;
+  int n = 0;
+  for (int i = 0; i < dry.n_ops(); ++i) {
+    if (!dry.ops()[i].epi_wide) continue;
+    if (ops && n < cap) ops[n] = i;
+    ++n;
+  }
+  return n;
+}
+
 int mvlm_hourglass_create(const char* const* names, const void* const* ptrs, const long long* numels, int n_entries,
                           int n_landmarks, int cin, int n_views, int h, int w, void* workspace, size_t workspace_bytes,
                           mvlm_hourglass** out) {
diff --git a/mvlm_b200/csrc/conv_epilogue.cuh b/mvlm_b200/csrc/conv_epilogue.cuh
--- a/mvlm_b200/csrc/conv_epilogue.cuh
+++ b/mvlm_b200/csrc/conv_epilogue.cuh
@@ -6,8 +6,6 @@
 namespace mvlm {
 namespace epi {
 
-constexpr int kThreads = 352;
-constexpr int kEpiWarps = 8;
 constexpr int kTileW = 8;
 constexpr int kMaxTileH = 32;
 constexpr int kMTile = 128;
@@ -21,8 +19,19 @@
               F_M64 = 1024 ,
               F_POST2 = 2048 ,
               F_POOLX = 4096 ,
-              F_STAT = 8192  };
+              F_STAT = 8192 ,
+              F_EPI16 = 16384  };
 constexpr int F_HEAD = F_F32 | F_ARGMAX;
+
+constexpr int epi_warps(int f) { return (f & F_EPI16) ? 16 : 8; }
+constexpr int first_epi_warp(int f) { return (f & F_EPI16) ? 4 : 2; }
+constexpr int weight_warp(int f) { return (f & F_EPI16) ? 2 : 10; }
+constexpr int cta_threads(int f) { return (f & F_EPI16) ? 640 : 352; }
+constexpr int kWideLaunchRegs = 96;
+constexpr int kWideProducerRegs = 64;
+constexpr int kWideEpiRegs = 104;
+static_assert(128 * kWideProducerRegs + 512 * kWideEpiRegs <= 640 * kWideLaunchRegs, "setmaxnreg split exceeds the pool");
+constexpr bool epi_wide_supported(int f) { return (f & ~(F_M64 | F_STAT | F_EPI16)) == F_RAW; }
 
 inline int feature_mask(const ConvEpilogue& e) {
   return (e.out_pre ? F_PRE : 0) | (e.res1 ? F_RES1 : 0) | (e.res2 ? F_RES2 : 0) | (e.out_raw ? F_RAW : 0) |
@@ -148,12 +157,13 @@
   constexpr int kUnitRows = kCols / 8;
   static_assert(kCols * kPitch <= kStageFloats, "transpose buffer");
   const int rep_log2 = !WS ? 0 : (s.cout_pad <= 32 ? 2 : 1);
+  constexpr int kShareLog2 = (F & F_EPI16) ? 2 : 1;
   const int n_cgrp = 4 >> rep_log2;
   const int cgrp = lane_grp & (n_cgrp - 1);
   const int replica = lane_grp >> (2 - rep_log2);
   const int n_units = max(1, tile_h / kUnitRows);
   const int upr = max(1, n_units >> rep_log2);
-  const int upw = max(1, upr >> 1);
+  const int upw = max(1, upr >> kShareLog2);
   const int u_local = (ew >> 2) * upw;
   const int u_begin = replica * upr + u_local;
   const int oh = s.h * e.up_sy, ow = s.w * e.up_sx;
@@ -168,7 +178,7 @@
   const uint32_t rs_aux1 = static_cast<uint32_t>(((F & F_POOLX) ? (s.w >> 1) : s.w) * e.aux1_cs) * 2u;
   const uint32_t rs_aux2 = static_cast<uint32_t>((s.w >> 1) * e.aux2_cs) * 2u;
   constexpr bool kHasRes = (F & (F_RES1 | F_RES2 | F_UP)) != 0;
-  constexpr int kMaxUpw = WS ? 4 : 8;
+  constexpr int kMaxUpw = (WS ? 8 : 16) >> kShareLog2;
   constexpr int kResRegs = 4 * (2 * (((F & F_RES1) ? 1 : 0) + ((F & F_RES2) ? 1 : 0)) + ((F & F_UP) ? 1 : 0));
   constexpr int kResBudget = 64;
   constexpr int kPref = !kHasRes ? 1 : (kResRegs * kMaxUpw <= kResBudget ? kMaxUpw : (kResRegs * kMaxUpw <= 2 * kResBudget ? kMaxUpw / 2 : (kMaxUpw >= 4 ? kMaxUpw / 4 : 1)));
diff --git a/mvlm_b200/csrc/conv_umma.cu b/mvlm_b200/csrc/conv_umma.cu
--- a/mvlm_b200/csrc/conv_umma.cu
+++ b/mvlm_b200/csrc/conv_umma.cu
@@ -12,6 +12,8 @@
 constexpr int kMaxHSlots = 4;
 constexpr int kMaxWSlots = 12;
 constexpr int kPoolBytes = 198 * 1024;
+constexpr int kPoolBytesWide = 182 * 1024;
+constexpr int pool_bytes(bool epi_wide) { return epi_wide ? kPoolBytesWide : kPoolBytes; }
 
 struct __align__(8) Barriers {
   uint64_t h_full[kMaxHSlots];
@@ -34,9 +36,11 @@
   float post_t[kMaxCout];
 };
 
-constexpr int kSmemBytes = kPoolBytes + kEpiWarps * kStageFloats * 4 + 512 + static_cast<int>(sizeof(EpiParams)) +
-                           1024 ;
-static_assert(kSmemBytes <= 227 * 1024, "shared memory budget");
+constexpr int smem_bytes(int f) {
+  return pool_bytes((f & F_EPI16) != 0) + epi_warps(f) * kStageFloats * 4 + 512 + static_cast<int>(sizeof(EpiParams)) +
+         1024 ;
+}
+static_assert(smem_bytes(0) <= 227 * 1024 && smem_bytes(F_EPI16) <= 227 * 1024, "shared memory budget");
 
 __device__ __forceinline__ TileCoord decode_tile(const ConvParams& p, int t) {
   TileCoord c;
@@ -69,14 +73,17 @@
 };
 
 template <int F>
-__global__ void __launch_bounds__(kThreads, 1) conv_umma_kernel(const __grid_constant__ ConvParams p) {
+__global__ void __launch_bounds__(cta_threads(F), 1) conv_umma_kernel(const __grid_constant__ ConvParams p) {
   constexpr bool ARGMAX = (F & F_ARGMAX) != 0;
+  constexpr bool WIDE = (F & F_EPI16) != 0;
+  constexpr int kThreads = cta_threads(F), kEpiWarps = epi_warps(F), kEpi0 = first_epi_warp(F);
+  static_assert(!WIDE || epi_wide_supported(F), "no 16-warp epilogue for this feature set");
   extern __shared__ uint8_t smem_raw[];
   const uint32_t raw_addr = ptx::smem_u32(smem_raw);
   uint8_t* smem = smem_raw + ((1024u - (raw_addr & 1023u)) & 1023u);
   uint8_t* h_slots = smem;
   uint8_t* w_slots = smem + p.n_hslots * p.h_slot_bytes;
-  float* stage_all = reinterpret_cast<float*>(smem + kPoolBytes);
+  float* stage_all = reinterpret_cast<float*>(smem + pool_bytes(WIDE));
   Barriers* bar = reinterpret_cast<Barriers*>(reinterpret_cast<uint8_t*>(stage_all) + kEpiWarps * kStageFloats * 4);
   EpiParams* ep = reinterpret_cast<EpiParams*>(reinterpret_cast<uint8_t*>(bar) + 512);
 
@@ -158,193 +165,197 @@
     if (trace && trace_i < kTraceTiles) trace[trace_i * 16 + (slot)] = clock64() - t_kernel0; \
   } while (0)
 
-  if (warp == 0) {
-    if (ptx::elect_one() && (p.debug_mode & 1) == 0) {
-      int sh = 0;
-      uint32_t ph = 0;
-      TileIter it(p, t_begin, t_step);
-      for (int t = t_begin; t < t_end; t += t_step, it.next()) {
-        const TileCoord tc = it.c;
-        const int x0 = tc.tx * kTileW + s.x_off0;
-        const int y0 = tc.ty * p.tile_h + s.y_off0;
-        for (int c = 0; c < n_chunks; ++c) {
-          const bool is_tail = p.tail != 0 && c == n_chunks - 1;
-          const uint32_t row_b = is_tail ? static_cast<uint32_t>(p.tail) * 2u : 128u;
-          timed_wait(&bar->h_empty[sh], ph ^ 1, prof, w0);
-          ptx::mbar_expect_tx(&bar->h_full[sh], static_cast<uint32_t>(halo_rows * halo_px) * row_b);
-          ptx::tma_load_4d(is_tail ? &p.tm_a2 : &p.tm_a, &bar->h_full[sh], h_slots + sh * p.h_slot_bytes, c * 64, x0, y0, tc.img);
-          if (c == 0) MVLM_TRACE(0);
-          if (++sh == n_hslots) { sh = 0; ph ^= 1; }
+  if (warp < kEpi0 || warp == weight_warp(F)) {
+    if constexpr (WIDE) asm volatile("setmaxnreg.dec.sync.aligned.u32 %0;" ::"n"(kWideProducerRegs));
+    if (warp == 0) {
+      if (ptx::elect_one() && (p.debug_mode & 1) == 0) {
+        int sh = 0;
+        uint32_t ph = 0;
+        TileIter it(p, t_begin, t_step);
+        for (int t = t_begin; t < t_end; t += t_step, it.next()) {
+          const TileCoord tc = it.c;
+          const int x0 = tc.tx * kTileW + s.x_off0;
+          const int y0 = tc.ty * p.tile_h + s.y_off0;
+          for (int c = 0; c < n_chunks; ++c) {
+            const bool is_tail = p.tail != 0 && c == n_chunks - 1;
+            const uint32_t row_b = is_tail ? static_cast<uint32_t>(p.tail) * 2u : 128u;
+            timed_wait(&bar->h_empty[sh], ph ^ 1, prof, w0);
+            ptx::mbar_expect_tx(&bar->h_full[sh], static_cast<uint32_t>(halo_rows * halo_px) * row_b);
+            ptx::tma_load_4d(is_tail ? &p.tm_a2 : &p.tm_a, &bar->h_full[sh], h_slots + sh * p.h_slot_bytes, c * 64, x0, y0, tc.img);
+            if (c == 0) MVLM_TRACE(0);
+            if (++sh == n_hslots) { sh = 0; ph ^= 1; }
+          }
+          if constexpr ((F & (F_RES1 | F_RES2 | F_UP)) != 0) {
+            const int xa = tc.tx * kTileW, ya = tc.ty * p.tile_h, c_lo = tc.mt * kM;
+            if (F & F_RES1) ptx::tma_prefetch_l2_4d(&p.tm_r1, c_lo, xa, ya, tc.img);
+            if (F & F_RES2) ptx::tma_prefetch_l2_4d(&p.tm_r2, c_lo, xa, ya, tc.img);
+            if (F & F_UP) ptx::tma_prefetch_l2_4d(&p.tm_up, c_lo, xa >> 1, ya >> 1, tc.img);
+          }
+          ++trace_i;
         }
-        if constexpr ((F & (F_RES1 | F_RES2 | F_UP)) != 0) {
-          const int xa = tc.tx * kTileW, ya = tc.ty * p.tile_h, c_lo = tc.mt * kM;
-          if (F & F_RES1) ptx::tma_prefetch_l2_4d(&p.tm_r1, c_lo, xa, ya, tc.img);
-          if (F & F_RES2) ptx::tma_prefetch_l2_4d(&p.tm_r2, c_lo, xa, ya, tc.img);
-          if (F & F_UP) ptx::tma_prefetch_l2_4d(&p.tm_up, c_lo, xa >> 1, ya >> 1, tc.img);
-        }
-        ++trace_i;
+        if (prof) { p.prof[blockIdx.x * 8 + 0] = w0; p.prof[blockIdx.x * 8 + 7] = clock64() - t_kernel0; }
       }
-      if (prof) { p.prof[blockIdx.x * 8 + 0] = w0; p.prof[blockIdx.x * 8 + 7] = clock64() - t_kernel0; }
-    }
-  } else if (warp == 10) {
-    if (ptx::elect_one() && (p.debug_mode & 1) == 0) {
-      int sw = 0;
-      uint32_t pw = 0;
-      for (int t = t_begin; t < t_end; t += t_step) {
-        const int mt = t % p.n_nt;
-        for (int c = 0; c < n_chunks; ++c) {
-          const bool is_tail = p.tail != 0 && c == n_chunks - 1;
-          const void* tmb = is_tail ? &p.tm_b2 : &p.tm_b;
-          const uint32_t row_b = is_tail ? static_cast<uint32_t>(p.tail) * 2u : 128u;
-          const uint32_t wb = static_cast<uint32_t>(w_rows) * row_b;
-          if constexpr (M64) {
-            for (int kx = 0; kx < s.kw; ++kx) {
+    } else if (warp == weight_warp(F)) {
+      if (ptx::elect_one() && (p.debug_mode & 1) == 0) {
+        int sw = 0;
+        uint32_t pw = 0;
+        for (int t = t_begin; t < t_end; t += t_step) {
+          const int mt = t % p.n_nt;
+          for (int c = 0; c < n_chunks; ++c) {
+            const bool is_tail = p.tail != 0 && c == n_chunks - 1;
+            const void* tmb = is_tail ? &p.tm_b2 : &p.tm_b;
+            const uint32_t row_b = is_tail ? static_cast<uint32_t>(p.tail) * 2u : 128u;
+            const uint32_t wb = static_cast<uint32_t>(w_rows) * row_b;
+            if constexpr (M64) {
+              for (int kx = 0; kx < s.kw; ++kx) {
+                if (!w_stat) timed_wait(&bar->w_empty[sw], pw ^ 1, prof, w1);
+                ptx::mbar_expect_tx(&bar->w_full[sw], wb * static_cast<uint32_t>(s.kh));
+                for (int ky = 0; ky < s.kh; ++ky)
+                  ptx::tma_load_2d(tmb, &bar->w_full[sw], w_slots + sw * w_slot_bytes + ky * w_tap_bytes,
+                                   (kx * s.kh + ky) * s.cin + c * 64, mt * kM);
+                if (++sw == n_wslots) { sw = 0; pw ^= 1; }
+              }
+            } else
+            for (int tap = 0; tap < s.kw * s.kh; ++tap) {
               if (!w_stat) timed_wait(&bar->w_empty[sw], pw ^ 1, prof, w1);
-              ptx::mbar_expect_tx(&bar->w_full[sw], wb * static_cast<uint32_t>(s.kh));
-              for (int ky = 0; ky < s.kh; ++ky)
-                ptx::tma_load_2d(tmb, &bar->w_full[sw], w_slots + sw * w_slot_bytes + ky * w_tap_bytes,
-                                 (kx * s.kh + ky) * s.cin + c * 64, mt * kM);
-              if (++sw == n_wslots) { sw = 0; pw ^= 1; }
-            }
-          } else
-          for (int tap = 0; tap < s.kw * s.kh; ++tap) {
-            if (!w_stat) timed_wait(&bar->w_empty[sw], pw ^ 1, prof, w1);
-            ptx::mbar_expect_tx(&bar->w_full[sw], wb);
-            ptx::tma_load_2d(tmb, &bar->w_full[sw], w_slots + sw * w_slot_bytes, tap * s.cin + c * 64, mt * kM);
-            if (++sw == n_wslots) { sw = 0; pw ^= 1; }
-          }
-        }
-        MVLM_TRACE(1);
-        ++trace_i;
-        if (w_stat) break;
-      }
-      if (prof) p.prof[blockIdx.x * 8 + 1] = w1;
-    }
-  } else if (warp == 1) {
-    if (ptx::elect_one()) {
-      const uint32_t idesc = ptx::umma_idesc_bf16(mma_m, p.tile_h * kTileW);
-      const bool live = (p.debug_mode & 1) == 0;
-      const int n_kx = s.kw, n_ky = s.kh;
-      const uint32_t tail_row_b = p.tail ? static_cast<uint32_t>(p.tail) * 2u : 128u;
-      const uint32_t tail_swz = !p.tail ? 2u : (p.tail == 16 ? 6u : 4u);
-      const uint64_t a_hi_full = static_cast<uint64_t>(((8u * 128u) >> 4) | (1u << 14) | (2u << 29)) << 32;
-      const uint64_t b_hi_full = static_cast<uint64_t>(((static_cast<uint32_t>(halo_px) * 128u) >> 4) | (1u << 14) | (2u << 29)) << 32;
-      const uint64_t a_hi_tail = static_cast<uint64_t>(((8u * tail_row_b) >> 4) | (1u << 14) | (tail_swz << 29)) << 32;
-      const uint64_t b_hi_tail = static_cast<uint64_t>(((static_cast<uint32_t>(halo_px) * tail_row_b) >> 4) | (1u << 14) | (tail_swz << 29)) << 32;
-      const uint32_t h_lo0 = (ptx::smem_u32(h_slots) >> 4) | (1u << 16), h_step = static_cast<uint32_t>(p.h_slot_bytes) >> 4;
-      const uint32_t w_lo0 = (ptx::smem_u32(w_slots) >> 4) | (1u << 16), w_step = w_slot_bytes >> 4;
-      const int last_chunk = n_chunks - 1;
-      const int nk_last = (s.cin - last_chunk * 64) >= 64 ? 4 : ((s.cin - last_chunk * 64) >> 4);
-      int sh = 0, sw = 0;
-      uint32_t ph = 0, pw = 0;
-      int acc = 0;
-      uint32_t pacc = 0;
-      bool w_wait = live;
-      for (int t = t_begin; t < t_end; t += t_step) {
-        timed_wait(&bar->t_empty[acc], pacc ^ 1, prof, w1);
-        ptx::tc_fence_after();
-        MVLM_TRACE(2);
-        const uint32_t d = tmem_base + static_cast<uint32_t>(acc * 256);
-        uint32_t accumulate = 0;
-        for (int c = 0; c < n_chunks; ++c) {
-          const bool is_tail = p.tail != 0 && c == last_chunk;
-          const int nk = c == last_chunk ? nk_last : 4;
-          const uint32_t rb16 = (is_tail ? tail_row_b : 128u) >> 4;
-          const uint64_t a_hi = is_tail ? a_hi_tail : a_hi_full;
-          const uint64_t b_hi = is_tail ? b_hi_tail : b_hi_full;
-          const uint32_t ky_step = static_cast<uint32_t>(halo_px) * rb16;
-          if (live) timed_wait(&bar->h_full[sh], ph, prof, w0);
-          if (c == 0) MVLM_TRACE(3);
-          uint32_t x_col = h_lo0 + static_cast<uint32_t>(sh) * h_step;
-          if (STAT && !w_wait && (nk == 4 || nk == 2 || nk == 1)) {
-            auto taps = [&](auto nk_c, auto kk_c) __attribute__((always_inline)) {
-              constexpr int NK = decltype(nk_c)::value;
-              constexpr int KK = decltype(kk_c)::value;
-              constexpr uint32_t kRb16 = NK * 2;
-              const uint32_t tap16 = M64 ? (64u * 128u >> 4) : w_step;
-              const uint32_t w_base = w_lo0 + static_cast<uint32_t>(c * KK * KK) * tap16;
-#pragma unroll
-              for (int tap = 0; tap < KK * KK; ++tap) {
-                const uint32_t x_lo = x_col + static_cast<uint32_t>(((tap % KK) * (kTileW + KK - 1) + tap / KK)) * kRb16;
-                const uint32_t w_lo = w_base + static_cast<uint32_t>(tap) * tap16;
-#pragma unroll
-                for (int k = 0; k < NK; ++k) {
-                  const uint32_t en = (tap == 0 && k == 0) ? accumulate : 1u;
-                  if constexpr (M64) ptx::umma_ws_bf16(d, a_hi | (w_lo + 2 * k), b_hi | (x_lo + 2 * k), idesc, en);
-                  else ptx::umma_bf16(d, a_hi | (w_lo + 2 * k), b_hi | (x_lo + 2 * k), idesc, en);
-                }
-              }
-              accumulate = 1;
-            };
-            using std::integral_constant;
-            if constexpr (M64) {
-              if (nk == 4) taps(integral_constant<int, 4>(), integral_constant<int, 3>());
-              else if (nk == 2) taps(integral_constant<int, 2>(), integral_constant<int, 3>());
-              else taps(integral_constant<int, 1>(), integral_constant<int, 3>());
-            } else {
-              if (nk == 4) taps(integral_constant<int, 4>(), integral_constant<int, 2>());
-              else if (nk == 2) taps(integral_constant<int, 2>(), integral_constant<int, 2>());
-              else taps(integral_constant<int, 1>(), integral_constant<int, 2>());
-            }
-          } else if constexpr (M64) {
-            for (int kx = 0; kx < n_kx; ++kx, x_col += rb16) {
-              if (w_wait) timed_wait(&bar->w_full[sw], w_stat ? 0u : pw, prof, w0);
-              uint32_t x_lo = x_col;
-              uint32_t w_lo = w_lo0 + static_cast<uint32_t>(sw) * w_step;
-              for (int ky = 0; ky < n_ky; ++ky, x_lo += ky_step, w_lo += (w_tap_bytes >> 4)) {
-                ptx::umma_ws_bf16(d, a_hi | w_lo, b_hi | x_lo, idesc, accumulate);
-                if (nk == 4) {
-                  ptx::umma_ws_bf16(d, a_hi | (w_lo + 2), b_hi | (x_lo + 2), idesc, 1u);
-                  ptx::umma_ws_bf16(d, a_hi | (w_lo + 4), b_hi | (x_lo + 4), idesc, 1u);
-                  ptx::umma_ws_bf16(d, a_hi | (w_lo + 6), b_hi | (x_lo + 6), idesc, 1u);
-                } else {
-                  for (int k = 1; k < nk; ++k) ptx::umma_ws_bf16(d, a_hi | (w_lo + 2 * k), b_hi | (x_lo + 2 * k), idesc, 1u);
-                }
-                accumulate = 1;
-              }
-              if (live && !w_stat) ptx::umma_commit(&bar->w_empty[sw]);
-              if (++sw == n_wslots) { sw = 0; pw ^= 1; }
-            }
-          } else
-          for (int kx = 0; kx < n_kx; ++kx, x_col += rb16) {
-            uint32_t x_lo = x_col;
-            for (int ky = 0; ky < n_ky; ++ky, x_lo += ky_step) {
-              if (w_wait) timed_wait(&bar->w_full[sw], w_stat ? 0u : pw, prof, w0);
-              const uint32_t w_lo = w_lo0 + static_cast<uint32_t>(sw) * w_step;
-              auto mma = [&](int k, uint32_t en) __attribute__((always_inline)) {
-                if constexpr (M64) ptx::umma_ws_bf16(d, a_hi | (w_lo + 2 * k), b_hi | (x_lo + 2 * k), idesc, en);
-                else ptx::umma_bf16(d, a_hi | (w_lo + 2 * k), b_hi | (x_lo + 2 * k), idesc, en);
-              };
-              mma(0, accumulate);
-              if (nk == 4) {
-                mma(1, 1u); mma(2, 1u); mma(3, 1u);
-              } else {
-                for (int k = 1; k < nk; ++k) mma(k, 1u);
-              }
-              accumulate = 1;
-              if (live && !w_stat) ptx::umma_commit(&bar->w_empty[sw]);
+              ptx::mbar_expect_tx(&bar->w_full[sw], wb);
+              ptx::tma_load_2d(tmb, &bar->w_full[sw], w_slots + sw * w_slot_bytes, tap * s.cin + c * 64, mt * kM);
               if (++sw == n_wslots) { sw = 0; pw ^= 1; }
             }
           }
-          if (live) ptx::umma_commit(&bar->h_empty[sh]);
-          if (++sh == n_hslots) { sh = 0; ph ^= 1; }
+          MVLM_TRACE(1);
+          ++trace_i;
+          if (w_stat) break;
         }
-        ptx::umma_commit(&bar->t_full[acc]);
-        MVLM_TRACE(4);
-        ++trace_i;
-        if (w_stat) w_wait = false;
-        if (++acc == 2) { acc = 0; pacc ^= 1; }
+        if (prof) p.prof[blockIdx.x * 8 + 1] = w1;
       }
-      if (prof) { p.prof[blockIdx.x * 8 + 2] = w0; p.prof[blockIdx.x * 8 + 3] = w1; p.prof[blockIdx.x * 8 + 4] = clock64() - t_kernel0; }
+    } else if (warp == 1) {
+      if (ptx::elect_one()) {
+        const uint32_t idesc = ptx::umma_idesc_bf16(mma_m, p.tile_h * kTileW);
+        const bool live = (p.debug_mode & 1) == 0;
+        const int n_kx = s.kw, n_ky = s.kh;
+        const uint32_t tail_row_b = p.tail ? static_cast<uint32_t>(p.tail) * 2u : 128u;
+        const uint32_t tail_swz = !p.tail ? 2u : (p.tail == 16 ? 6u : 4u);
+        const uint64_t a_hi_full = static_cast<uint64_t>(((8u * 128u) >> 4) | (1u << 14) | (2u << 29)) << 32;
+        const uint64_t b_hi_full = static_cast<uint64_t>(((static_cast<uint32_t>(halo_px) * 128u) >> 4) | (1u << 14) | (2u << 29)) << 32;
+        const uint64_t a_hi_tail = static_cast<uint64_t>(((8u * tail_row_b) >> 4) | (1u << 14) | (tail_swz << 29)) << 32;
+        const uint64_t b_hi_tail = static_cast<uint64_t>(((static_cast<uint32_t>(halo_px) * tail_row_b) >> 4) | (1u << 14) | (tail_swz << 29)) << 32;
+        const uint32_t h_lo0 = (ptx::smem_u32(h_slots) >> 4) | (1u << 16), h_step = static_cast<uint32_t>(p.h_slot_bytes) >> 4;
+        const uint32_t w_lo0 = (ptx::smem_u32(w_slots) >> 4) | (1u << 16), w_step = w_slot_bytes >> 4;
+        const int last_chunk = n_chunks - 1;
+        const int nk_last = (s.cin - last_chunk * 64) >= 64 ? 4 : ((s.cin - last_chunk * 64) >> 4);
+        int sh = 0, sw = 0;
+        uint32_t ph = 0, pw = 0;
+        int acc = 0;
+        uint32_t pacc = 0;
+        bool w_wait = live;
+        for (int t = t_begin; t < t_end; t += t_step) {
+          timed_wait(&bar->t_empty[acc], pacc ^ 1, prof, w1);
+          ptx::tc_fence_after();
+          MVLM_TRACE(2);
+          const uint32_t d = tmem_base + static_cast<uint32_t>(acc * 256);
+          uint32_t accumulate = 0;
+          for (int c = 0; c < n_chunks; ++c) {
+            const bool is_tail = p.tail != 0 && c == last_chunk;
+            const int nk = c == last_chunk ? nk_last : 4;
+            const uint32_t rb16 = (is_tail ? tail_row_b : 128u) >> 4;
+            const uint64_t a_hi = is_tail ? a_hi_tail : a_hi_full;
+            const uint64_t b_hi = is_tail ? b_hi_tail : b_hi_full;
+            const uint32_t ky_step = static_cast<uint32_t>(halo_px) * rb16;
+            if (live) timed_wait(&bar->h_full[sh], ph, prof, w0);
+            if (c == 0) MVLM_TRACE(3);
+            uint32_t x_col = h_lo0 + static_cast<uint32_t>(sh) * h_step;
+            if (STAT && !w_wait && (nk == 4 || nk == 2 || nk == 1)) {
+              auto taps = [&](auto nk_c, auto kk_c) __attribute__((always_inline)) {
+                constexpr int NK = decltype(nk_c)::value;
+                constexpr int KK = decltype(kk_c)::value;
+                constexpr uint32_t kRb16 = NK * 2;
+                const uint32_t tap16 = M64 ? (64u * 128u >> 4) : w_step;
+                const uint32_t w_base = w_lo0 + static_cast<uint32_t>(c * KK * KK) * tap16;
+  #pragma unroll
+                for (int tap = 0; tap < KK * KK; ++tap) {
+                  const uint32_t x_lo = x_col + static_cast<uint32_t>(((tap % KK) * (kTileW + KK - 1) + tap / KK)) * kRb16;
+                  const uint32_t w_lo = w_base + static_cast<uint32_t>(tap) * tap16;
+  #pragma unroll
+                  for (int k = 0; k < NK; ++k) {
+                    const uint32_t en = (tap == 0 && k == 0) ? accumulate : 1u;
+                    if constexpr (M64) ptx::umma_ws_bf16(d, a_hi | (w_lo + 2 * k), b_hi | (x_lo + 2 * k), idesc, en);
+                    else ptx::umma_bf16(d, a_hi | (w_lo + 2 * k), b_hi | (x_lo + 2 * k), idesc, en);
+                  }
+                }
+                accumulate = 1;
+              };
+              using std::integral_constant;
+              if constexpr (M64) {
+                if (nk == 4) taps(integral_constant<int, 4>(), integral_constant<int, 3>());
+                else if (nk == 2) taps(integral_constant<int, 2>(), integral_constant<int, 3>());
+                else taps(integral_constant<int, 1>(), integral_constant<int, 3>());
+              } else {
+                if (nk == 4) taps(integral_constant<int, 4>(), integral_constant<int, 2>());
+                else if (nk == 2) taps(integral_constant<int, 2>(), integral_constant<int, 2>());
+                else taps(integral_constant<int, 1>(), integral_constant<int, 2>());
+              }
+            } else if constexpr (M64) {
+              for (int kx = 0; kx < n_kx; ++kx, x_col += rb16) {
+                if (w_wait) timed_wait(&bar->w_full[sw], w_stat ? 0u : pw, prof, w0);
+                uint32_t x_lo = x_col;
+                uint32_t w_lo = w_lo0 + static_cast<uint32_t>(sw) * w_step;
+                for (int ky = 0; ky < n_ky; ++ky, x_lo += ky_step, w_lo += (w_tap_bytes >> 4)) {
+                  ptx::umma_ws_bf16(d, a_hi | w_lo, b_hi | x_lo, idesc, accumulate);
+                  if (nk == 4) {
+                    ptx::umma_ws_bf16(d, a_hi | (w_lo + 2), b_hi | (x_lo + 2), idesc, 1u);
+                    ptx::umma_ws_bf16(d, a_hi | (w_lo + 4), b_hi | (x_lo + 4), idesc, 1u);
+                    ptx::umma_ws_bf16(d, a_hi | (w_lo + 6), b_hi | (x_lo + 6), idesc, 1u);
+                  } else {
+                    for (int k = 1; k < nk; ++k) ptx::umma_ws_bf16(d, a_hi | (w_lo + 2 * k), b_hi | (x_lo + 2 * k), idesc, 1u);
+                  }
+                  accumulate = 1;
+                }
+                if (live && !w_stat) ptx::umma_commit(&bar->w_empty[sw]);
+                if (++sw == n_wslots) { sw = 0; pw ^= 1; }
+              }
+            } else
+            for (int kx = 0; kx < n_kx; ++kx, x_col += rb16) {
+              uint32_t x_lo = x_col;
+              for (int ky = 0; ky < n_ky; ++ky, x_lo += ky_step) {
+                if (w_wait) timed_wait(&bar->w_full[sw], w_stat ? 0u : pw, prof, w0);
+                const uint32_t w_lo = w_lo0 + static_cast<uint32_t>(sw) * w_step;
+                auto mma = [&](int k, uint32_t en) __attribute__((always_inline)) {
+                  if constexpr (M64) ptx::umma_ws_bf16(d, a_hi | (w_lo + 2 * k), b_hi | (x_lo + 2 * k), idesc, en);
+                  else ptx::umma_bf16(d, a_hi | (w_lo + 2 * k), b_hi | (x_lo + 2 * k), idesc, en);
+                };
+                mma(0, accumulate);
+                if (nk == 4) {
+                  mma(1, 1u); mma(2, 1u); mma(3, 1u);
+                } else {
+                  for (int k = 1; k < nk; ++k) mma(k, 1u);
+                }
+                accumulate = 1;
+                if (live && !w_stat) ptx::umma_commit(&bar->w_empty[sw]);
+                if (++sw == n_wslots) { sw = 0; pw ^= 1; }
+              }
+            }
+            if (live) ptx::umma_commit(&bar->h_empty[sh]);
+            if (++sh == n_hslots) { sh = 0; ph ^= 1; }
+          }
+          ptx::umma_commit(&bar->t_full[acc]);
+          MVLM_TRACE(4);
+          ++trace_i;
+          if (w_stat) w_wait = false;
+          if (++acc == 2) { acc = 0; pacc ^= 1; }
+        }
+        if (prof) { p.prof[blockIdx.x * 8 + 2] = w0; p.prof[blockIdx.x * 8 + 3] = w1; p.prof[blockIdx.x * 8 + 4] = clock64() - t_kernel0; }
+      }
     }
   } else {
-    float* stage = stage_all + (warp - 2) * kStageFloats;
+    if constexpr (WIDE) asm volatile("setmaxnreg.inc.sync.aligned.u32 %0;" ::"n"(kWideEpiRegs));
+    float* stage = stage_all + (warp - kEpi0) * kStageFloats;
     const ChannelParams cp = {ep->bias, ep->mid_s, ep->mid_t, ep->pre_s, ep->pre_t, ep->post_s, ep->post_t};
     int acc = 0;
     uint32_t pacc = 0;
     ArgmaxState am;
     EpiTrace tr;
-    tr.trace = trace; tr.t0 = t_kernel0; tr.on = warp == 2 && lane == 0;
+    tr.trace = trace; tr.t0 = t_kernel0; tr.on = warp == kEpi0 && lane == 0;
     TileIter it(p, t_begin, t_step);
     for (int t = t_begin; t < t_end; t += t_step, it.next()) {
       const TileCoord tc = it.c;
@@ -354,17 +365,17 @@
         ptx::tc_fence_after();
       } else {
         epilogue_tile<F>(s, e, p.tile_h, cp, tc, &bar->t_full[acc], pacc, tmem_base + static_cast<uint32_t>(acc * 256),
-                         stage, warp - 2, warp & 3, lane, am, prof, w0, tr);
+                         stage, warp - kEpi0, warp & 3, lane, am, prof, w0, tr);
       }
       ptx::tc_fence_before();
       __syncwarp();
       if (lane == 0) ptx::mbar_arrive(&bar->t_empty[acc]);
-      if (warp == 2 && lane == 0) MVLM_TRACE(6);
+      if (warp == kEpi0 && lane == 0) MVLM_TRACE(6);
       ++trace_i;
       if (++acc == 2) { acc = 0; pacc ^= 1; }
     }
     epilogue_argmax_flush<F>(s, e, warp & 3, lane, am);
-    if (prof && warp == 2 && lane == 0) { p.prof[blockIdx.x * 8 + 5] = w0; p.prof[blockIdx.x * 8 + 6] = clock64() - t_kernel0; }
+    if (prof && warp == kEpi0 && lane == 0) { p.prof[blockIdx.x * 8 + 5] = w0; p.prof[blockIdx.x * 8 + 6] = clock64() - t_kernel0; }
   }
 
 #undef MVLM_TRACE
@@ -395,18 +406,25 @@
 
 template <int F>
 int launch_t(const ConvParams& p, cudaStream_t stream) {
+  constexpr int kSmemBytes = smem_bytes(F);
   static std::atomic<bool> configured[kMaxDevices];
   int dev = 0;
   MVLM_CHECK_CUDA(cudaGetDevice(&dev));
   if (dev < 0 || dev >= kMaxDevices || !configured[dev].load(std::memory_order_acquire)) {
     MVLM_CHECK_CUDA(cudaFuncSetAttribute(conv_umma_kernel<F>, cudaFuncAttributeMaxDynamicSharedMemorySize, kSmemBytes));
+    if (F & F_EPI16) {
+      cudaFuncAttributes fa;
+      MVLM_CHECK_CUDA(cudaFuncGetAttributes(&fa, conv_umma_kernel<F>));
+      MVLM_REQUIRE(fa.numRegs == kWideLaunchRegs, "conv_launch: 16-warp epilogue variant 0x%x built with %d registers, not %d",
+                   F, fa.numRegs, kWideLaunchRegs);
+    }
     if (dev >= 0 && dev < kMaxDevices) configured[dev].store(true, std::memory_order_release);
   }
   const int n_sms = sm_count();
   const int grid = p.total_tiles < n_sms ? p.total_tiles : n_sms;
   cudaLaunchConfig_t cfg = {};
   cfg.gridDim = dim3(static_cast<unsigned>(grid));
-  cfg.blockDim = dim3(kThreads);
+  cfg.blockDim = dim3(cta_threads(F));
   cfg.dynamicSmemBytes = kSmemBytes;
   cfg.stream = stream;
   cudaLaunchAttribute attr[1];
@@ -420,12 +438,18 @@
   return MVLM_OK;
 }
 
+template <int F>
+int launch_form(const ConvParams& p, cudaStream_t stream) {
+  if constexpr (!epi_wide_supported(F)) return launch_t<F>(p, stream);
+  else return p.epi_wide ? launch_t<F | F_EPI16>(p, stream) : launch_t<F>(p, stream);
+}
+
 thread_local long long* g_prof_buf = nullptr;
 thread_local int g_debug_mode = 0;
 
 }
 
-int conv_plan(const ConvShape& s, const ConvEpilogue& e, ConvParams* out) {
+int conv_plan(const ConvShape& s, const ConvEpilogue& e, bool epi_wide, ConvParams* out) {
   MVLM_REQUIRE(s.in && s.wpacked, "conv_plan: null input/weights");
   MVLM_REQUIRE(s.n > 0 && s.h > 0 && s.w > 0, "conv_plan: bad image dims %d %d %d", s.n, s.h, s.w);
   MVLM_REQUIRE(s.cin >= 16 && s.cin % 16 == 0, "conv_plan: cin=%d must be a multiple of 16", s.cin);
@@ -450,6 +474,8 @@
                "conv_plan: fp32 / arg-max outputs cannot be combined with bf16 outputs or residual inputs");
   MVLM_REQUIRE(1ll * s.n * s.h * s.w < (1ll << 32), "conv_plan: %d x %d x %d pixels exceed 32-bit pixel indices", s.n, s.h, s.w);
   MVLM_REQUIRE(s.kh >= 1 && s.kh <= 3 && s.kw >= 1 && s.kw <= 3, "conv_plan: kernel %dx%d unsupported", s.kh, s.kw);
+  MVLM_REQUIRE(!epi_wide || epi_wide_supported(feature_mask(e)), "conv_plan: no 16-warp epilogue for features 0x%x",
+               feature_mask(e));
   MVLM_REQUIRE((reinterpret_cast<uintptr_t>(s.in) & 15) == 0 && (reinterpret_cast<uintptr_t>(s.wpacked) & 15) == 0,
                "conv_plan: pointers must be 16-byte aligned");
   EncodeTiledFn enc = get_encode_fn();
@@ -463,6 +489,8 @@
   p.e = e;
   const int tile_h = s.h >= 32 ? kMaxTileH : (s.h >= 16 ? 16 : ((s.h >= 8 || s.cout_pad <= 64) ? 8 : 4));
   p.tile_h = tile_h;
+  p.epi_wide = epi_wide ? 1 : 0;
+  const int pool = pool_bytes(epi_wide);
   {
     const int hbytes = (kTileW + s.kw - 1) * (tile_h + s.kh - 1) * 128;
     p.h_slot_bytes = (hbytes + 1023) & ~1023;
@@ -472,12 +500,12 @@
     const int n_wtiles = ((s.cin + 63) / 64) * (m_tile == 64 ? s.kw : s.kh * s.kw);
     int nh = s.kh * s.kw == 1 ? 3 : 2, nw = s.kh * s.kw == 1 ? 6 : (m_tile == 64 ? kMaxWSlots : 7);
     const bool fits_128 = m_tile == kMTile && s.cout_pad <= kMTile && n_wtiles <= kMaxWSlots &&
-                          nh * p.h_slot_bytes + n_wtiles * wslot <= kPoolBytes;
+                          nh * p.h_slot_bytes + n_wtiles * wslot <= pool;
     p.w_stationary = (m_tile == 64 ? n_wtiles * wslot <= kMaxWSlots * 8192 : fits_128) ? 1 : 0;
     if (p.w_stationary) nw = n_wtiles;
-    while (nh * p.h_slot_bytes + nw * wslot > kPoolBytes && nw > 2 && !p.w_stationary) --nw;
-    while (nh * p.h_slot_bytes + nw * wslot > kPoolBytes && nh > 2) --nh;
-    MVLM_REQUIRE(nh * p.h_slot_bytes + nw * wslot <= kPoolBytes, "conv_plan: operand rings do not fit");
+    while (nh * p.h_slot_bytes + nw * wslot > pool && nw > 2 && !p.w_stationary) --nw;
+    while (nh * p.h_slot_bytes + nw * wslot > pool && nh > 2) --nh;
+    MVLM_REQUIRE(nh * p.h_slot_bytes + nw * wslot <= pool, "conv_plan: operand rings do not fit");
     p.n_hslots = nh;
     p.n_wslots = nw;
   }
@@ -576,10 +604,10 @@
   const bool stat = m64 && p.w_stationary && p.s.kw == 3 && p.s.kh == 3;
 #define MVLM_CASE_BOTH(FLAGS) \
   case (FLAGS):               \
-    return m64 ? (stat ? launch_t<(FLAGS) | F_M64 | F_STAT>(p, stream) : launch_t<(FLAGS) | F_M64>(p, stream)) : launch_t<(FLAGS)>(p, stream)
+    return m64 ? (stat ? launch_form<(FLAGS) | F_M64 | F_STAT>(p, stream) : launch_form<(FLAGS) | F_M64>(p, stream)) : launch_form<(FLAGS)>(p, stream)
 #define MVLM_CASE_128(FLAGS) \
   case (FLAGS):              \
-    if (!m64) return launch_t<(FLAGS)>(p, stream); \
+    if (!m64) return launch_form<(FLAGS)>(p, stream); \
     break
   if (f == F_ARGMAX && !m64 && p.w_stationary && p.s.kw == 2 && p.s.kh == 2) return launch_t<F_ARGMAX | F_STAT>(p, stream);
   switch (f) {
diff --git a/mvlm_b200/csrc/conv_umma.cuh b/mvlm_b200/csrc/conv_umma.cuh
--- a/mvlm_b200/csrc/conv_umma.cuh
+++ b/mvlm_b200/csrc/conv_umma.cuh
@@ -62,11 +62,12 @@
   int tile_h;
   int h_slot_bytes, n_hslots, n_wslots;
   int w_stationary;
+  int epi_wide;
   long long* prof;
   int debug_mode;
 };
 
-int conv_plan(const ConvShape& s, const ConvEpilogue& e, ConvParams* out);
+int conv_plan(const ConvShape& s, const ConvEpilogue& e, bool epi_wide, ConvParams* out);
 int conv_launch(const ConvParams& p, cudaStream_t stream);
 int pack_conv_weight(const float* w_oihw, int cout, int cin, int kh, int kw, int cout_pad, int cin_pad,
                      __nv_bfloat16* out, cudaStream_t stream);
diff --git a/mvlm_b200/csrc/hourglass.cu b/mvlm_b200/csrc/hourglass.cu
--- a/mvlm_b200/csrc/hourglass.cu
+++ b/mvlm_b200/csrc/hourglass.cu
@@ -300,12 +300,13 @@
   op.tag = tag;
   op.is_head = is_head;
   op.h = in.h; op.w = in.w;
+  op.epi_wide = epi_wide_ && !is_head && in.h >= 128 && kh == 1;
   if (!layout_pass_) {
     ConvShape s;
     s.in = in.p; s.n = V_; s.h = in.h; s.w = in.w; s.cin = cin; s.in_cs = in.c;
     s.wpacked = w; s.cout_pad = cout_pad; s.n_tile = n_tile; s.kh = kh; s.kw = kw;
     s.y_off0 = y_off0; s.x_off0 = x_off0;
-    const int rc = conv_plan(s, e, &op.conv);
+    const int rc = conv_plan(s, e, op.epi_wide, &op.conv);
     if (rc) return rc;
   }
   ops_.push_back(op);
@@ -478,11 +479,14 @@
   keep_probes_ = getenv("MVLM_HG_KEEP_PROBES") != nullptr && atoi(getenv("MVLM_HG_KEEP_PROBES")) != 0;
   reuse_ = !(getenv("MVLM_HG_NO_REUSE") != nullptr && atoi(getenv("MVLM_HG_NO_REUSE")) != 0);
   fuse_elt_ = !(getenv("MVLM_HG_ELT_FUSION") != nullptr && atoi(getenv("MVLM_HG_ELT_FUSION")) == 0);
+  epi_wide_ = !(getenv("MVLM_HG_EPI_WIDE") != nullptr && atoi(getenv("MVLM_HG_EPI_WIDE")) == 0);
   bufs_.clear(); fake_off_ = 0; ws_needed_ = 0; next_buf_ = 0;
   layout_pass_ = true;
   int rc = emit();
   layout_pass_ = false;
   if (rc) return rc;
+  std::vector<bool> wide_layout;
+  for (const NetOp& op : ops_) wide_layout.push_back(op.epi_wide);
   assign_offsets();
   if (dry) return MVLM_OK;
   MVLM_REQUIRE(ws_needed_ <= ws_size_, "hourglass: workspace too small (%zu needed, %zu given)", ws_needed_, ws_size_);
@@ -495,6 +499,12 @@
   if (rc == MVLM_OK && param_off_ > param_bytes) {
     set_error("hourglass: parameter arena overrun (%zu of %zu bytes)", param_off_, param_bytes);
     rc = MVLM_E_INVALID;
+  }
+  for (size_t i = 0; rc == MVLM_OK && i < ops_.size(); ++i) {
+    if (i >= wide_layout.size() || ops_[i].epi_wide != wide_layout[i]) {
+      set_error("hourglass: op %zu: the real pass chose another epilogue form than the layout pass", i);
+      rc = MVLM_E_INVALID;
+    }
   }
   const cudaError_t ce = cudaStreamSynchronize(build_stream_);
   cudaStreamDestroy(build_stream_);
@@ -786,10 +796,10 @@
     case NetOp::CONV: {
       const ConvShape& s = op.conv.s;
       const ConvEpilogue& e = op.conv.e;
-      snprintf(buf, sizeof(buf), "conv %s %dx%d %d->%d k%d%s%s%s%s%s%s%s%s", op.tag, s.h, s.w, s.cin, s.cout_pad, s.kh,
+      snprintf(buf, sizeof(buf), "conv %s %dx%d %d->%d k%d%s%s%s%s%s%s%s%s%s", op.tag, s.h, s.w, s.cin, s.cout_pad, s.kh,
                e.out_pre ? " pre" : "", e.res1 ? " res1" : "", e.res2 ? " res2" : "", e.res_up ? " up" : "", e.out_raw ? " raw" : "",
                e.out_post ? " post" : "", e.pool2 ? " pool" : (e.aux_mode == 2 ? " +pooled" : (e.aux_mode == 1 ? " +act2" : "")),
-               e.argmax_keys ? " argmax" : "");
+               e.argmax_keys ? " argmax" : "", op.conv.epi_wide ? " epi16" : "");
       break;
     }
     case NetOp::POOL: snprintf(buf, sizeof(buf), "pool %dx%dx%d", op.h, op.w, op.c); break;
diff --git a/mvlm_b200/csrc/hourglass.cuh b/mvlm_b200/csrc/hourglass.cuh
--- a/mvlm_b200/csrc/hourglass.cuh
+++ b/mvlm_b200/csrc/hourglass.cuh
@@ -25,6 +25,7 @@
   int h = 0, w = 0, c = 0;
   size_t bytes = 0;
   bool is_head = false;
+  bool epi_wide = false;
   const char* tag = "";
 };
 
@@ -80,7 +81,7 @@
   static constexpr size_t kMaxGraphs = 8;
   std::vector<Buf> bufs_;
   size_t fake_off_ = 0, ws_needed_ = 0, next_buf_ = 0;
-  bool layout_pass_ = false, keep_probes_ = false, reuse_ = true, fuse_elt_ = false;
+  bool layout_pass_ = false, keep_probes_ = false, reuse_ = true, fuse_elt_ = false, epi_wide_ = true;
   int bn(const std::string& name, int c, const float** scale, const float** shift);
   int packed(const std::string& name, int cout, int cin, int k, int cout_pad, int cin_pad, const __nv_bfloat16** out);
   int bias(const std::string& name, int cout, int cout_pad, const float** out);
diff --git a/mvlm_b200/ops.py b/mvlm_b200/ops.py
--- a/mvlm_b200/ops.py
+++ b/mvlm_b200/ops.py
@@ -26,7 +26,7 @@
                 kh: int = 3, kw: int = 3, y_off0: int | None = None, x_off0: int | None = None,
                 bias=None, mid=None, pre=None, res1=None, res2=None, out_raw=None, post=None,
                 out_f32=None, argmax_keys=None, cout_real: int | None = None,
-                up=(1, 1, 0, 0), pool2: bool = False, res_up=None) -> None:
+                up=(1, 1, 0, 0), pool2: bool = False, res_up=None, epi_wide: bool = False) -> None:
     lib = _lib.load()
     n, h, w, cs = x.shape
     a = ConvArgs()
@@ -57,6 +57,7 @@
     a.cout_real = cout_real if cout_real is not None else wpacked.shape[0]
     a.up_sy, a.up_sx, a.up_py, a.up_px = up
     a.pool2 = 1 if pool2 else 0
+    a.epi_wide = 1 if epi_wide else 0
     if res_up is not None:
         a.res_up, a.up_cs, a.up_co = ptr(res_up[0]), res_up[0].shape[-1], res_up[1]
     check(lib.mvlm_conv2d_bf16(C.byref(a), cur_stream()), "mvlm_conv2d_bf16")
```

Result: no change. 62.76, median of 6 (+0.5%).
